# jilljenn/vae

Hardware: AMD Instinct MI355X
Metric: rating-triples/sec (ELBO step) at d=128 (higher is better)
Workload: dtype f32

## Files before the change

### include/vfm_hip.h

```cpp
#ifndef VFM_HIP_H
#define VFM_HIP_H

#include <stdint.h>

#ifdef __cplusplus
extern "C" {
#endif

#define VFM_ABI_VERSION 5
#define VFM_MAX_FIELDS 64
#define VFM_STRUCT_INIT(s) do { memset(&(s), 0, sizeof(s)); (s).struct_size = (uint32_t)sizeof(s); \
                                (s).abi_version = VFM_ABI_VERSION; } while (0)

#define VFM_E_INVALID (-1)
#define VFM_E_UNSUPPORTED (-2)

#define VFM_LIK_NORMAL 0
#define VFM_LIK_BERNOULLI 1

#define VFM_FLAG_NO_PRIOR_TERMS 1
#define VFM_FLAG_SPARSE_ADAM 4
#define VFM_FLAG_SCALED_MOMENTS 32
#define VFM_MOMENT_PERIOD 128
#define VFM_FLAG_ROWS_TOUCHED 128
#define VFM_FLAG_ZREC 1024
#define VFM_FLAG_SHARE_GPU 2048
#define VFM_FLAG_EPS_ZERO 2
#define VFM_FLAG_LINK_SOFTPLUS 16

#define VFM_P_LL 0
#define VFM_P_KL 1
#define VFM_P_G 2
#define VFM_P_ALPHA 3
#define VFM_P_BADID 4
#define VFM_P_GE0 5
#define VFM_P_REDUCED 6
#define VFM_N_PARTIALS 8
#define VFM_SLOT_NTERMS 6
#define VFM_MAX_FWD_BLOCKS 4096
#define VFM_PARTIALS_LEN (VFM_N_PARTIALS * (1 + VFM_MAX_FWD_BLOCKS))

typedef struct vfm_step_consts {
  float step_size, bc2_sqrt;
  float a1, q2, c1, c2, s1, s2;
  int32_t store_true;
  int32_t k;
  int32_t scaled;
  int32_t reserved;
  float lr, beta1, beta2, eps;
} vfm_step_consts_t;
typedef struct vfm_dev_step {
  uint64_t philox_step;
  int64_t adam_step;
  uint64_t philox_step_bwd;
  int64_t adam_step_bwd;
  int64_t tab_first, tab_len;
  const vfm_step_consts_t* tab;
  int64_t error;
} vfm_dev_step_t;
int vfm_step_consts(float lr, float beta1, float beta2, float eps_adam, int64_t step, int32_t scaled,
                    vfm_step_consts_t* out);
int vfm_dev_step_set(vfm_dev_step_t* dev_step, uint64_t philox_step, int64_t adam_step, void* stream);

typedef struct vfm_problem {
  uint32_t struct_size;
  uint32_t abi_version;
  int64_t B;
  int64_t B_global;
  int64_t T;
  int64_t nb_train;
  int32_t F;
  int32_t d;
  int32_t likelihood;
  int32_t id_bits;
  int32_t n_samples;
  int32_t flags;
  int64_t group_hi[VFM_MAX_FIELDS];
  double group_n[VFM_MAX_FIELDS];
  uint64_t seed;
  uint64_t step;
  int64_t e_lo, e_hi;
  vfm_dev_step_t* dev_step;
  float* wrec;
} vfm_problem_t;
int vfm_wrec_build_f32(const float* bias_params, const float* inv_occ, int64_t T, float* wrec, void* stream);

#define VFM_HEAVY_LIST 64
#define VFM_HEAVY_MIN 8
#define VFM_HEAVY_DIRECT 8
typedef struct vfm_index {
  uint32_t struct_size;
  uint32_t abi_version;
  const int32_t* occ_ptr;
  const int32_t* occ_rows;
  const int32_t* heavy_ids;
  const int32_t* heavy_items;
  float* heavy_acc;
  int32_t n_heavy;
  int32_t n_items;
  const int32_t* touched_ids;
  int64_t n_touched;
  const int32_t* occ_other;
  int32_t max_items;
  int32_t heavy_list, heavy_threshold;
  int32_t* status;
} vfm_index_t;

int vfm_abi_version(void);
const char* vfm_last_error(void);

int64_t vfm_index_workspace_bytes(int64_t B, int32_t F, int64_t T);
int vfm_rebuild_heavy(int64_t T, const int32_t* occ_ptr, void* ws, int32_t heavy_list, int32_t threshold, int32_t* heavy_ids,
                      int64_t cap_heavy, int32_t* heavy_items, int64_t cap_items, int32_t* counts , void* stream);
int32_t vfm_heavy_threshold(int32_t heavy_list);
#define VFM_HEAVY_UNITS 8192
int32_t vfm_heavy_list_for(int64_t n_occ, int64_t T);
int vfm_build_index(int64_t B, int32_t F, int64_t T, int32_t id_bits, const void* x, void* ws, int32_t* occ_ptr,
                    int32_t* occ_rows, int32_t heavy_list, int32_t* heavy_ids, int64_t cap_heavy,
                    int32_t* heavy_items, int64_t cap_items, int32_t* touched_ids, int32_t* occ_other,
                    const float* inv_occ, double* W, int32_t* counts, int32_t* counts_host, void* stream);

int vfm_inv_occ_f32(const int64_t* nb_occ, float* inv_occ, int64_t T, void* stream);

int vfm_batch_norms(const vfm_problem_t* p, const void* x, const float* inv_occ, double* W,
                    void* stream);

int vfm_elbo_fwd_f32(const vfm_problem_t* p, const void* x, const float* y,
                     const float* entity_params, const float* bias_params,
                     const float* inv_occ, const float* scalars, const double* W,
                     const float* eps_entity, const float* eps_bias, const float* eps_global,
                     float* pred, double* partials, float* sumz, float* grow, void* stream);

int vfm_elbo_finalize_f32(const vfm_problem_t* p, double* partials, const float* scalars,
                          float* loss, void* stream);

int vfm_elbo_bwd_f32(const vfm_problem_t* p, const vfm_index_t* idx,
                     const float* entity_params, const float* bias_params,
                     const float* inv_occ, const float* scalars, const double* W,
                     const float* eps_entity, const float* eps_bias, const float* eps_global,
                     const float* sumz, const float* grow, const double* partials,
                     const float* grad_out, float* g_entity, float* g_bias, float* g_scalars,
                     void* stream);

int vfm_elbo_bwd_adam_f32(const vfm_problem_t* p, const vfm_index_t* idx,
                          float* entity_params, float* bias_params, float* scalars,
                          const float* inv_occ, const double* W,
                          const float* eps_entity, const float* eps_bias, const float* eps_global,
                          const float* sumz, const float* grow, double* partials,
                          float* m_entity, float* v_entity, float* m_bias, float* v_bias,
                          float* m_scalars, float* v_scalars,
                          float lr, float beta1, float beta2, float eps_adam, int64_t step, float* loss,
                          void* stream);

int vfm_elbo_bwd_acc_f32(const vfm_problem_t* p, const vfm_index_t* idx,
                         const float* sumz, const float* grow, const double* partials, float* acc,
                         float* sums, void* stream);
int vfm_elbo_apply_adam_f32(const vfm_problem_t* p, const float* acc, const float* sums,
                            float* entity_params, float* bias_params, float* scalars, const float* inv_occ,
                            const double* W, const float* eps_entity, const float* eps_bias,
                            const float* eps_global, float* m_entity, float* v_entity, float* m_bias,
                            float* v_bias, float* m_scalars, float* v_scalars, float lr, float beta1,
                            float beta2, float eps_adam, int64_t step, void* stream);
int vfm_elbo_bwd_acc_rows_f32(const vfm_problem_t* p, const vfm_index_t* idx, const int32_t* row_ids, int64_t n_rows,
                              const float* sumz, const float* grow, const double* partials, float* acc,
                              float* sums, void* stream);
int vfm_elbo_apply_adam_rows_f32(const vfm_problem_t* p, const float* acc, const float* sums, const int32_t* row_ids,
                                 int64_t n_rows, int32_t compact_records, float* entity_params, float* bias_params, float* scalars,
                                 const float* inv_occ, const double* W, float* m_entity, float* v_entity, float* m_bias,
                                 float* v_bias, float* m_scalars, float* v_scalars, float lr, float beta1, float beta2,
                                 float eps_adam, int64_t step, void* stream);
int vfm_adam_f32(float* p, const float* g, float* m, float* v, int64_t n, float lr, float beta1,
                 float beta2, float eps, int64_t step, void* stream);

typedef struct vfm_pipe {
  uint32_t struct_size;
  uint32_t abi_version;
  const float* zrec;
  float* zrec_next;
  const int32_t* next_occ_ptr;
  const double* next_W;
  uint64_t next_step;
  int32_t* last_step;
  float* step_tab;
} vfm_pipe_t;
int vfm_sample_records_f32(const vfm_problem_t* p, const int32_t* ids, int64_t n, const float* entity_params,
                           const float* bias_params, const float* inv_occ, const double* W, float* zrec, void* stream);
int vfm_elbo_bwd_adam_pipe_f32(const vfm_problem_t* p, const vfm_index_t* idx, const vfm_pipe_t* pipe,
                               float* entity_params, float* bias_params, float* scalars,
                               const float* inv_occ, const double* W, const float* grow, double* partials,
                               float* m_entity, float* v_entity, float* m_bias, float* v_bias,
                               float* m_scalars, float* v_scalars,
                               float lr, float beta1, float beta2, float eps_adam, int64_t step, float* loss,
                               void* stream);

int vfm_adam_catchup_f32(float* entity_params, float* bias_params, const float* m_entity, const float* v_entity,
                         const float* m_bias, const float* v_bias, int32_t* last_step, const int32_t* ids, int64_t n,
                         int64_t T, int32_t d, const float* lr_of_step, int64_t n_lr, float beta1, float beta2,
                         float eps_adam, int64_t upto, int64_t mark, float* wrec, void* stream);

int64_t vfm_union_workspace_bytes(int64_t T);
int vfm_union_rows(int64_t T, const int32_t* occ_ptr_a, const int32_t* occ_ptr_b, void* ws, int32_t* rows, int32_t* count,
                   int32_t* count_host, void* stream);
int vfm_elbo_bwd_adam_lookahead_f32(const vfm_problem_t* p, const vfm_index_t* idx,
                                    float* entity_params, float* bias_params, float* scalars,
                                    const float* inv_occ, const double* W,
                                    const float* sumz, const float* grow, double* partials,
                                    float* m_entity, float* v_entity, float* m_bias, float* v_bias,
                                    float* m_scalars, float* v_scalars,
                                    float lr, float beta1, float beta2, float eps_adam, int64_t step, float* loss,
                                    int32_t* last_step, const int32_t* next_occ_ptr, float* step_tab, void* stream);

int vfm_moments_rescale_f32(float* m, float* v, int64_t n, float beta1, float beta2, int64_t step, int32_t to_scaled,
                            void* stream);

#define VFM_OBJ_SAMPLED 0
#define VFM_OBJ_CLOSED_FORM 1
int vfm_variant_fwd_f32(const vfm_problem_t* p, int32_t objective, const void* x, const float* values, const float* y,
                        const float* entity_params, const float* bias_params, const float* inv_occ,
                        const float* scalars, const double* W, const float* priors, const float* eps_entity,
                        const float* eps_bias, const float* eps_global, float* pred, double* partials, float* state,
                        float* grow, float* loss, void* stream);
int64_t vfm_variant_workspace_elems(int64_t B, int32_t F, int32_t d);
int vfm_variant_bwd_f32(const vfm_problem_t* p, int32_t objective, const vfm_index_t* idx, int32_t* occ_pos_ws,
                        const void* x, const float* values, const float* entity_params, const float* bias_params,
                        const float* inv_occ, const float* scalars, const double* W, const float* priors,
                        const float* eps_entity, const float* eps_bias, const float* eps_global, const float* state,
                        const float* grow, const double* partials, const float* grad_out, float* g_entity,
                        float* g_bias, float* g_scalars, float* g_priors, void* stream);

int vfm_philox_eps_f32(const vfm_problem_t* p, float* eps_entity, float* eps_bias,
                       float* eps_global, void* stream);

#ifdef __cplusplus
}
#endif
#endif
```

### vae_amd/_abi_gen.py

```python
import ctypes as C

VFM_ABI_VERSION = 5
VFM_E_INVALID = -1
VFM_E_UNSUPPORTED = -2
VFM_FLAG_EPS_ZERO = 2
VFM_FLAG_LINK_SOFTPLUS = 16
VFM_FLAG_NO_PRIOR_TERMS = 1
VFM_FLAG_ROWS_TOUCHED = 128
VFM_FLAG_SCALED_MOMENTS = 32
VFM_FLAG_SHARE_GPU = 2048
VFM_FLAG_SPARSE_ADAM = 4
VFM_FLAG_ZREC = 1024
VFM_HEAVY_DIRECT = 8
VFM_HEAVY_LIST = 64
VFM_HEAVY_MIN = 8
VFM_HEAVY_UNITS = 8192
VFM_LIK_BERNOULLI = 1
VFM_LIK_NORMAL = 0
VFM_MAX_FIELDS = 64
VFM_MAX_FWD_BLOCKS = 4096
VFM_MOMENT_PERIOD = 128
VFM_N_PARTIALS = 8
VFM_OBJ_CLOSED_FORM = 1
VFM_OBJ_SAMPLED = 0
VFM_PARTIALS_LEN = 32776
VFM_P_ALPHA = 3
VFM_P_BADID = 4
VFM_P_G = 2
VFM_P_GE0 = 5
VFM_P_KL = 1
VFM_P_LL = 0
VFM_P_REDUCED = 6
VFM_SLOT_NTERMS = 6


class StepConsts(C.Structure):
    _fields_ = [
        ("step_size", C.c_float),
        ("bc2_sqrt", C.c_float),
        ("a1", C.c_float),
        ("q2", C.c_float),
        ("c1", C.c_float),
        ("c2", C.c_float),
        ("s1", C.c_float),
        ("s2", C.c_float),
        ("store_true", C.c_int32),
        ("k", C.c_int32),
        ("scaled", C.c_int32),
        ("reserved", C.c_int32),
        ("lr", C.c_float),
        ("beta1", C.c_float),
        ("beta2", C.c_float),
        ("eps", C.c_float),
    ]


class DevStep(C.Structure):
    _fields_ = [
        ("philox_step", C.c_uint64),
        ("adam_step", C.c_int64),
        ("philox_step_bwd", C.c_uint64),
        ("adam_step_bwd", C.c_int64),
        ("tab_first", C.c_int64),
        ("tab_len", C.c_int64),
        ("tab", C.c_void_p),
        ("error", C.c_int64),
    ]


class Problem(C.Structure):
    _fields_ = [
        ("struct_size", C.c_uint32),
        ("abi_version", C.c_uint32),
        ("B", C.c_int64),
        ("B_global", C.c_int64),
        ("T", C.c_int64),
        ("nb_train", C.c_int64),
        ("F", C.c_int32),
        ("d", C.c_int32),
        ("likelihood", C.c_int32),
        ("id_bits", C.c_int32),
        ("n_samples", C.c_int32),
        ("flags", C.c_int32),
        ("group_hi", C.c_int64 * VFM_MAX_FIELDS),
        ("group_n", C.c_double * VFM_MAX_FIELDS),
        ("seed", C.c_uint64),
        ("step", C.c_uint64),
        ("e_lo", C.c_int64),
        ("e_hi", C.c_int64),
        ("dev_step", C.c_void_p),
        ("wrec", C.c_void_p),
    ]

    def __init__(self, *a, **k):
        super().__init__(*a, **k)
        self.struct_size, self.abi_version = C.sizeof(type(self)), VFM_ABI_VERSION


class Index(C.Structure):
    _fields_ = [
        ("struct_size", C.c_uint32),
        ("abi_version", C.c_uint32),
        ("occ_ptr", C.c_void_p),
        ("occ_rows", C.c_void_p),
        ("heavy_ids", C.c_void_p),
        ("heavy_items", C.c_void_p),
        ("heavy_acc", C.c_void_p),
        ("n_heavy", C.c_int32),
        ("n_items", C.c_int32),
        ("touched_ids", C.c_void_p),
        ("n_touched", C.c_int64),
        ("occ_other", C.c_void_p),
        ("max_items", C.c_int32),
        ("heavy_list", C.c_int32),
        ("heavy_threshold", C.c_int32),
        ("status", C.c_void_p),
    ]

    def __init__(self, *a, **k):
        super().__init__(*a, **k)
        self.struct_size, self.abi_version = C.sizeof(type(self)), VFM_ABI_VERSION


class Pipe(C.Structure):
    _fields_ = [
        ("struct_size", C.c_uint32),
        ("abi_version", C.c_uint32),
        ("zrec", C.c_void_p),
        ("zrec_next", C.c_void_p),
        ("next_occ_ptr", C.c_void_p),
        ("next_W", C.c_void_p),
        ("next_step", C.c_uint64),
        ("last_step", C.c_void_p),
        ("step_tab", C.c_void_p),
    ]

    def __init__(self, *a, **k):
        super().__init__(*a, **k)
        self.struct_size, self.abi_version = C.sizeof(type(self)), VFM_ABI_VERSION
```

### vae_amd/csrc/vfm_abi.hip

```cpp
#include <stdio.h>
#include <string.h>
#include <math.h>
#include <stdlib.h>
#include <mutex>

#include "vfm_args.hpp"

namespace vfm {

namespace {
thread_local char g_err[512] = "";
}

int fail(int code, const char* msg) {
  snprintf(g_err, sizeof(g_err), "%s", msg);
  return code;
}
int fail_hip(hipError_t e, const char* where) {
  snprintf(g_err, sizeof(g_err), "%s: %s", where, hipGetErrorString(e));
  return (int)e;
}
int env_int(const char* name, int dflt) {
  const char* v = getenv(name);
  return (v && *v) ? atoi(v) : dflt;
}

namespace {

#include "vfm_rng.hpp"
#include "vfm_common.hpp"
#include "vfm_reduce.hpp"
#include "vfm_small_kernels.hpp"
#include "vfm_heavy.hpp"
#include "vfm_adam.hpp"

bool pick_shape(int d, Shape* s) {
  auto pow2ceil = [](int v) { int p = 1; while (p < v) p <<= 1; return p; };
  if (d % 4 == 0) {
    const int C = d / 4;
    s->vec = 4;
    s->lpe = pow2ceil(C) < 64 ? (pow2ceil(C) < 4 ? 4 : pow2ceil(C)) : 64;
    const int cpl = (C + s->lpe - 1) / s->lpe;
    s->cpl = cpl <= 1 ? 1 : (cpl <= 2 ? 2 : 4);
    return cpl <= 4;
  }
  s->vec = 1;
  if (d <= 8) { s->lpe = 8; s->cpl = 1; return true; }
  if (d <= 64) { s->lpe = 64; s->cpl = 1; return true; }
  s->lpe = 64; s->cpl = 4;
  return d <= 256;
}

int check_struct(uint32_t size, uint32_t abi, size_t want, const char* name) {
  if (size == (uint32_t)want && abi == (uint32_t)VFM_ABI_VERSION) return 0;
  snprintf(g_err, sizeof(g_err), "%s: struct_size %u / abi_version %u, this library expects %zu / %d (set them with "
           "VFM_STRUCT_INIT; a binding generated from another version of include/vfm_hip.h must be regenerated)",
           name, size, abi, want, VFM_ABI_VERSION);
  return VFM_E_INVALID;
}

int check_problem(const vfm_problem_t* p, bool dev_ok = false) {
  if (!p) return fail(VFM_E_INVALID, "problem is NULL");
  if (int rc = check_struct(p->struct_size, p->abi_version, sizeof(vfm_problem_t), "vfm_problem_t")) return rc;
  if (p->dev_step && !dev_ok)
    return fail(VFM_E_UNSUPPORTED, "vfm_problem_t.dev_step: only the training forward and the fused backward+Adam entry points read the step from device memory");
  if (p->dev_step && p->n_samples != 1) return fail(VFM_E_UNSUPPORTED, "vfm_problem_t.dev_step: one variational sample");
  if (p->dev_step && (((uintptr_t)p->dev_step) & 15) != 0) return fail(VFM_E_INVALID, "vfm_problem_t.dev_step must be 16-byte aligned");
  if (p->wrec && (((uintptr_t)p->wrec) & 15) != 0) return fail(VFM_E_INVALID, "vfm_problem_t.wrec must be 16-byte aligned");
  if (p->B < 0 || p->T <= 0 || p->T > 0xFFFFFFFELL) return fail(VFM_E_INVALID, "bad B or T");
  if (p->F < 1 || p->F > VFM_MAX_FIELDS) return fail(VFM_E_INVALID, "F out of range [1,64]");
  if (p->d < 1) return fail(VFM_E_INVALID, "d < 1");
  if (p->id_bits != 32 && p->id_bits != 64) return fail(VFM_E_INVALID, "id_bits must be 32 or 64");
  if (p->likelihood != VFM_LIK_NORMAL && p->likelihood != VFM_LIK_BERNOULLI)
    return fail(VFM_E_INVALID, "unknown likelihood");
  if (p->n_samples < 1 || p->n_samples > MAX_SAMPLES) return fail(VFM_E_INVALID, "n_samples out of range [1,64]");
  if (p->n_samples > 1 && (p->step >> 48) != 0) return fail(VFM_E_INVALID, "step must stay below 2^48 when n_samples > 1");
  if (p->B_global < p->B) return fail(VFM_E_INVALID, "B_global < B");
  if (p->B * (int64_t)p->F > 0x7FFFFFFFLL) return fail(VFM_E_INVALID, "B*F exceeds int32 index range");
  if (p->e_lo < 0 || p->e_lo > p->T || (p->e_hi != 0 && p->e_hi < p->e_lo)) return fail(VFM_E_INVALID, "bad entity range");
  if (p->flags & ~(VFM_FLAG_NO_PRIOR_TERMS | VFM_FLAG_EPS_ZERO | VFM_FLAG_SPARSE_ADAM | VFM_FLAG_LINK_SOFTPLUS |
                   VFM_FLAG_SCALED_MOMENTS | VFM_FLAG_ROWS_TOUCHED | VFM_FLAG_ZREC | VFM_FLAG_SHARE_GPU))
    return fail(VFM_E_INVALID, "unknown bit in vfm_problem_t.flags");
  Shape s;
  if (!pick_shape(p->d, &s)) return fail(VFM_E_UNSUPPORTED, "embedding size d not supported (d%4==0: d<=1024, else d<=256)");
  return 0;
}

bool softplus(const vfm_problem_t* p) { return (p->flags & VFM_FLAG_LINK_SOFTPLUS) != 0; }

int single_sample_only(const vfm_problem_t* p, const char* who) {
  if (p->n_samples == 1) return 0;
  snprintf(g_err, sizeof(g_err), "%s: n_samples > 1 is not supported by this entry point", who);
  return VFM_E_UNSUPPORTED;
}


int eps_mode(const vfm_problem_t* p, const float* ee, const float* eb, const float* eg, int* mode) {
  const int neps = (ee != nullptr) + (eb != nullptr) + (eg != nullptr);
  if (neps != 0 && neps != 3) return fail(VFM_E_INVALID, "give all three eps tables or none");
  *mode = (p->flags & VFM_FLAG_EPS_ZERO) ? EPS_ZERO : (neps == 3 ? EPS_TABLE : EPS_PHILOX);
  return 0;
}

KArgs make_args(const vfm_problem_t* p, const void* x, const float* y, const float* entity,
                const float* bias, const float* inv_occ, const float* scalars, const double* W,
                const float* ee, const float* eb, const float* eg, int sample = 0) {
  KArgs a;
  memset(&a, 0, sizeof(a));
  a.S = p->n_samples; a.sample = sample; a.inv_S = 1.0f / (float)p->n_samples;
  if (sample > 0) {
    if (ee) ee += (size_t)sample * (size_t)p->T * (size_t)p->d;
    if (eb) eb += (size_t)sample * (size_t)p->T;
  }
  a.B = p->B; a.T = p->T; a.F = p->F; a.d = p->d; a.lik = p->likelihood;
  a.e_lo = p->e_lo; a.e_hi = (p->e_hi > 0 && p->e_hi < p->T) ? p->e_hi : p->T;
  a.id64 = p->id_bits == 64; a.G = p->F; a.flags = p->flags;
  a.ll_scale_d = (double)p->nb_train / ((double)(p->B_global > 0 ? p->B_global : 1) * (double)p->n_samples);
  a.ll_scale = (float)a.ll_scale_d;
  a.key.seed_lo = (uint32_t)p->seed; a.key.seed_hi = (uint32_t)(p->seed >> 32);
  a.key.step_lo = (uint32_t)p->step; a.key.step_hi = (uint32_t)(p->step >> 32);
  a.key.chunk_off = 0;
  a.x = x; a.y = y; a.entity = entity; a.bias = bias; a.inv_occ = inv_occ; a.scalars = scalars;
  a.W = W; a.eps_entity = ee; a.eps_bias = eb; a.eps_global = eg;
  a.dev = p->dev_step; a.wrec = p->wrec;
  for (int g = 0; g < p->F; ++g) { a.group_hi[g] = p->group_hi[g]; a.group_n[g] = p->group_n[g]; }
  return a;
}

bool use_fwd2(const vfm_problem_t* p, int eps, bool multi = false) {
  if (p->F != 2 || (p->d & 3) != 0 || p->d > 512) return false;
  if (multi ? (p->n_samples < 2 || p->n_samples > 4 || eps == EPS_ZERO) : p->n_samples != 1) return false;
  if (softplus(p)) return false;
  const int forced = env_int("VFM_FWD_KERNEL", 0);
  if (forced == 1) return false;
  return forced == 2 || eps == EPS_ZREC || multi || p->d >= 20;
}

bool use_fwdg(const vfm_problem_t* p, int eps, int mode) {
  if (p->F == 2 || (p->d & 3) != 0 || p->d < 16 || p->d > 512 || p->n_samples != 1) return false;
  if ((p->flags & VFM_FLAG_ZREC) || softplus(p)) return false;
  if (!(eps == EPS_PHILOX || (eps == EPS_ZERO && mode == MODE_PREDICT))) return false;
  return env_int("VFM_FWD_KERNEL", 0) != 1;
}

int dispatch_fwd(const vfm_problem_t* p, const Shape& s, int eps, int mode, int ff, KArgs& a, const FwdOut& o,
                 hipStream_t st) {
  if (use_fwdg(p, eps, mode)) return launch_fwdg_abs(eps, mode, a, o, st);
  if (use_fwd2(p, eps)) {
    if (mode == MODE_TRAIN && eps == EPS_PHILOX && env_int("VFM_FWD_AB_NORNG", 0) == 1) eps = EPS_ZERO;
    return launch_fwd2_abs(eps, mode, a, o, st);
  }
  return softplus(p) ? launch_fwd_softplus(s, eps, mode, ff, a, o, st) : launch_fwd_abs(s, eps, mode, ff, a, o, st);
}
int dispatch_bwd(const vfm_problem_t* p, const Shape& s, int eps, int adam, KArgs& a, const BwdArgs& b,
                 const AdamArgs& ad, hipStream_t st) {
  if (adam == 0 || adam == 10)
    return softplus(p) ? launch_bwd0_softplus(s, eps, adam, a, b, ad, st) : launch_bwd0_abs(s, eps, adam, a, b, ad, st);
  return softplus(p) ? launch_bwd1_softplus(s, eps, adam, a, b, ad, st) : launch_bwd1_abs(s, eps, adam, a, b, ad, st);
}

BwdArgs bwd_args(const vfm_problem_t* p, const vfm_index_t* idx) {
  BwdArgs b;
  memset(&b, 0, sizeof(b));
  if (idx) { b.occ_ptr = idx->occ_ptr; b.occ_rows = idx->occ_rows; b.status = idx->status; }
  b.n_occ = (int32_t)(p->B * (int64_t)p->F);
  return b;
}

template <int LPE, int CPL, int VEC>
int launch_heavy_t(const vfm_problem_t* p, const vfm_index_t* idx, const float* sumz, const float* grow, float* hacc, int d,
                   hipStream_t st, const float* zrec = nullptr) {
  constexpr int GPB = BLOCK / LPE;
  const size_t xs = 4 + (((size_t)d + 3) & ~(size_t)3);
  float* item_acc = hacc + xs * (size_t)idx->n_heavy;
  int64_t nb = ((int64_t)idx->n_items + GPB - 1) / GPB;
  if (nb > 4096) nb = 4096;
  hipLaunchKernelGGL((k_heavy<LPE, CPL, VEC>), dim3((unsigned)nb), dim3(BLOCK), 0, st, idx->heavy_items,
                     (int)idx->n_items, idx->occ_rows, sumz, grow, item_acc, d, zrec ? idx->occ_other : nullptr, zrec, hacc,
                     (int)idx->n_heavy, (int)(p->B * (int64_t)p->F), (int)p->B, p->T, idx->status);
  if (idx->max_items > 0 && idx->max_items <= VFM_HEAVY_DIRECT) return 0;
  nb = idx->n_heavy;
  if (nb > 4096) nb = 4096;
  hipLaunchKernelGGL((k_heavy_sum<LPE, CPL, VEC>), dim3((unsigned)nb), dim3(BLOCK), 0, st, idx->heavy_items,
                     (int)idx->n_items, (int)idx->n_heavy, item_acc, hacc, d);
  return 0;
}

int run_heavy(const vfm_problem_t* p, const vfm_index_t* idx, const float* sumz, const float* grow,
              hipStream_t st, BwdArgs* b, const float* zrec = nullptr) {
  b->heavy_ids = nullptr; b->heavy_acc = nullptr; b->n_heavy = 0; b->heavy_stride = 0;
  if (idx->n_heavy <= 0 || idx->n_items <= 0) return 0;
  if (!idx->heavy_ids || !idx->heavy_items || !idx->heavy_acc)
    return fail(VFM_E_INVALID, "index: heavy_ids / heavy_items / heavy_acc missing");
  if ((int64_t)idx->n_heavy > p->T || (int64_t)idx->n_items > p->B * (int64_t)p->F + idx->n_heavy)
    return fail(VFM_E_INVALID, "index: more heavy entities than table rows, or more work items than occurrences");
  const size_t xs = 4 + (((size_t)p->d + 3) & ~(size_t)3);
  const size_t per_sample = xs * ((size_t)idx->n_heavy + (size_t)idx->n_items);
  Shape s;
  pick_shape(p->d, &s);
  for (int sm = 0; sm < p->n_samples; ++sm) {
    const float* sz = sumz ? sumz + (size_t)sm * (size_t)p->B * (size_t)p->d : nullptr;
    float* hacc = idx->heavy_acc + (size_t)sm * per_sample;
#define X(L_, C_, V_) \
    if (s.lpe == L_ && s.cpl == C_ && s.vec == V_) launch_heavy_t<L_, C_, V_>(p, idx, sz, grow, hacc, p->d, st, zrec);
    VFM_FOR_SHAPES(X)
#undef X
  }
  b->heavy_ids = idx->heavy_ids; b->heavy_acc = idx->heavy_acc; b->n_heavy = idx->n_heavy;
  b->heavy_stride = idx->n_heavy + idx->n_items;
  return 0;
}

struct Side { hipStream_t s = nullptr; hipEvent_t e1 = nullptr, e2 = nullptr; bool ok = false, tried = false; std::mutex mu; };
Side* side_of_device() {
  static Side sides[64];
  static std::mutex mu;
  int dev = 0;
  if (hipGetDevice(&dev) != hipSuccess || dev < 0 || dev >= 64) return nullptr;
  std::lock_guard<std::mutex> lk(mu);
  Side& sd = sides[dev];
  if (!sd.tried) {
    sd.tried = true;
    sd.ok = hipStreamCreateWithFlags(&sd.s, hipStreamNonBlocking) == hipSuccess &&
            hipEventCreateWithFlags(&sd.e1, hipEventDisableTiming) == hipSuccess &&
            hipEventCreateWithFlags(&sd.e2, hipEventDisableTiming) == hipSuccess;
  }
  return sd.ok ? &sd : nullptr;
}
bool heavy_overlap(const vfm_problem_t* p, const vfm_index_t* idx) {
  return idx->n_heavy > 0 && idx->n_items > 0 && (int64_t)idx->n_heavy * 16 < p->T && p->n_samples == 1 &&
         env_int("VFM_HEAVY_OVERLAP", 1) != 0;
}

int bwd_adam_overlapped(const vfm_problem_t* p, const vfm_index_t* idx, const Shape& s, int eps, int adam, KArgs& a, BwdArgs& b,
                        const AdamArgs& ad, const float* sumz, const float* grow, hipStream_t st, Side* sd) {
  std::lock_guard<std::mutex> lk(sd->mu);
  hipError_t e = hipEventRecord(sd->e1, st);
  if (e == hipSuccess) e = hipStreamWaitEvent(sd->s, sd->e1, 0);
  if (e != hipSuccess) return fail_hip(e, "heavy-list overlap: events");
  if (int rc = run_heavy(p, idx, sumz, grow, sd->s, &b)) return rc;
  e = hipEventRecord(sd->e2, sd->s);
  if (e != hipSuccess) return fail_hip(e, "heavy-list overlap: events");
  const int32_t keep = a.row_filter;
  a.row_filter = 4;
  if (int rc = dispatch_bwd(p, s, eps, adam, a, b, ad, st)) return rc;
  e = hipStreamWaitEvent(st, sd->e2, 0);
  if (e != hipSuccess) return fail_hip(e, "heavy-list overlap: events");
  BwdArgs bh = b;
  bh.row_ids = idx->heavy_ids; bh.n_rows = idx->n_heavy;
  a.row_filter = 3;
  const int rc = dispatch_bwd(p, s, eps, adam, a, bh, ad, st);
  a.row_filter = keep;
  return rc;
}

bool small_table_step(const vfm_problem_t* p, const vfm_index_t* idx, int eps, int rows_flags) {
  if (eps != EPS_PHILOX || rows_flags != 0 || p->n_samples != 1 || (p->flags & VFM_FLAG_SPARSE_ADAM)) return false;
  if ((p->d & 3) != 0 || p->d > 256) return false;
  if (idx->heavy_list < VFM_HEAVY_MIN || idx->heavy_threshold < VFM_HEAVY_MIN || idx->heavy_threshold > idx->heavy_list) return false;
  if (p->T * (2 * (int64_t)p->d + 2) * 4 > (2LL << 20)) return false;
  return env_int("VFM_BWD_SMALL", 1) != 0;
}

int check_index(const vfm_problem_t* p, const vfm_index_t* idx, const char* who) {
  if (!idx) { snprintf(g_err, sizeof(g_err), "%s: inverted index missing", who); return VFM_E_INVALID; }
  if (int rc = check_struct(idx->struct_size, idx->abi_version, sizeof(vfm_index_t), "vfm_index_t")) return rc;
  if (!idx->occ_ptr || (p->B > 0 && !idx->occ_rows)) {
    snprintf(g_err, sizeof(g_err), "%s: inverted index missing", who);
    return VFM_E_INVALID;
  }
  if (idx->n_heavy < 0 || idx->n_items < 0 || idx->n_touched < 0 || idx->max_items < 0) {
    snprintf(g_err, sizeof(g_err), "%s: negative count in vfm_index_t", who);
    return VFM_E_INVALID;
  }
  return 0;
}

int after_launch(const char* where) {
  const hipError_t e = hipGetLastError();
  if (e != hipSuccess) return fail_hip(e, where);
  return 0;
}

void adam_consts(float lr, float beta1, float beta2, int64_t step, float* step_size, float* bc2_sqrt) {
  const double bc1 = 1.0 - pow((double)beta1, (double)step);
  const double bc2 = 1.0 - pow((double)beta2, (double)step);
  *step_size = (float)((double)lr / bc1);
  *bc2_sqrt = (float)sqrt(bc2);
}

void scaled_step_consts(float step_size, float bc2_sqrt, double s1, double s2, float* a1, float* q2) {
  *a1 = (float)((double)step_size * s1);
  *q2 = (float)(sqrt(s2) / (double)bc2_sqrt);
}

int scaled_moment_consts(const vfm_problem_t* p, float beta1, float beta2, int64_t step, AdamArgs* ad) {
  ad->scaled = 0; ad->store_true = 0; ad->s1 = ad->s2 = 1.f; ad->c1 = 1.f - beta1; ad->c2 = 1.f - beta2;
  ad->inv_bc2_sqrt = 1.0f / ad->bc2_sqrt;
  ad->a1 = ad->step_size; ad->q2 = ad->inv_bc2_sqrt;
  if (!(p->flags & VFM_FLAG_SCALED_MOMENTS)) return 0;
  if (p->flags & VFM_FLAG_SPARSE_ADAM)
    return fail(VFM_E_INVALID, "VFM_FLAG_SCALED_MOMENTS and VFM_FLAG_SPARSE_ADAM exclude each other");
  const int64_t k = (step - 1) % VFM_MOMENT_PERIOD + 1;
  const double s1 = pow((double)beta1, (double)k), s2 = pow((double)beta2, (double)k);
  if (!(s1 > 1e-30) || !(s2 > 1e-30))
    return fail(VFM_E_UNSUPPORTED, "VFM_FLAG_SCALED_MOMENTS: beta^128 underflows (use the plain moments for such betas)");
  ad->scaled = 1; ad->store_true = (k == VFM_MOMENT_PERIOD);
  ad->s1 = (float)s1; ad->s2 = (float)s2;
  ad->c1 = (float)((1.0 - (double)beta1) / s1); ad->c2 = (float)((1.0 - (double)beta2) / s2);
  scaled_step_consts(ad->step_size, ad->bc2_sqrt, s1, s2, &ad->a1, &ad->q2);
  return 0;
}

}
}

using namespace vfm;

int vfm::launch_norms(int64_t B, int F, int64_t T, int id_bits, const void* x, const float* inv_occ, double* W, hipStream_t st) {
  hipLaunchKernelGGL(k_zero_f64, dim3(1), dim3(64), 0, st, W, F);
  if (B == 0) return after_launch("vfm_batch_norms");
  int64_t nbx = (B + BLOCK * 8 - 1) / (BLOCK * 8);
  if (nbx > 1024) nbx = 1024;
  hipLaunchKernelGGL(k_norms, dim3((unsigned)nbx, (unsigned)F), dim3(BLOCK), 0, st, x, (int)(id_bits == 64), inv_occ, B, F, T,
                     reinterpret_cast<unsigned long long*>(W));
  hipLaunchKernelGGL(k_norms_fix, dim3(1), dim3(64), 0, st, W, F);
  return after_launch("vfm_batch_norms");
}

extern "C" {

int vfm_abi_version(void) { return VFM_ABI_VERSION; }
const char* vfm_last_error(void) { return g_err; }

int vfm_step_consts(float lr, float beta1, float beta2, float eps_adam, int64_t step, int32_t scaled,
                    vfm_step_consts_t* out) {
  if (!out || step < 1) return fail(VFM_E_INVALID, "vfm_step_consts: bad argument");
  vfm_problem_t p;
  memset(&p, 0, sizeof(p));
  p.flags = scaled ? VFM_FLAG_SCALED_MOMENTS : 0;
  AdamArgs ad;
  memset(&ad, 0, sizeof(ad));
  ad.b1 = beta1; ad.b2 = beta2; ad.eps = eps_adam;
  adam_consts(lr, beta1, beta2, step, &ad.step_size, &ad.bc2_sqrt);
  if (int rc = scaled_moment_consts(&p, beta1, beta2, step, &ad)) return rc;
  memset(out, 0, sizeof(*out));
  out->step_size = ad.step_size; out->bc2_sqrt = ad.bc2_sqrt; out->a1 = ad.a1; out->q2 = ad.q2;
  out->c1 = ad.c1; out->c2 = ad.c2; out->s1 = ad.s1; out->s2 = ad.s2;
  out->store_true = ad.store_true; out->k = (int32_t)((step - 1) % VFM_MOMENT_PERIOD + 1); out->scaled = ad.scaled;
  out->lr = lr; out->beta1 = beta1; out->beta2 = beta2; out->eps = eps_adam;
  return 0;
}

int vfm_dev_step_set(vfm_dev_step_t* dev_step, uint64_t philox_step, int64_t adam_step, void* stream) {
  if (!dev_step || adam_step < 1) return fail(VFM_E_INVALID, "vfm_dev_step_set: bad argument");
  hipLaunchKernelGGL(k_dev_step_set, dim3(1), dim3(64), 0, (hipStream_t)stream, dev_step, philox_step, adam_step);
  return after_launch("vfm_dev_step_set");
}

int vfm_wrec_build_f32(const float* bias_params, const float* inv_occ, int64_t T, float* wrec, void* stream) {
  if (!bias_params || !inv_occ || !wrec || T <= 0 || (((uintptr_t)wrec) & 15) != 0)
    return fail(VFM_E_INVALID, "vfm_wrec_build_f32: bad argument");
  const int grid = (int)((T + 255) / 256 < 2048 ? (T + 255) / 256 : 2048);
  hipLaunchKernelGGL(k_wrec_build, dim3(grid), dim3(256), 0, (hipStream_t)stream, bias_params, inv_occ, T, wrec);
  return after_launch("vfm_wrec_build_f32");
}

int vfm_inv_occ_f32(const int64_t* nb_occ, float* inv_occ, int64_t T, void* stream) {
  if (!nb_occ || !inv_occ || T <= 0) return fail(VFM_E_INVALID, "vfm_inv_occ_f32: bad argument");
  const int grid = (int)((T + 255) / 256 < 2048 ? (T + 255) / 256 : 2048);
  hipLaunchKernelGGL(k_inv_occ, dim3(grid), dim3(256), 0, (hipStream_t)stream, nb_occ, inv_occ, T);
  return after_launch("vfm_inv_occ_f32");
}

int vfm_batch_norms(const vfm_problem_t* p, const void* x, const float* inv_occ, double* W,
                    void* stream) {
  if (int rc = check_problem(p)) return rc;
  if (!W || (p->B > 0 && (!x || !inv_occ))) return fail(VFM_E_INVALID, "vfm_batch_norms: NULL pointer");
  return launch_norms(p->B, p->F, p->T, p->id_bits, x, inv_occ, W, (hipStream_t)stream);
}

int vfm_elbo_fwd_f32(const vfm_problem_t* p, const void* x, const float* y,
                     const float* entity_params, const float* bias_params,
                     const float* inv_occ, const float* scalars, const double* W,
                     const float* eps_entity, const float* eps_bias, const float* eps_global,
                     float* pred, double* partials, float* sumz, float* grow, void* stream) {
  if (int rc = check_problem(p, true)) return rc;
  if (!partials) return fail(VFM_E_INVALID, "vfm_elbo_fwd_f32: partials is NULL");
  if (p->dev_step && (eps_entity || eps_bias || eps_global || (p->flags & VFM_FLAG_EPS_ZERO)))
    return fail(VFM_E_UNSUPPORTED, "vfm_elbo_fwd_f32: dev_step goes with the in-kernel Philox eps stream only");
  hipStream_t st0 = (hipStream_t)stream;
  if (p->B == 0) {
    hipLaunchKernelGGL(k_zero_f64, dim3(1), dim3(64), 0, st0, partials, (int)VFM_N_PARTIALS);
    return after_launch("vfm_elbo_fwd_f32");
  }
  const bool zrec = (p->flags & VFM_FLAG_ZREC) != 0;
  if (zrec) {
    if (!use_fwd2(p, EPS_ZREC)) return fail(VFM_E_UNSUPPORTED, "VFM_FLAG_ZREC: two fields, one sample, d % 4 == 0, d <= 512, |.| link");
    if (!x || !y || !entity_params || !scalars || !pred || !grow || eps_entity || eps_bias || eps_global)
      return fail(VFM_E_INVALID, "vfm_elbo_fwd_f32 (VFM_FLAG_ZREC): x, y, the record table, scalars, pred, grow; no eps tables");
    KArgs a = make_args(p, x, y, entity_params, nullptr, nullptr, scalars, nullptr, nullptr, nullptr, nullptr, 0);
    FwdOut o{pred, partials, nullptr, grow};
    if (int rc = launch_fwd2_abs(EPS_ZREC, MODE_TRAIN, a, o, (hipStream_t)stream)) return rc;
    return after_launch("vfm_elbo_fwd_f32");
  }
  if (!x || !entity_params || !bias_params || !scalars || !pred)
    return fail(VFM_E_INVALID, "vfm_elbo_fwd_f32: NULL pointer");
  const bool train = y != nullptr;
  if (train && (!inv_occ || !W || !sumz || !grow))
    return fail(VFM_E_INVALID, "vfm_elbo_fwd_f32: y given, so inv_occ, W, sumz and grow are required");
  if (!train && (sumz || grow)) return fail(VFM_E_INVALID, "vfm_elbo_fwd_f32: sumz / grow need y");
  int eps;
  if (int rc = eps_mode(p, eps_entity, eps_bias, eps_global, &eps)) return rc;
  if (train && eps == EPS_ZERO) return fail(VFM_E_UNSUPPORTED, "vfm_elbo_fwd_f32: VFM_FLAG_EPS_ZERO is prediction-only");
  hipStream_t st = (hipStream_t)stream;
  FwdOut o{pred, partials, sumz, grow};
  Shape s;
  pick_shape(p->d, &s);
  if (use_fwd2(p, eps, true)) {
    KArgs a = make_args(p, x, y, entity_params, bias_params, inv_occ, scalars, W, eps_entity, eps_bias, eps_global, 0);
    const int md = train ? MODE_TRAIN : MODE_PREDICT;
    if (int rc = launch_fwd2m_abs(eps, md, a, o, st)) return rc;
    return after_launch("vfm_elbo_fwd_f32");
  }
  for (int sm = 0; sm < p->n_samples; ++sm) {
    KArgs a = make_args(p, x, y, entity_params, bias_params, inv_occ, scalars, W, eps_entity, eps_bias,
                        eps_global, sm);
    if (int rc = dispatch_fwd(p, s, eps, train ? MODE_TRAIN : MODE_PREDICT, p->F == 2 ? 2 : 0, a, o, st)) return rc;
  }
  return after_launch("vfm_elbo_fwd_f32");
}

int vfm_elbo_finalize_f32(const vfm_problem_t* p, double* partials, const float* scalars,
                          float* loss, void* stream) {
  if (int rc = check_problem(p)) return rc;
  if (!partials || !scalars || !loss) return fail(VFM_E_INVALID, "vfm_elbo_finalize_f32: NULL pointer");
  const double ll_scale = (double)p->nb_train / ((double)(p->B_global > 0 ? p->B_global : 1) * (double)p->n_samples);
  hipLaunchKernelGGL(k_finalize, dim3(1), dim3(BLOCK), 0, (hipStream_t)stream, partials, scalars, ll_scale,
                     (int)p->flags, loss);
  return after_launch("vfm_elbo_finalize_f32");
}

int vfm_elbo_bwd_f32(const vfm_problem_t* p, const vfm_index_t* idx,
                     const float* entity_params, const float* bias_params,
                     const float* inv_occ, const float* scalars, const double* W,
                     const float* eps_entity, const float* eps_bias, const float* eps_global,
                     const float* sumz, const float* grow, const double* partials,
                     const float* grad_out, float* g_entity, float* g_bias, float* g_scalars,
                     void* stream) {
  if (int rc = check_problem(p)) return rc;
  if (int rc = check_index(p, idx, "vfm_elbo_bwd_f32")) return rc;
  if (!entity_params || !bias_params || !inv_occ || !scalars || !W || !partials || !grad_out ||
      !g_entity || !g_bias || !g_scalars || (p->B > 0 && (!sumz || !grow)))
    return fail(VFM_E_INVALID, "vfm_elbo_bwd_f32: NULL pointer");
  int eps;
  if (int rc = eps_mode(p, eps_entity, eps_bias, eps_global, &eps)) return rc;
  if (eps == EPS_ZERO) return fail(VFM_E_UNSUPPORTED, "vfm_elbo_bwd_f32: VFM_FLAG_EPS_ZERO is prediction-only");
  KArgs a = make_args(p, nullptr, nullptr, entity_params, bias_params, inv_occ, scalars, W, eps_entity,
                      eps_bias, eps_global);
  BwdArgs b = bwd_args(p, idx);
  b.sumz = sumz; b.grow = grow; b.partials = const_cast<double*>(partials); b.grad_out = grad_out;
  b.g_entity = g_entity; b.g_bias = g_bias; b.g_scalars = g_scalars;
  if (int rc = run_heavy(p, idx, sumz, grow, (hipStream_t)stream, &b)) return rc;
  AdamArgs ad;
  memset(&ad, 0, sizeof(ad));
  Shape s;
  pick_shape(p->d, &s);
  if (int rc = dispatch_bwd(p, s, eps, 0, a, b, ad, (hipStream_t)stream)) return rc;
  return after_launch("vfm_elbo_bwd_f32");
}

int vfm_elbo_bwd_adam_f32(const vfm_problem_t* p, const vfm_index_t* idx,
                          float* entity_params, float* bias_params, float* scalars,
                          const float* inv_occ, const double* W,
                          const float* eps_entity, const float* eps_bias, const float* eps_global,
                          const float* sumz, const float* grow, double* partials,
                          float* m_entity, float* v_entity, float* m_bias, float* v_bias,
                          float* m_scalars, float* v_scalars,
                          float lr, float beta1, float beta2, float eps_adam, int64_t step, float* loss,
                          void* stream) {
  if (int rc = check_problem(p, true)) return rc;
  if (int rc = check_index(p, idx, "vfm_elbo_bwd_adam_f32")) return rc;
  if (p->dev_step) {
    if ((p->flags & VFM_FLAG_SPARSE_ADAM) || eps_entity || eps_bias || eps_global)
      return fail(VFM_E_UNSUPPORTED, "vfm_elbo_bwd_adam_f32: dev_step excludes VFM_FLAG_SPARSE_ADAM and eps tables");
    step = 1; lr = 0.f;
  }
  const int rows_flags = p->flags & VFM_FLAG_ROWS_TOUCHED;
  if (rows_flags && (p->flags & VFM_FLAG_SPARSE_ADAM))
    return fail(VFM_E_INVALID, "vfm_elbo_bwd_adam_f32: VFM_FLAG_ROWS_TOUCHED does not combine with VFM_FLAG_SPARSE_ADAM");
  if (!entity_params || !bias_params || !scalars || !m_entity ||
      !v_entity || !m_bias || !v_bias || !m_scalars || !v_scalars || step < 1 ||
      !inv_occ || !W || !partials || (p->B > 0 && (!sumz || !grow)))
    return fail(VFM_E_INVALID, "vfm_elbo_bwd_adam_f32: bad argument");
  if (p->flags & VFM_FLAG_NO_PRIOR_TERMS)
    return fail(VFM_E_INVALID, "vfm_elbo_bwd_adam_f32: single-rank only (gradients never leave the kernel)");
  int eps;
  if (int rc = eps_mode(p, eps_entity, eps_bias, eps_global, &eps)) return rc;
  if (eps == EPS_ZERO) return fail(VFM_E_UNSUPPORTED, "vfm_elbo_bwd_adam_f32: VFM_FLAG_EPS_ZERO is prediction-only");
  KArgs a = make_args(p, nullptr, nullptr, entity_params, bias_params, inv_occ, scalars, W, eps_entity,
                      eps_bias, eps_global);
  a.row_filter = rows_flags == VFM_FLAG_ROWS_TOUCHED ? 2 : 0;
  BwdArgs b = bwd_args(p, idx);
  b.sumz = sumz; b.grow = grow; b.partials = partials; b.loss = loss;
  if (small_table_step(p, idx, eps, rows_flags)) {
    AdamArgs ad{m_entity, v_entity, m_bias, v_bias, m_scalars, v_scalars, beta1, beta2, eps_adam, 0.f, 0.f};
    adam_consts(lr, beta1, beta2, step, &ad.step_size, &ad.bc2_sqrt);
    if (int rc = scaled_moment_consts(p, beta1, beta2, step, &ad)) return rc;
    Shape s;
    pick_shape(p->d, &s);
    if (int rc = softplus(p) ? launch_bwd_small_softplus(s, a, b, ad, idx->heavy_list, idx->heavy_threshold, (hipStream_t)stream)
                             : launch_bwd_small_abs(s, a, b, ad, idx->heavy_list, idx->heavy_threshold, (hipStream_t)stream))
      return rc;
    return after_launch("vfm_elbo_bwd_adam_f32");
  }
  Side* sd = (!(p->flags & VFM_FLAG_SPARSE_ADAM) && heavy_overlap(p, idx)) ? side_of_device() : nullptr;
  if (!sd)
    if (int rc = run_heavy(p, idx, sumz, grow, (hipStream_t)stream, &b)) return rc;
  AdamArgs ad{m_entity, v_entity, m_bias, v_bias, m_scalars, v_scalars, beta1, beta2, eps_adam, 0.f, 0.f};
  adam_consts(lr, beta1, beta2, step, &ad.step_size, &ad.bc2_sqrt);
  if (int rc = scaled_moment_consts(p, beta1, beta2, step, &ad)) return rc;
  Shape s;
  pick_shape(p->d, &s);
  int adam = (p->flags & VFM_FLAG_SPARSE_ADAM) ? 2 : 1;
  if (rows_flags == VFM_FLAG_ROWS_TOUCHED && idx->touched_ids && idx->n_touched <= p->T && env_int("VFM_ROWS_LIST", 1) != 0) {
    b.row_ids = idx->touched_ids; b.n_rows = idx->n_touched;
    a.row_filter = 0;
  }
  if (sd && a.row_filter == 0) {
    if (int rc = bwd_adam_overlapped(p, idx, s, eps, adam, a, b, ad, sumz, grow, (hipStream_t)stream, sd)) return rc;
    return after_launch("vfm_elbo_bwd_adam_f32");
  }
  if (sd)
    if (int rc = run_heavy(p, idx, sumz, grow, (hipStream_t)stream, &b)) return rc;
  if (int rc = dispatch_bwd(p, s, eps, adam, a, b, ad, (hipStream_t)stream)) return rc;
  return after_launch("vfm_elbo_bwd_adam_f32");
}

static int bwd_acc_impl(const vfm_problem_t* p, const vfm_index_t* idx, const int32_t* row_ids, int64_t n_rows,
                        const float* sumz, const float* grow, const double* partials, float* acc, float* sums, void* stream,
                        const char* who) {
  if (int rc = check_problem(p)) return rc;
  if (int rc = single_sample_only(p, who)) return rc;
  if (int rc = check_index(p, idx, who)) return rc;
  if (!partials || !acc || !sums || (p->B > 0 && (!sumz || !grow)))
    return fail(VFM_E_INVALID, "vfm_elbo_bwd_acc_f32: NULL pointer");
  KArgs a = make_args(p, nullptr, nullptr, nullptr, nullptr, nullptr, nullptr, nullptr, nullptr, nullptr, nullptr);
  BwdArgs b = bwd_args(p, idx);
  b.sumz = sumz; b.grow = grow; b.partials = const_cast<double*>(partials); b.acc = acc; b.sums = sums;
  if (row_ids) {
    if (n_rows < 0 || n_rows > p->T || p->e_lo != 0 || (p->e_hi != 0 && p->e_hi != p->T))
      return fail(VFM_E_INVALID, "vfm_elbo_bwd_acc_rows_f32: 0 <= n_rows <= T, whole entity range");
    b.row_ids = row_ids; b.n_rows = n_rows; b.rec_by_slot = 1;
  }
  if (p->e_lo == 0)
    if (int rc = run_heavy(p, idx, sumz, grow, (hipStream_t)stream, &b)) return rc;
  if (p->e_lo != 0 && idx->n_heavy > 0) {
    b.heavy_ids = idx->heavy_ids; b.heavy_acc = idx->heavy_acc; b.n_heavy = idx->n_heavy;
    b.heavy_stride = idx->n_heavy + idx->n_items;
  }
  AdamArgs ad;
  memset(&ad, 0, sizeof(ad));
  Shape s;
  pick_shape(p->d, &s);
  if (int rc = dispatch_bwd(p, s, EPS_ZERO, 10, a, b, ad, (hipStream_t)stream)) return rc;
  return after_launch(who);
}

int vfm_elbo_bwd_acc_f32(const vfm_problem_t* p, const vfm_index_t* idx,
                         const float* sumz, const float* grow, const double* partials, float* acc,
                         float* sums, void* stream) {
  return bwd_acc_impl(p, idx, nullptr, 0, sumz, grow, partials, acc, sums, stream, "vfm_elbo_bwd_acc_f32");
}

int vfm_elbo_bwd_acc_rows_f32(const vfm_problem_t* p, const vfm_index_t* idx, const int32_t* row_ids, int64_t n_rows,
                              const float* sumz, const float* grow, const double* partials, float* acc,
                              float* sums, void* stream) {
  static const int32_t none = 0;
  if (!row_ids && n_rows != 0) return fail(VFM_E_INVALID, "vfm_elbo_bwd_acc_rows_f32: row_ids is NULL");
  return bwd_acc_impl(p, idx, row_ids ? row_ids : &none, n_rows, sumz, grow, partials, acc, sums, stream,
                      "vfm_elbo_bwd_acc_rows_f32");
}

static int apply_adam_impl(const vfm_problem_t* p, const float* acc, const float* sums,
                           float* entity_params, float* bias_params, float* scalars, const float* inv_occ,
                           const double* W, const float* eps_entity, const float* eps_bias,
                           const float* eps_global, float* m_entity, float* v_entity, float* m_bias,
                           float* v_bias, float* m_scalars, float* v_scalars, float lr, float beta1,
                           float beta2, float eps_adam, int64_t step, const int32_t* row_ids, int64_t n_rows,
                           int32_t compact, void* stream, const char* who) {
  if (int rc = check_problem(p)) return rc;
  if (int rc = single_sample_only(p, who)) return rc;
  if (!acc || !sums || !entity_params || !bias_params || !scalars || !inv_occ || !W || !m_entity ||
      !v_entity || !m_bias || !v_bias || !m_scalars || !v_scalars || step < 1)
    return fail(VFM_E_INVALID, "vfm_elbo_apply_adam_f32: bad argument");
  int eps;
  if (int rc = eps_mode(p, eps_entity, eps_bias, eps_global, &eps)) return rc;
  if (eps == EPS_ZERO) return fail(VFM_E_UNSUPPORTED, "vfm_elbo_apply_adam_f32: VFM_FLAG_EPS_ZERO is prediction-only");
  KArgs a = make_args(p, nullptr, nullptr, entity_params, bias_params, inv_occ, scalars, W, eps_entity, eps_bias,
                      eps_global);
  BwdArgs b = bwd_args(p, nullptr);
  b.acc = const_cast<float*>(acc); b.sums = const_cast<float*>(sums);
  if (row_ids) {
    if (n_rows < 0 || n_rows > p->T) return fail(VFM_E_INVALID, "vfm_elbo_apply_adam_rows_f32: 0 <= n_rows <= T");
    b.row_ids = row_ids; b.n_rows = n_rows; b.rec_by_slot = compact ? 1 : 0;
  }
  AdamArgs ad{m_entity, v_entity, m_bias, v_bias, m_scalars, v_scalars, beta1, beta2, eps_adam, 0.f, 0.f};
  adam_consts(lr, beta1, beta2, step, &ad.step_size, &ad.bc2_sqrt);
  if (int rc = scaled_moment_consts(p, beta1, beta2, step, &ad)) return rc;
  if (row_ids && (!ad.scaled || ad.store_true))
    return fail(VFM_E_INVALID, "vfm_elbo_apply_adam_rows_f32: scaled moments only, and not on the last step of a moment period "
                               "(bring every row up to date and run vfm_elbo_apply_adam_f32)");
  Shape s;
  pick_shape(p->d, &s);
  if (int rc = dispatch_bwd(p, s, eps, 11, a, b, ad, (hipStream_t)stream)) return rc;
  return after_launch(who);
}

int vfm_elbo_apply_adam_f32(const vfm_problem_t* p, const float* acc, const float* sums,
                            float* entity_params, float* bias_params, float* scalars, const float* inv_occ,
                            const double* W, const float* eps_entity, const float* eps_bias,
                            const float* eps_global, float* m_entity, float* v_entity, float* m_bias,
                            float* v_bias, float* m_scalars, float* v_scalars, float lr, float beta1,
                            float beta2, float eps_adam, int64_t step, void* stream) {
  return apply_adam_impl(p, acc, sums, entity_params, bias_params, scalars, inv_occ, W, eps_entity, eps_bias, eps_global,
                         m_entity, v_entity, m_bias, v_bias, m_scalars, v_scalars, lr, beta1, beta2, eps_adam, step,
                         nullptr, 0, 0, stream, "vfm_elbo_apply_adam_f32");
}

int vfm_elbo_apply_adam_rows_f32(const vfm_problem_t* p, const float* acc, const float* sums, const int32_t* row_ids,
                                 int64_t n_rows, int32_t compact_records, float* entity_params, float* bias_params, float* scalars,
                                 const float* inv_occ, const double* W, float* m_entity, float* v_entity, float* m_bias,
                                 float* v_bias, float* m_scalars, float* v_scalars, float lr, float beta1, float beta2,
                                 float eps_adam, int64_t step, void* stream) {
  if (!row_ids && n_rows != 0) return fail(VFM_E_INVALID, "vfm_elbo_apply_adam_rows_f32: row_ids is NULL");
  static const int32_t none = 0;
  return apply_adam_impl(p, acc, sums, entity_params, bias_params, scalars, inv_occ, W, nullptr, nullptr, nullptr,
                         m_entity, v_entity, m_bias, v_bias, m_scalars, v_scalars, lr, beta1, beta2, eps_adam, step,
                         row_ids ? row_ids : &none, n_rows, compact_records, stream,
                         "vfm_elbo_apply_adam_rows_f32");
}

int vfm_adam_f32(float* p, const float* g, float* m, float* v, int64_t n, float lr, float beta1,
                 float beta2, float eps, int64_t step, void* stream) {
  if (!p || !g || !m || !v || n < 0 || step < 1) return fail(VFM_E_INVALID, "vfm_adam_f32: bad argument");
  if (n == 0) return 0;
  if ((((uintptr_t)p | (uintptr_t)g | (uintptr_t)m | (uintptr_t)v) & 15) != 0)
    return fail(VFM_E_INVALID, "vfm_adam_f32: pointers must be 16-byte aligned");
  float step_size, bc2_sqrt;
  adam_consts(lr, beta1, beta2, step, &step_size, &bc2_sqrt);
  const int64_t n4 = n / 4;
  int64_t nb = (n4 + BLOCK - 1) / BLOCK;
  if (nb < 1) nb = 1;
  const int grid = (int)(nb < 4096 ? nb : 4096);
  hipLaunchKernelGGL(k_adam, dim3(grid), dim3(BLOCK), 0, (hipStream_t)stream, p, g, m, v, n4, n, beta1,
                     beta2, eps, step_size, bc2_sqrt);
  return after_launch("vfm_adam_f32");
}

int vfm_sample_records_f32(const vfm_problem_t* p, const int32_t* ids, int64_t n, const float* entity_params,
                           const float* bias_params, const float* inv_occ, const double* W, float* zrec, void* stream) {
  if (int rc = check_problem(p)) return rc;
  if (int rc = single_sample_only(p, "vfm_sample_records_f32")) return rc;
  if ((p->d & 3) != 0 || softplus(p)) return fail(VFM_E_UNSUPPORTED, "vfm_sample_records_f32: d % 4 == 0, |.| link");
  if (n < 0 || n > 0x7FFFFFFFLL || (n > 0 && (!ids || !entity_params || !bias_params || !inv_occ || !W || !zrec)))
    return fail(VFM_E_INVALID, "vfm_sample_records_f32: bad argument");
  if (n == 0) return 0;
  KArgs a = make_args(p, nullptr, nullptr, entity_params, bias_params, inv_occ, nullptr, W, nullptr, nullptr, nullptr);
  Shape s;
  pick_shape(p->d, &s);
  if (int rc = launch_sample_rec_abs(s, a, ids, (int)n, zrec, (hipStream_t)stream)) return rc;
  return after_launch("vfm_sample_records_f32");
}

int vfm_elbo_bwd_adam_pipe_f32(const vfm_problem_t* p, const vfm_index_t* idx, const vfm_pipe_t* pipe,
                               float* entity_params, float* bias_params, float* scalars,
                               const float* inv_occ, const double* W, const float* grow, double* partials,
                               float* m_entity, float* v_entity, float* m_bias, float* v_bias,
                               float* m_scalars, float* v_scalars,
                               float lr, float beta1, float beta2, float eps_adam, int64_t step, float* loss,
                               void* stream) {
  if (int rc = check_problem(p, true)) return rc;
  if (p->dev_step) { step = 1; lr = 0.f; }
  if (int rc = single_sample_only(p, "vfm_elbo_bwd_adam_pipe_f32")) return rc;
  if (int rc = check_index(p, idx, "vfm_elbo_bwd_adam_pipe_f32")) return rc;
  if (p->F != 2 || (p->d & 3) != 0 || p->d > 512)
    return fail(VFM_E_UNSUPPORTED, "vfm_elbo_bwd_adam_pipe_f32: two fields, d % 4 == 0, d <= 512");
  if (p->flags & ~(VFM_FLAG_SCALED_MOMENTS | VFM_FLAG_SHARE_GPU))
    return fail(VFM_E_UNSUPPORTED, "vfm_elbo_bwd_adam_pipe_f32: only VFM_FLAG_SCALED_MOMENTS (the record step exists for the |.| link)");
  if (!pipe) return fail(VFM_E_INVALID, "vfm_elbo_bwd_adam_pipe_f32: pipe is NULL");
  if (int rc = check_struct(pipe->struct_size, pipe->abi_version, sizeof(vfm_pipe_t), "vfm_pipe_t")) return rc;
  if (!pipe->zrec || (p->B > 0 && !idx->occ_other) ||
      (pipe->zrec_next && (!pipe->next_occ_ptr || !pipe->next_W)))
    return fail(VFM_E_INVALID, "vfm_elbo_bwd_adam_pipe_f32: pipe / idx->occ_other incomplete");
  if (pipe->last_step) {
    if (!pipe->next_occ_ptr || !pipe->step_tab || !(p->flags & VFM_FLAG_SCALED_MOMENTS))
      return fail(VFM_E_INVALID, "vfm_elbo_bwd_adam_pipe_f32 (look-ahead form): next_occ_ptr, step_tab and VFM_FLAG_SCALED_MOMENTS");
    if (!p->dev_step && step % VFM_MOMENT_PERIOD == 0)
      return fail(VFM_E_INVALID, "vfm_elbo_bwd_adam_pipe_f32 (look-ahead form): the last step of a moment period is a dense one");
  }
  if (!entity_params || !bias_params || !scalars || !m_entity || !v_entity || !m_bias || !v_bias || !m_scalars ||
      !v_scalars || step < 1 || !inv_occ || !W || !partials || (p->B > 0 && !grow))
    return fail(VFM_E_INVALID, "vfm_elbo_bwd_adam_pipe_f32: bad argument");
  KArgs a = make_args(p, nullptr, nullptr, entity_params, bias_params, inv_occ, scalars, W, nullptr, nullptr, nullptr);
  BwdArgs b = bwd_args(p, idx);
  b.grow = grow; b.partials = partials; b.loss = loss;
  if (int rc = run_heavy(p, idx, nullptr, grow, (hipStream_t)stream, &b, pipe->zrec)) return rc;
  b.zrec = pipe->zrec; b.occ_other = idx->occ_other;
  b.zrec_next = pipe->zrec_next; b.next_occ_ptr = pipe->next_occ_ptr; b.next_W = pipe->next_W;
  b.next_key = a.key;
  b.next_key.step_lo = (uint32_t)pipe->next_step; b.next_key.step_hi = (uint32_t)(pipe->next_step >> 32);
  if (pipe->last_step) {
    b.last_step = pipe->last_step; b.step_tab = reinterpret_cast<float2*>(pipe->step_tab);
    b.la_step = (int32_t)step; b.la_k = (int32_t)((step - 1) % VFM_MOMENT_PERIOD + 1);
    if (idx->touched_ids && idx->n_touched > 0) {
      if (idx->n_touched > p->T) return fail(VFM_E_INVALID, "vfm_elbo_bwd_adam_pipe_f32: more listed rows than table rows");
      b.row_ids = idx->touched_ids; b.n_rows = idx->n_touched;
    }
  }
  AdamArgs ad{m_entity, v_entity, m_bias, v_bias, m_scalars, v_scalars, beta1, beta2, eps_adam, 0.f, 0.f};
  adam_consts(lr, beta1, beta2, step, &ad.step_size, &ad.bc2_sqrt);
  if (int rc = scaled_moment_consts(p, beta1, beta2, step, &ad)) return rc;
  Shape s;
  pick_shape(p->d, &s);
  if (int rc = dispatch_bwd(p, s, EPS_PHILOX, 1, a, b, ad, (hipStream_t)stream)) return rc;
  return after_launch("vfm_elbo_bwd_adam_pipe_f32");
}

int vfm_elbo_bwd_adam_lookahead_f32(const vfm_problem_t* p, const vfm_index_t* idx,
                                    float* entity_params, float* bias_params, float* scalars,
                                    const float* inv_occ, const double* W,
                                    const float* sumz, const float* grow, double* partials,
                                    float* m_entity, float* v_entity, float* m_bias, float* v_bias,
                                    float* m_scalars, float* v_scalars,
                                    float lr, float beta1, float beta2, float eps_adam, int64_t step, float* loss,
                                    int32_t* last_step, const int32_t* next_occ_ptr, float* step_tab, void* stream) {
  if (int rc = check_problem(p, true)) return rc;
  if (p->dev_step) { step = 1; lr = 0.f; }
  if (int rc = single_sample_only(p, "vfm_elbo_bwd_adam_lookahead_f32")) return rc;
  if (int rc = check_index(p, idx, "vfm_elbo_bwd_adam_lookahead_f32")) return rc;
  if ((p->flags & ~(VFM_FLAG_LINK_SOFTPLUS | VFM_FLAG_SHARE_GPU)) != VFM_FLAG_SCALED_MOMENTS)
    return fail(VFM_E_INVALID, "vfm_elbo_bwd_adam_lookahead_f32: VFM_FLAG_SCALED_MOMENTS (and optionally the link flag) only");
  if (!entity_params || !bias_params || !scalars || !m_entity || !v_entity || !m_bias || !v_bias || !m_scalars ||
      !v_scalars || step < 1 || !inv_occ || !W || !partials || (p->B > 0 && (!sumz || !grow)) || !last_step ||
      !next_occ_ptr || !step_tab)
    return fail(VFM_E_INVALID, "vfm_elbo_bwd_adam_lookahead_f32: bad argument");
  if (step % VFM_MOMENT_PERIOD == 0)
    return fail(VFM_E_INVALID, "vfm_elbo_bwd_adam_lookahead_f32: the last step of a moment period is a dense one "
                               "(bring every row up to date, then vfm_elbo_bwd_adam_f32)");
  KArgs a = make_args(p, nullptr, nullptr, entity_params, bias_params, inv_occ, scalars, W, nullptr, nullptr, nullptr);
  BwdArgs b = bwd_args(p, idx);
  b.sumz = sumz; b.grow = grow; b.partials = partials; b.loss = loss;
  Side* sd = heavy_overlap(p, idx) ? side_of_device() : nullptr;
  if (!sd)
    if (int rc = run_heavy(p, idx, sumz, grow, (hipStream_t)stream, &b)) return rc;
  b.last_step = last_step; b.next_occ_ptr = next_occ_ptr; b.step_tab = reinterpret_cast<float2*>(step_tab);
  if (idx->touched_ids && idx->n_touched > 0) {
    if (idx->n_touched > p->T) return fail(VFM_E_INVALID, "vfm_elbo_bwd_adam_lookahead_f32: more listed rows than table rows");
    b.row_ids = idx->touched_ids; b.n_rows = idx->n_touched;
  }
  b.la_step = (int32_t)step; b.la_k = (int32_t)((step - 1) % VFM_MOMENT_PERIOD + 1);
  AdamArgs ad{m_entity, v_entity, m_bias, v_bias, m_scalars, v_scalars, beta1, beta2, eps_adam, 0.f, 0.f};
  adam_consts(lr, beta1, beta2, step, &ad.step_size, &ad.bc2_sqrt);
  if (int rc = scaled_moment_consts(p, beta1, beta2, step, &ad)) return rc;
  Shape s;
  pick_shape(p->d, &s);
  if (sd) {
    if (int rc = bwd_adam_overlapped(p, idx, s, EPS_PHILOX, 1, a, b, ad, sumz, grow, (hipStream_t)stream, sd)) return rc;
    return after_launch("vfm_elbo_bwd_adam_lookahead_f32");
  }
  if (int rc = dispatch_bwd(p, s, EPS_PHILOX, 1, a, b, ad, (hipStream_t)stream)) return rc;
  return after_launch("vfm_elbo_bwd_adam_lookahead_f32");
}

int vfm_adam_catchup_f32(float* entity_params, float* bias_params, const float* m_entity, const float* v_entity,
                         const float* m_bias, const float* v_bias, int32_t* last_step, const int32_t* ids, int64_t n,
                         int64_t T, int32_t d, const float* lr_of_step, int64_t n_lr, float beta1, float beta2,
                         float eps_adam, int64_t upto, int64_t mark, float* wrec, void* stream) {
  if (!entity_params || !bias_params || !m_entity || !v_entity || !m_bias || !v_bias || !last_step || n < 0 || T < 1 ||
      d < 1 || upto < 0 || mark < upto || mark > 0x7FFFFFFFLL || (ids == nullptr && n != T))
    return fail(VFM_E_INVALID, "vfm_adam_catchup_f32: bad argument (ids == NULL means all T rows: n == T)");
  if (n == 0 || upto == 0) {
    if (n == 0) return 0;
  }
  const int64_t pstart = upto > 0 ? ((upto - 1) / VFM_MOMENT_PERIOD) * VFM_MOMENT_PERIOD : 0;
  const int kmax = (int)(upto - pstart);
  if (kmax > 0 && (!lr_of_step || n_lr < kmax))
    return fail(VFM_E_INVALID, "vfm_adam_catchup_f32: lr_of_step (host) needs one entry per step of the period up to `upto` (n_lr too small)");
  if (wrec && (((uintptr_t)wrec) & 15) != 0) return fail(VFM_E_INVALID, "vfm_adam_catchup_f32: wrec must be 16-byte aligned");
  CatchTab tab;
  memset(&tab, 0, sizeof(tab));
  for (int k = 1; k <= kmax; ++k) {
    float step_size, bc2_sqrt;
    adam_consts(lr_of_step[k - 1], beta1, beta2, pstart + k, &step_size, &bc2_sqrt);
    const double s1 = pow((double)beta1, (double)k), s2 = pow((double)beta2, (double)k);
    if (!(s1 > 1e-30) || !(s2 > 1e-30)) return fail(VFM_E_UNSUPPORTED, "vfm_adam_catchup_f32: beta^k underflows");
    float a1, q2;
    scaled_step_consts(step_size, bc2_sqrt, s1, s2, &a1, &q2);
    tab.c[k] = make_float4(a1, q2, 0.f, 0.f);
  }
  int64_t nb = (n + BLOCK / 64 - 1) / (BLOCK / 64);
  if (nb > 8192) nb = 8192;
  if ((d & 1) == 0)
    hipLaunchKernelGGL(k_adam_catchup<4>, dim3((unsigned)nb), dim3(BLOCK), 0, (hipStream_t)stream, entity_params, bias_params,
                       m_entity, v_entity, m_bias, v_bias, last_step, ids, n, (int)d, (int32_t)pstart, (int32_t)upto,
                       (int32_t)mark, eps_adam, tab, wrec);
  else
    hipLaunchKernelGGL(k_adam_catchup<1>, dim3((unsigned)nb), dim3(BLOCK), 0, (hipStream_t)stream, entity_params, bias_params,
                       m_entity, v_entity, m_bias, v_bias, last_step, ids, n, (int)d, (int32_t)pstart, (int32_t)upto,
                       (int32_t)mark, eps_adam, tab, wrec);
  return after_launch("vfm_adam_catchup_f32");
}

int vfm_moments_rescale_f32(float* m, float* v, int64_t n, float beta1, float beta2, int64_t step, int32_t to_scaled,
                            void* stream) {
  if (!m || !v || n < 0 || step < 0) return fail(VFM_E_INVALID, "vfm_moments_rescale_f32: bad argument");
  const int64_t k = step % VFM_MOMENT_PERIOD;
  if (k == 0 || n == 0) return 0;
  double c1 = pow((double)beta1, (double)k), c2 = pow((double)beta2, (double)k);
  if (!(c1 > 1e-30) || !(c2 > 1e-30)) return fail(VFM_E_UNSUPPORTED, "vfm_moments_rescale_f32: beta^k underflows");
  if (to_scaled) { c1 = 1.0 / c1; c2 = 1.0 / c2; }
  int64_t nb = (n + BLOCK - 1) / BLOCK;
  if (nb > 4096) nb = 4096;
  hipLaunchKernelGGL(k_rescale2, dim3((unsigned)nb), dim3(BLOCK), 0, (hipStream_t)stream, m, v, n, (float)c1, (float)c2);
  return after_launch("vfm_moments_rescale_f32");
}

int vfm_philox_eps_f32(const vfm_problem_t* p, float* eps_entity, float* eps_bias, float* eps_global,
                       void* stream) {
  if (int rc = check_problem(p)) return rc;
  if (!eps_entity || !eps_bias || !eps_global) return fail(VFM_E_INVALID, "vfm_philox_eps_f32: NULL pointer");
  for (int sm = 0; sm < p->n_samples; ++sm) {
    KArgs a = make_args(p, nullptr, nullptr, nullptr, nullptr, nullptr, nullptr, nullptr, nullptr, nullptr,
                        nullptr, sm);
    hipLaunchKernelGGL(k_philox_dump, dim3(1024), dim3(256), 0, (hipStream_t)stream, a,
                       eps_entity + (size_t)sm * (size_t)p->T * (size_t)p->d, eps_bias + (size_t)sm * (size_t)p->T,
                       eps_global + sm);
  }
  return after_launch("vfm_philox_eps_f32");
}

}
```

### vae_amd/csrc/vfm_args.hpp

```cpp
#pragma once
#include <hip/hip_runtime.h>
#include <stdint.h>

#include "vfm_hip.h"

#define VFM_INTERNAL __attribute__((visibility("hidden")))

namespace vfm {

constexpr int BLOCK = 256;
constexpr float LOG_SQRT_2PI = 0.918938533204672742f;
constexpr float LN2 = 0.693147180559945309f;
constexpr float LOG2E = 1.4426950408889634f;

struct RngKey {
  uint32_t seed_lo, seed_hi, step_lo, step_hi;
  uint32_t chunk_off;
};

struct KArgs {
  int64_t B, T;
  int64_t e_lo, e_hi;
  int32_t F, d, lik, id64, G, flags;
  int32_t S, sample;
  int32_t row_filter;
  float inv_S;
  float ll_scale;
  double ll_scale_d;
  RngKey key;
  const void* x;
  const float* y;
  const float* entity;
  const float* bias;
  const float* inv_occ;
  const float* scalars;
  const double* W;
  const float* eps_entity;
  const float* eps_bias;
  const float* eps_global;
  vfm_dev_step_t* dev;
  float* wrec;
  int64_t group_hi[VFM_MAX_FIELDS];
  double group_n[VFM_MAX_FIELDS];
};

struct FwdOut {
  float* pred;
  double* partials;
  float* sumz;
  float* grow;
};

struct BwdArgs {
  const int32_t* occ_ptr;
  const int32_t* occ_rows;
  const float* sumz;
  const float* grow;
  double* partials;
  const float* grad_out;
  float* g_entity;
  float* g_bias;
  float* g_scalars;
  float* loss;
  float* acc;
  float* sums;
  const int32_t* heavy_ids;
  const float* heavy_acc;
  int32_t n_heavy;
  int32_t heavy_stride;
  const int32_t* row_ids;
  int64_t n_rows;
  const float* zrec;
  const int32_t* occ_other;
  float* zrec_next;
  const int32_t* next_occ_ptr;
  const double* next_W;
  RngKey next_key;
  int32_t* last_step;
  float2* step_tab;
  int32_t la_step, la_k;
  int32_t rec_by_slot;
  int32_t n_occ;
  int32_t* status;
};

struct AdamArgs {
  float* m_entity; float* v_entity; float* m_bias; float* v_bias; float* m_scal; float* v_scal;
  float b1, b2, eps, step_size, bc2_sqrt;
  int32_t scaled, store_true;
  float s1, s2, c1, c2, inv_bc2_sqrt;
  float a1, q2;
};

__device__ __forceinline__ RngKey key_of_step(const KArgs& a, bool writer) {
  RngKey key = a.key;
  if (a.dev) {
    const uint64_t s = a.dev->philox_step;
    key.step_lo = (uint32_t)s; key.step_hi = (uint32_t)(s >> 32);
    if (writer) { a.dev->philox_step_bwd = s; a.dev->adam_step_bwd = a.dev->adam_step; }
  }
  return key;
}
__device__ __forceinline__ void load_dev_step(const KArgs& a, RngKey& key, AdamArgs& ad, int32_t& la_step, int32_t& la_k,
                                              RngKey& next_key, bool bump) {
  if (!a.dev) return;
  const uint64_t s = a.dev->philox_step_bwd;
  const int64_t t = a.dev->adam_step_bwd;
  key.step_lo = (uint32_t)s; key.step_hi = (uint32_t)(s >> 32);
  next_key.step_lo = (uint32_t)(s + 1); next_key.step_hi = (uint32_t)((s + 1) >> 32);
  int64_t i = t - a.dev->tab_first;
  const bool miss = i < 0 || i >= a.dev->tab_len;
  if (miss) i = i < 0 ? 0 : a.dev->tab_len - 1;
  const vfm_step_consts_t c = a.dev->tab[i];
  ad.step_size = c.step_size; ad.bc2_sqrt = c.bc2_sqrt; ad.inv_bc2_sqrt = 1.0f / c.bc2_sqrt;
  ad.a1 = c.a1; ad.q2 = c.q2; ad.c1 = c.c1; ad.c2 = c.c2; ad.s1 = c.s1; ad.s2 = c.s2;
  ad.store_true = c.store_true; ad.scaled = c.scaled;
  ad.b1 = c.beta1; ad.b2 = c.beta2; ad.eps = c.eps;
  la_step = (int32_t)t; la_k = c.k;
  if (bump) {
    a.dev->philox_step = s + 1; a.dev->adam_step = t + 1;
    if (miss) a.dev->error = 1;
  }
}

struct Shape {
  int lpe, cpl, vec;
};

enum { EPS_PHILOX = 0, EPS_TABLE = 1, EPS_ZERO = 2, EPS_ZREC = 4 };
enum { MODE_PREDICT = 0, MODE_TRAIN = 1 };
enum { STAGE_FULL = 0, STAGE_ACC = 1, STAGE_APPLY = 2 };
enum { LINK_ABS = 0, LINK_SOFTPLUS = 1 };
constexpr int MAX_SAMPLES = 64;

VFM_INTERNAL int fail(int code, const char* msg);
VFM_INTERNAL int fail_hip(hipError_t e, const char* where);
VFM_INTERNAL int env_int(const char* name, int dflt);
VFM_INTERNAL int launch_norms(int64_t B, int F, int64_t T, int id_bits, const void* x, const float* inv_occ, double* W,
                              hipStream_t st);

#define VFM_DECLARE_LAUNCHERS(SUFFIX)                                                                          \
  VFM_INTERNAL int launch_fwd_##SUFFIX(const Shape& s, int eps, int mode, int ff, KArgs& a, const FwdOut& o,   \
                                       hipStream_t st);                                                        \
  VFM_INTERNAL int launch_bwd0_##SUFFIX(const Shape& s, int eps, int adam, KArgs& a, const BwdArgs& b,         \
                                        const AdamArgs& ad, hipStream_t st);                                   \
  VFM_INTERNAL int launch_bwd1_##SUFFIX(const Shape& s, int eps, int adam, KArgs& a, const BwdArgs& b,         \
                                        const AdamArgs& ad, hipStream_t st);
VFM_DECLARE_LAUNCHERS(abs)
VFM_DECLARE_LAUNCHERS(softplus)
VFM_INTERNAL int launch_bwd_small_abs(const Shape& s, KArgs& a, const BwdArgs& b, const AdamArgs& ad, int L, int THR, hipStream_t st);
VFM_INTERNAL int launch_bwd_small_softplus(const Shape& s, KArgs& a, const BwdArgs& b, const AdamArgs& ad, int L, int THR, hipStream_t st);
VFM_INTERNAL int launch_fwd2_abs(int eps, int mode, KArgs& a, const FwdOut& o, hipStream_t st);
VFM_INTERNAL int launch_fwd2m_abs(int eps, int mode, KArgs& a, const FwdOut& o, hipStream_t st);
VFM_INTERNAL int launch_fwdg_abs(int eps, int mode, KArgs& a, const FwdOut& o, hipStream_t st);
VFM_INTERNAL int launch_sample_rec_abs(const Shape& s, KArgs& a, const int32_t* ids, int n, float* zrec, hipStream_t st);

#define VFM_FOR_SHAPES(X)                                                                      \
  X(4, 1, 4) X(8, 1, 4) X(16, 1, 4) X(32, 1, 4) X(64, 1, 4) X(64, 2, 4) \
  X(64, 4, 4) X(8, 1, 1) X(64, 1, 1) X(64, 4, 1)

}
```

### vae_amd/csrc/vfm_bwd.hip

```cpp
#include <math.h>

#include "vfm_args.hpp"

#ifndef VFM_LINK
#error "compile with -DVFM_LINK=0 (abs) or -DVFM_LINK=1 (softplus)"
#endif
#ifndef VFM_BWD_PART
#error "compile with -DVFM_BWD_PART=0 (gradient / statistics forms) or =1 (fused-Adam forms)"
#endif

namespace vfm {
namespace {

#include "vfm_rng.hpp"
#include "vfm_common.hpp"
#include "vfm_reduce.hpp"
#include "vfm_bwd.hpp"
#include "vfm_sample.hpp"
#if VFM_BWD_PART == 1
#include "vfm_bwd_small.hpp"
#endif

constexpr int LINK = VFM_LINK;

template <int LPE, int CPL, int VEC, int EPS, int ADAM, int STAGE = STAGE_FULL>
int launch_bwd_t(KArgs& a, const BwdArgs& b, const AdamArgs& ad, hipStream_t st) {
  constexpr int GPB = BLOCK / LPE;
  const int per_cu = env_int("VFM_BWD_BLOCKS_PER_CU", 8);
  int64_t nb = (a.e_hi - a.e_lo + GPB - 1) / GPB;
  if (ADAM != 0 && b.row_ids) nb = (b.n_rows + GPB - 1) / GPB;
  const int64_t cap = 256LL * per_cu;
  if (nb > cap) nb = cap;
  { const int share = env_int("VFM_SHARE_CAP", 960); if ((a.flags & VFM_FLAG_SHARE_GPU) && share > 0 && nb > share) nb = share; }
  { const int forced = env_int("VFM_BWD_GRID", 0); if (forced > 0 && nb > forced) nb = forced; }
  if (nb < 1) nb = 1;
  if constexpr (STAGE == STAGE_FULL && ADAM == 1 && EPS == EPS_PHILOX && VEC == 4 && LINK == LINK_ABS) {
    if (b.zrec != nullptr) {
      if (a.S > 1) return fail(VFM_E_UNSUPPORTED, "pipelined step: one variational sample");
      if (b.last_step != nullptr)
        hipLaunchKernelGGL((k_bwd<LPE, CPL, VEC, EPS, ADAM, STAGE, LINK, false, true, true>), dim3((unsigned)nb), dim3(BLOCK), 0, st, a, b, ad);
      else
        hipLaunchKernelGGL((k_bwd<LPE, CPL, VEC, EPS, ADAM, STAGE, LINK, false, true>), dim3((unsigned)nb), dim3(BLOCK), 0, st, a, b, ad);
      return 0;
    }
  }
  if (b.zrec != nullptr) return fail(VFM_E_UNSUPPORTED, "pipelined step: fused Adam, Philox eps, d % 4 == 0, |.| link only");
  if constexpr (STAGE == STAGE_FULL && ADAM == 1 && EPS == EPS_PHILOX) {
    if (b.last_step != nullptr) {
      if (a.S > 1) return fail(VFM_E_UNSUPPORTED, "look-ahead lazy Adam: one variational sample");
      hipLaunchKernelGGL((k_bwd<LPE, CPL, VEC, EPS, ADAM, STAGE, LINK, false, false, true>), dim3((unsigned)nb), dim3(BLOCK), 0, st, a, b, ad);
      return 0;
    }
  }
  if (b.last_step != nullptr) return fail(VFM_E_UNSUPPORTED, "look-ahead lazy Adam: fused Adam with Philox eps only");
  if constexpr (STAGE == STAGE_FULL) {
    if (a.S > 1) {
      hipLaunchKernelGGL((k_bwd<LPE, CPL, VEC, EPS, ADAM, STAGE, LINK, true>), dim3((unsigned)nb), dim3(BLOCK), 0, st, a, b, ad);
      return 0;
    }
  }
  hipLaunchKernelGGL((k_bwd<LPE, CPL, VEC, EPS, ADAM, STAGE, LINK, false>), dim3((unsigned)nb), dim3(BLOCK), 0, st, a, b, ad);
  return 0;
}

template <int LPE, int CPL, int VEC>
int launch_bwd_s(int eps, int adam, KArgs& a, const BwdArgs& b, const AdamArgs& ad, hipStream_t st) {
#if VFM_BWD_PART == 0
  if (eps == EPS_PHILOX && adam == 0) return launch_bwd_t<LPE, CPL, VEC, EPS_PHILOX, 0>(a, b, ad, st);
  if (eps == EPS_TABLE && adam == 0) return launch_bwd_t<LPE, CPL, VEC, EPS_TABLE, 0>(a, b, ad, st);
  if (adam == 10) return launch_bwd_t<LPE, CPL, VEC, EPS_ZERO, 0, STAGE_ACC>(a, b, ad, st);
#else
  if (eps == EPS_PHILOX && adam == 1) return launch_bwd_t<LPE, CPL, VEC, EPS_PHILOX, 1>(a, b, ad, st);
  if (eps == EPS_TABLE && adam == 1) return launch_bwd_t<LPE, CPL, VEC, EPS_TABLE, 1>(a, b, ad, st);
  if (eps == EPS_PHILOX && adam == 2) return launch_bwd_t<LPE, CPL, VEC, EPS_PHILOX, 2>(a, b, ad, st);
  if (eps == EPS_TABLE && adam == 2) return launch_bwd_t<LPE, CPL, VEC, EPS_TABLE, 2>(a, b, ad, st);
  if (eps == EPS_PHILOX && adam == 11) return launch_bwd_t<LPE, CPL, VEC, EPS_PHILOX, 1, STAGE_APPLY>(a, b, ad, st);
  if (eps == EPS_TABLE && adam == 11) return launch_bwd_t<LPE, CPL, VEC, EPS_TABLE, 1, STAGE_APPLY>(a, b, ad, st);
#endif
  return fail(VFM_E_UNSUPPORTED, "backward: unsupported eps source / form in this translation unit");
}

int dispatch_bwd(const Shape& s, int eps, int adam, KArgs& a, const BwdArgs& b, const AdamArgs& ad,
                 hipStream_t st) {
#define X(L_, C_, V_) \
  if (s.lpe == L_ && s.cpl == C_ && s.vec == V_) return launch_bwd_s<L_, C_, V_>(eps, adam, a, b, ad, st);
  VFM_FOR_SHAPES(X)
#undef X
  return fail(VFM_E_UNSUPPORTED, "no kernel instance for this embedding size");
}

#if VFM_BWD_PART == 1 && VFM_LINK == 0
int dispatch_sample_rec(const Shape& s, KArgs& a, const int32_t* ids, int n, float* zrec, hipStream_t st) {
#define X(L_, C_, V_)                                                                                   \
  if (s.lpe == L_ && s.cpl == C_ && s.vec == V_) {                                                      \
    constexpr int GPB = BLOCK / L_;                                                                     \
    int64_t nb = ((int64_t)n + GPB - 1) / GPB;                                                          \
    if (nb > 65535) nb = 65535;                                                                         \
    hipLaunchKernelGGL((k_sample_rec<L_, C_, V_, LINK>), dim3((unsigned)nb), dim3(BLOCK), 0, st, a, ids, n, zrec); \
    return 0;                                                                                           \
  }
  VFM_FOR_SHAPES(X)
#undef X
  return fail(VFM_E_UNSUPPORTED, "no kernel instance for this embedding size");
}

#endif

}

#if VFM_BWD_PART == 1 && VFM_LINK == 0
int launch_sample_rec_abs(const Shape& s, KArgs& a, const int32_t* ids, int n, float* zrec, hipStream_t st) {
  return dispatch_sample_rec(s, a, ids, n, zrec, st);
}
#endif

#if VFM_BWD_PART == 1
namespace {
int dispatch_bwd_small(const Shape& s, KArgs& a, const BwdArgs& b, const AdamArgs& ad, int L, int THR, hipStream_t st) {
  if (s.vec != 4 || s.cpl != 1) return fail(VFM_E_UNSUPPORTED, "small-table backward: d % 4 == 0, d <= 256");
  int64_t nb = (a.T + BLOCK / 64 - 1) / (BLOCK / 64);
  if (nb > 256 * 16) nb = 256 * 16;
#define X(L_)                                                                                                              \
  if (s.lpe == L_) {                                                                                                       \
    hipLaunchKernelGGL((k_bwd_small<L_, LINK>), dim3((unsigned)nb), dim3(BLOCK), 0, st, a, b, ad, L, THR);                 \
    return 0;                                                                                                              \
  }
  X(4) X(8) X(16) X(32) X(64)
#undef X
  return fail(VFM_E_UNSUPPORTED, "small-table backward: no instance for this embedding size");
}
}
#if VFM_LINK == 0
int launch_bwd_small_abs(const Shape& s, KArgs& a, const BwdArgs& b, const AdamArgs& ad, int L, int THR, hipStream_t st) {
  return dispatch_bwd_small(s, a, b, ad, L, THR, st);
}
#else
int launch_bwd_small_softplus(const Shape& s, KArgs& a, const BwdArgs& b, const AdamArgs& ad, int L, int THR, hipStream_t st) {
  return dispatch_bwd_small(s, a, b, ad, L, THR, st);
}
#endif
#endif

#define VFM_CAT3(a, b, c) a##b##c
#define VFM_BWD_NAME(part, suffix) VFM_CAT3(launch_bwd, part, suffix)
#if VFM_LINK == 0
int VFM_BWD_NAME(VFM_BWD_PART, _abs)(const Shape& s, int eps, int adam, KArgs& a, const BwdArgs& b, const AdamArgs& ad, hipStream_t st) {
  return dispatch_bwd(s, eps, adam, a, b, ad, st);
}
#else
int VFM_BWD_NAME(VFM_BWD_PART, _softplus)(const Shape& s, int eps, int adam, KArgs& a, const BwdArgs& b, const AdamArgs& ad, hipStream_t st) {
  return dispatch_bwd(s, eps, adam, a, b, ad, st);
}
#endif

}
```

### vae_amd/csrc/vfm_bwd.hpp

```cpp
#pragma once

__device__ __forceinline__ float adam_update(float p, float g, float& m, float& v, const AdamArgs& ad) {
  if (ad.scaled) {
    m = fmaf(ad.c1, g, m);
    v = fmaf(ad.c2 * g, g, v);
    const float denom = fmaf(__builtin_amdgcn_sqrtf(v), ad.q2, ad.eps);
    const float pn = fmaf(-ad.a1 * m, __builtin_amdgcn_rcpf(denom), p);
    if (ad.store_true) { m = m * ad.s1; v = v * ad.s2; }
    return pn;
  }
  m = m + (g - m) * (1.0f - ad.b1);
  v = v * ad.b2 + ((1.0f - ad.b2) * g) * g;
  const float denom = __fsqrt_rn(v) / ad.bc2_sqrt + ad.eps;
  return p + (-ad.step_size * m) / denom;
}

__device__ __forceinline__ int heavy_slot_of(const int32_t* ids, int n, int e) {
  int lo = 0, hi = n - 1;
  while (lo < hi) {
    const int mid = (lo + hi) >> 1;
    if (ids[mid] < e) lo = mid + 1; else hi = mid;
  }
  return (n > 0 && ids[lo] == e) ? lo : -1;
}
// ... 64 lines not shown
    const float prior = (a.flags & VFM_FLAG_NO_PRIOR_TERMS) ? 0.f : 1.f;
    const float ga = (a.lik == VFM_LIK_NORMAL)
                         ? gout * dlink_f<LINK>(alpha) * a.ll_scale * sum_a : 0.f;
    const float gm = gout * (sum_g + prior * m0);
    const float ge0 = MULTI ? (float)(fold ? fin[VFM_P_GE0] : b.partials[VFM_P_GE0]) : e0 * sum_g;
    const float gs = gout * dlink_f<LINK>(s0) * (ge0 + prior * (as0 - inv_sigma(as0)));
    if constexpr (ADAM) {
      float* sc = const_cast<float*>(a.scalars);
      auto upd = [&](int i, float g) {
        float m = ad.m_scal[i], v = ad.v_scal[i];
        sc[i] = adam_update(sc[i], g, m, v, ad);
        ad.m_scal[i] = m; ad.v_scal[i] = v;
      };
      if (a.lik == VFM_LIK_NORMAL) upd(0, ga);
      upd(1, gm);
      upd(2, gs);
    } else {
      b.g_scalars[0] = ga; b.g_scalars[1] = gm; b.g_scalars[2] = gs;
    }
  }

  const int64_t stride = (int64_t)gridDim.x * GPB;
  const int64_t xs = 4 + (((int64_t)d + 3) & ~(int64_t)3);
  const bool listed = b.row_ids != nullptr && (STAGE == STAGE_FULL ? ADAM != 0 : true);
  int nclamp = 0;
  const int n_occ = b.n_occ;
  const int Bm1 = a.B > 0 ? (int)a.B - 1 : 0;
  auto ent_ok = [&](int64_t v) -> int64_t {
    const bool ok = v >= 0 && v < a.T;
    nclamp += ok ? 0 : 1;
    return ok ? v : 0;
  };
  auto span_ok = [&](int2 v) -> int2 {
    const bool ok = v.x >= 0 && v.y >= v.x && v.y <= n_occ;
    nclamp += ok ? 0 : 1;
    return ok ? v : make_int2(0, 0);
  };
  auto row_ok = [&](int v) -> int {
    const bool ok = (unsigned)v <= (unsigned)Bm1;
    nclamp += ok ? 0 : 1;
    return ok ? v : 0;
  };
  const int64_t li_end = listed ? b.n_rows : a.e_hi;
  int64_t li = (listed ? 0 : a.e_lo) + (int64_t)blockIdx.x * GPB + tid / LPE;
  int64_t e_cur = li;
  if (listed && li < li_end) e_cur = ent_ok(b.row_ids[li]);
  int2 pq = make_int2(0, 0);
  if (STAGE != STAGE_APPLY && li < li_end) pq = span_ok(make_int2(b.occ_ptr[e_cur], b.occ_ptr[e_cur + 1]));
  for (; li < li_end; li += stride) {
    const int64_t e = listed ? e_cur : li;
    const int64_t rec = (listed && !b.rec_by_slot) ? e : li;
    int beg = pq.x, end = pq.y;
    const int64_t en = li + stride;
    float2 gc = make_float2(0.f, 0.f);
    if constexpr (STAGE == STAGE_APPLY) {
      gc = *reinterpret_cast<const float2*>(b.acc + (size_t)rec * xs);
      if (listed && en < li_end) e_cur = ent_ok(b.row_ids[en]);
      beg = 0; end = 0;
    } else {
      if (en < li_end) {
        const int64_t e_next = listed ? ent_ok(b.row_ids[en]) : en;
        e_cur = e_next;
        pq = span_ok(make_int2(b.occ_ptr[e_next], b.occ_ptr[e_next + 1]));
      }
    }
    bool in_next = false;
    if constexpr (PIPE) {
      if (b.zrec_next) in_next = b.next_occ_ptr[e + 1] != b.next_occ_ptr[e];
    }
    float* prow = const_cast<float*>(a.entity) + (size_t)e * (2 * (size_t)d);
    float* grow_e = (ADAM || STAGE == STAGE_ACC) ? nullptr : b.g_entity + (size_t)e * (2 * (size_t)d);
    const bool touched = (STAGE == STAGE_APPLY) ? gc.y > 0.f : beg != end;
    const float cntf = (STAGE == STAGE_APPLY) ? gc.y : (float)(end - beg);
    int la_gap = 0;
    if constexpr (LA) {
      if (!touched && b.next_occ_ptr[e + 1] == b.next_occ_ptr[e]) continue;
      la_gap = (la_step - 1) - b.last_step[e];
    }
    if (ADAM == 2 && !touched) continue;
    if (ADAM == 1 && STAGE == STAGE_FULL && a.row_filter == 2 && !touched) continue;

    Chunk<VEC> mu[CPL], s[CPL], ep[CPL], mm[CPL], ms[CPL], vm[CPL], vs[CPL];
    float2 th = make_float2(0.f, 1.f), mb = make_float2(0.f, 0.f), vb = make_float2(0.f, 0.f);
    float io = 0.f, epw = 0.f;
    if (STAGE != STAGE_ACC && (ADAM || touched)) {
#pragma unroll
      for (int i = 0; i < CPL; ++i) {
        const int j = lig + i * LPE;
        if (j < C) {
          mu[i] = ld_chunk<VEC>(prow + (size_t)j * VEC);
          s[i] = ld_chunk<VEC>(prow + d + (size_t)j * VEC);
          if constexpr (ADAM) {
            const size_t o = (size_t)e * (2 * (size_t)d) + (size_t)j * VEC;
            mm[i] = ld_chunk_nt<VEC>(ad.m_entity + o); ms[i] = ld_chunk_nt<VEC>(ad.m_entity + o + d);
            vm[i] = ld_chunk_nt<VEC>(ad.v_entity + o); vs[i] = ld_chunk_nt<VEC>(ad.v_entity + o + d);
          }
          if constexpr (EPS == EPS_TABLE)
            if (touched) ep[i] = ld_chunk<VEC>(a.eps_entity + (size_t)e * d + (size_t)j * VEC);
        }
      }
      if (lig == 0) {
        th = *reinterpret_cast<const float2*>(a.bias + 2 * (size_t)e);
        if constexpr (ADAM) {
          mb = *reinterpret_cast<const float2*>(ad.m_bias + 2 * (size_t)e);
          vb = *reinterpret_cast<const float2*>(ad.v_bias + 2 * (size_t)e);
        }
      }
      if (touched || (PIPE && in_next)) {
        io = a.inv_occ[e];
        if constexpr (EPS == EPS_TABLE) epw = a.eps_bias[e];
      }
    }

    int hslot = -1;
    if (STAGE != STAGE_APPLY && b.n_heavy > 0 && end - beg > VFM_HEAVY_MIN)
      hslot = heavy_slot_of(b.heavy_ids, b.n_heavy, (int)e);
    if (ADAM == 1 && STAGE == STAGE_FULL && a.row_filter == 4 && hslot >= 0) continue;
    auto walk = [&](const float* __restrict__ sz, const float* __restrict__ hacc, Chunk<VEC>(&A)[CPL], float& gs) {
#pragma unroll
      for (int i = 0; i < CPL; ++i)
#pragma unroll
        for (int t = 0; t < VEC; ++t) A[i].v[t] = 0.f;
      gs = 0.f;
      int o = beg;
      if (hslot >= 0) {
        const float* rec = hacc + (size_t)hslot * xs;
        int4 hd = *reinterpret_cast<const int4*>(rec);
        if (hd.z < 0 || hd.w < hd.z || hd.w > b.heavy_stride - b.n_heavy) { hd.z = hd.w = 0; ++nclamp; }
        if (hd.w - hd.z <= VFM_HEAVY_DIRECT) {
          for (int it = hd.z; it < hd.w; ++it) {
            const float* ir = hacc + ((size_t)b.n_heavy + (size_t)it) * xs;
            gs += ir[0];
#pragma unroll
            for (int i = 0; i < CPL; ++i) {
              const int j = lig + i * LPE;
              if (j < C) {
                const Chunk<VEC> t4 = ld_chunk<VEC>(ir + 4 + (size_t)j * VEC);
#pragma unroll
                for (int t = 0; t < VEC; ++t) A[i].v[t] += t4.v[t];
              }
            }
          }
        } else {
          gs = __int_as_float(hd.x);
#pragma unroll
          for (int i = 0; i < CPL; ++i) {
            const int j = lig + i * LPE;
            if (j < C) A[i] = ld_chunk<VEC>(rec + 4 + (size_t)j * VEC);
          }
        }
        o = end;
      }
      auto src = [&](int oo, int r) -> const float* {
        if constexpr (PIPE) return b.zrec + (size_t)ent_ok(b.occ_other[oo]) * xs + 4;
        return sz + (size_t)r * d;
      };
      for (; o + 1 < end; o += 2) {
        const int r0 = row_ok(b.occ_rows[o]), r1 = row_ok(b.occ_rows[o + 1]);
        const float g0 = b.grow[r0], g1 = b.grow[r1];
        const float* p0 = src(o, r0);
        const float* p1 = src(o + 1, r1);
        gs += g0 + g1;
#pragma unroll
        for (int i = 0; i < CPL; ++i) {
          const int j = lig + i * LPE;
          if (j < C) {
            const Chunk<VEC> s0v = ld_chunk<VEC>(p0 + (size_t)j * VEC);
            const Chunk<VEC> s1v = ld_chunk<VEC>(p1 + (size_t)j * VEC);
#pragma unroll
            for (int t = 0; t < VEC; ++t) A[i].v[t] = fmaf(g1, s1v.v[t], fmaf(g0, s0v.v[t], A[i].v[t]));
          }
        }
      }
      if (o < end) {
        const int r0 = row_ok(b.occ_rows[o]);
        const float g0 = b.grow[r0];
        const float* p0 = src(o, r0);
        gs += g0;
#pragma unroll
        for (int i = 0; i < CPL; ++i) {
          const int j = lig + i * LPE;
          if (j < C) {
            const Chunk<VEC> s0v = ld_chunk<VEC>(p0 + (size_t)j * VEC);
#pragma unroll
            for (int t = 0; t < VEC; ++t) A[i].v[t] = fmaf(g0, s0v.v[t], A[i].v[t]);
          }
        }
      }
    };
    Chunk<VEC> A[CPL];
    float gs;
    walk(b.sumz, b.heavy_acc, A, gs);

    if constexpr (STAGE == STAGE_ACC) {
#pragma unroll
      for (int i = 0; i < CPL; ++i) {
        const int j = lig + i * LPE;
        if (j < C) st_chunk<VEC>(b.acc + (size_t)rec * xs + 4 + (size_t)j * VEC, A[i]);
      }
      if (lig == 0) *reinterpret_cast<float4*>(b.acc + (size_t)rec * xs) = make_float4(gs, cntf, 0.f, 0.f);
      continue;
    }
    if constexpr (STAGE == STAGE_APPLY) {
      gs = gc.x;
      if (touched) {
#pragma unroll
        for (int i = 0; i < CPL; ++i) {
          const int j = lig + i * LPE;
          if (j < C) A[i] = ld_chunk<VEC>(b.acc + (size_t)rec * xs + 4 + (size_t)j * VEC);
        }
      }
    }

    if (!touched && !ADAM) {
      Chunk<VEC> zc;
#pragma unroll
      for (int t = 0; t < VEC; ++t) zc.v[t] = 0.f;
#pragma unroll
      for (int i = 0; i < CPL; ++i) {
        const int j = lig + i * LPE;
        if (j < C) {
          st_chunk_nt<VEC>(grow_e + (size_t)j * VEC, zc);
          st_chunk_nt<VEC>(grow_e + d + (size_t)j * VEC, zc);
        }
      }
      if (lig == 0) *reinterpret_cast<float2*>(b.g_bias + 2 * (size_t)e) = make_float2(0.f, 0.f);
      continue;
    }

    float c = 0.f;
    if (touched) {
      c = sh_cs[group_index(sh_hi, a.G, e)] * io * cntf;
    }
    float nb_eps = 0.f;
    float nb_next = 0.f, kl_next = 0.f, w_next = 0.f;
    constexpr bool multi = MULTI && STAGE == STAGE_FULL;
    Chunk<VEC> g1s[CPL], g2s[CPL];
    if (multi && touched) {
#pragma unroll
      for (int i = 0; i < CPL; ++i)
#pragma unroll
        for (int t = 0; t < VEC; ++t) { g1s[i].v[t] = 0.f; g2s[i].v[t] = 0.f; }
      for (int sm = 0; sm < a.S; ++sm) {
        if (sm > 0)
          walk(b.sumz + (size_t)sm * (size_t)a.B * d, b.heavy_acc + (size_t)sm * (size_t)b.heavy_stride * xs, A, gs);
        const RngKey ks = key_of_sample(key, sm);
#pragma unroll
        for (int i = 0; i < CPL; ++i) {
          const int j = lig + i * LPE;
          if (j < C) {
            Chunk<VEC> epc;
            if constexpr (EPS == EPS_TABLE) {
              epc = ld_chunk<VEC>(a.eps_entity + ((size_t)sm * (size_t)a.T + (size_t)e) * d + (size_t)j * VEC);
            } else if constexpr (EPS == EPS_ZERO) {
#pragma unroll
              for (int t = 0; t < VEC; ++t) epc.v[t] = 0.f;
            } else {
              float nb;
              eps_of_chunk<VEC>(ks, (uint32_t)e, j, epc.v, nb);
              if (i == 0) nb_eps += nb;
            }
#pragma unroll
            for (int t = 0; t < VEC; ++t) {
              const float z = fmaf(link_f<LINK>(s[i].v[t]), epc.v[t], mu[i].v[t]);
              const float gz = A[i].v[t] - z * gs;
              g1s[i].v[t] += gz;
              g2s[i].v[t] = fmaf(gz, epc.v[t], g2s[i].v[t]);
            }
          }
        }
        if constexpr (EPS == EPS_TABLE) nb_eps += a.eps_bias[(size_t)sm * (size_t)a.T + (size_t)e];
      }
      nb_eps *= a.inv_S;
#pragma unroll
      for (int i = 0; i < CPL; ++i)
#pragma unroll
        for (int t = 0; t < VEC; ++t) { g1s[i].v[t] *= a.inv_S; g2s[i].v[t] *= a.inv_S; }
    }
#pragma unroll
    for (int i = 0; i < CPL; ++i) {
      const int j = lig + i * LPE;
      if (j < C) {
        Chunk<VEC> gm, gv;
        if (touched && multi) {
#pragma unroll
          for (int t = 0; t < VEC; ++t) {
            const float sg = link_f<LINK>(s[i].v[t]);
            gm.v[t] = gout * (g1s[i].v[t] + c * mu[i].v[t]);
            gv.v[t] = gout * dlink_f<LINK>(s[i].v[t]) * (g2s[i].v[t] + c * (sg - inv_sigma(sg)));
          }
        } else if (touched) {
          Chunk<VEC> epc;
          if constexpr (EPS == EPS_TABLE) {
            epc = ep[i];
          } else if constexpr (EPS == EPS_ZERO) {
#pragma unroll
            for (int t = 0; t < VEC; ++t) epc.v[t] = 0.f;
          } else {
            float nb;
            eps_of_chunk<VEC>(key, (uint32_t)e, j, epc.v, nb);
            if (i == 0) nb_eps = nb;
          }
#pragma unroll
          for (int t = 0; t < VEC; ++t) {
            const float sg = link_f<LINK>(s[i].v[t]);
            const float z = fmaf(sg, epc.v[t], mu[i].v[t]);
            const float gz = PIPE ? A[i].v[t] : A[i].v[t] - z * gs;
            gm.v[t] = gout * (gz + c * mu[i].v[t]);
            gv.v[t] = gout * dlink_f<LINK>(s[i].v[t]) * (gz * epc.v[t] + c * (sg - inv_sigma(sg)));
          }
        } else {
#pragma unroll
          for (int t = 0; t < VEC; ++t) { gm.v[t] = 0.f; gv.v[t] = 0.f; }
        }
        if constexpr (LA) {
          if (la_gap > 0) {
            float rm[VEC], rs[VEC];
#pragma unroll
            for (int t = 0; t < VEC; ++t) { rm[t] = __builtin_amdgcn_sqrtf(vm[i].v[t]); rs[t] = __builtin_amdgcn_sqrtf(vs[i].v[t]); }
            for (int k = la_k - la_gap; k < la_k; ++k) {
              const float2 c = sh_tab[k];
#pragma unroll
              for (int t = 0; t < VEC; ++t) {
                mu[i].v[t] = replay_one(mu[i].v[t], mm[i].v[t], rm[t], c, ad.eps);
                s[i].v[t] = replay_one(s[i].v[t], ms[i].v[t], rs[t], c, ad.eps);
              }
            }
          }
        }
        if constexpr (ADAM) {
          Chunk<VEC> pm, ps;
#pragma unroll
          for (int t = 0; t < VEC; ++t) {
            pm.v[t] = adam_update(mu[i].v[t], gm.v[t], mm[i].v[t], vm[i].v[t], ad);
            ps.v[t] = adam_update(s[i].v[t], gv.v[t], ms[i].v[t], vs[i].v[t], ad);
          }
          const size_t o2 = (size_t)e * (2 * (size_t)d) + (size_t)j * VEC;
          st_chunk<VEC>(prow + (size_t)j * VEC, pm);
          st_chunk<VEC>(prow + d + (size_t)j * VEC, ps);
          if (!ad.scaled || touched || ad.store_true) {
            st_chunk_nt<VEC>(ad.m_entity + o2, mm[i]); st_chunk_nt<VEC>(ad.m_entity + o2 + d, ms[i]);
            st_chunk_nt<VEC>(ad.v_entity + o2, vm[i]); st_chunk_nt<VEC>(ad.v_entity + o2 + d, vs[i]);
          }
          if constexpr (PIPE) {
            if (in_next) {
              Chunk<VEC> ep2, zn;
              float nb2;
              eps_of_chunk<VEC>(next_key, (uint32_t)e, j, ep2.v, nb2);
              if (i == 0) nb_next = nb2;
#pragma unroll
              for (int t = 0; t < VEC; ++t) {
                const float sg2 = link_f<LINK>(ps.v[t]);
                zn.v[t] = fmaf(sg2, ep2.v[t], pm.v[t]);
                kl_next += kl_std_normal(pm.v[t], sg2);
              }
              st_chunk<VEC>(b.zrec_next + (size_t)e * xs + 4 + (size_t)j * VEC, zn);
            }
          }

        } else {
          st_chunk_nt<VEC>(grow_e + (size_t)j * VEC, gm);
          st_chunk_nt<VEC>(grow_e + d + (size_t)j * VEC, gv);
        }
      }
    }
    if (lig == 0) {
      float g0 = 0.f, g1 = 0.f;
      if (touched) {
        if constexpr (EPS == EPS_TABLE)
          if (!multi) nb_eps = epw;
        const float sg = link_f<LINK>(th.y);
        g0 = gout * (gs + c * th.x);
        g1 = gout * dlink_f<LINK>(th.y) * (gs * nb_eps + c * (sg - inv_sigma(sg)));
      }
      if constexpr (LA) {
        if (la_gap > 0) {
          const float r0 = __builtin_amdgcn_sqrtf(vb.x), r1 = __builtin_amdgcn_sqrtf(vb.y);
          for (int k = la_k - la_gap; k < la_k; ++k) {
            const float2 c = sh_tab[k];
            th.x = replay_one(th.x, mb.x, r0, c, ad.eps);
            th.y = replay_one(th.y, mb.y, r1, c, ad.eps);
          }
        }
        b.last_step[e] = la_step;
      }
      if constexpr (ADAM) {
        float2 pn;
        pn.x = adam_update(th.x, g0, mb.x, vb.x, ad);
        pn.y = adam_update(th.y, g1, mb.y, vb.y, ad);
        *reinterpret_cast<float2*>(const_cast<float*>(a.bias) + 2 * (size_t)e) = pn;
        if (a.wrec) *reinterpret_cast<float2*>(a.wrec + 4 * (size_t)e) = pn;
        if constexpr (PIPE) {
          if (in_next) {
            const float sgw2 = link_f<LINK>(pn.y);
            w_next = fmaf(sgw2, nb_next, pn.x);
            kl_next += kl_std_normal(pn.x, sgw2);
          }
        }
        if (!ad.scaled || touched || ad.store_true) {
          *reinterpret_cast<float2*>(ad.m_bias + 2 * (size_t)e) = mb;
          *reinterpret_cast<float2*>(ad.v_bias + 2 * (size_t)e) = vb;
        }
      } else {
        *reinterpret_cast<float2*>(b.g_bias + 2 * (size_t)e) = make_float2(g0, g1);
      }
    }
    if constexpr (PIPE) {
      if (in_next) {
        kl_next = group_sum<LPE>(kl_next);
        if (lig == 0)
          *reinterpret_cast<float4*>(b.zrec_next + (size_t)e * xs) =
              make_float4(w_next, kl_next * (sh_cs_next[group_index(sh_hi, a.G, e)] * io), 0.f, 0.f);
      }
    }
  }
  if (nclamp != 0 && b.status) atomicAdd(b.status, nclamp);
}
```

### vae_amd/csrc/vfm_fwd2.hpp

```cpp
#pragma once


template <int EPS>
struct EntRegs {
  uint32_t e;
  Chunk<4> mu[2], s[2], ep[2];
  float2 th;
  float io;
  float epw;
};

template <bool ID64>
struct RawIds {
  uint32_t ulo, uhi, ilo, ihi;
};
struct Ids {
  uint32_t u, i;
};
constexpr uint32_t BAD_ID = 0xFFFFFFFFu;

template <bool ID64>
__device__ __forceinline__ RawIds<ID64> load_row_ids(const KArgs& a, int r) {
  RawIds<ID64> v;
  if constexpr (ID64) {
    const uint4 t = reinterpret_cast<const uint4*>(a.x)[r];
    v.ulo = t.x; v.uhi = t.y; v.ilo = t.z; v.ihi = t.w;
  } else {
    const uint2 t = reinterpret_cast<const uint2*>(a.x)[r];
    v.ulo = t.x; v.uhi = 0u; v.ilo = t.y; v.ihi = 0u;
  }
  return v;
}

template <bool ID64>
__device__ __forceinline__ Ids fold_ids(const RawIds<ID64>& v, uint32_t T32) {
  Ids o;
  o.u = ((!ID64 || v.uhi == 0u) && v.ulo < T32) ? v.ulo : BAD_ID;
  o.i = ((!ID64 || v.ihi == 0u) && v.ilo < T32) ? v.ilo : BAD_ID;
  return o;
}

__device__ __forceinline__ uint32_t entity_of(uint32_t id, bool live, float& bad) {
  const bool ok = id != BAD_ID;
  bad += (live && !ok) ? 1.f : 0.f;
  return ok ? id : 0u;
}

template <int EPS, int MODE, bool WREC = false>
__device__ __forceinline__ void load_ent(const KArgs& a, uint32_t e, int off0, int off1, EntRegs<EPS>& R) {
  const size_t d = (size_t)a.d;
  R.e = e;
  if constexpr (EPS == EPS_ZREC) {
    const float* rec = a.entity + (size_t)e * (4 + d);
    R.mu[0] = ld_chunk<4>(rec + 4 + off0);
    R.mu[1] = ld_chunk<4>(rec + 4 + off1);
    const float4 h = *reinterpret_cast<const float4*>(rec);
    R.th = make_float2(h.x, 0.f);
    R.io = h.y;
    return;
  }
  const float* row = a.entity + (size_t)e * (2 * d);
  R.mu[0] = ld_chunk<4>(row + off0);
  R.mu[1] = ld_chunk<4>(row + off1);
  R.s[0] = ld_chunk<4>(row + d + off0);
  R.s[1] = ld_chunk<4>(row + d + off1);
  if constexpr (EPS == EPS_TABLE) {
    const float* er = a.eps_entity + (size_t)e * d;
    R.ep[0] = ld_chunk<4>(er + off0);
    R.ep[1] = ld_chunk<4>(er + off1);
    R.epw = a.eps_bias[e];
  }
  if constexpr (WREC) {
    const float4 h = *reinterpret_cast<const float4*>(a.wrec + 4 * (size_t)e);
    R.th = make_float2(h.x, h.y);
    R.io = h.z;
  } else {
    R.th = *reinterpret_cast<const float2*>(a.bias + 2 * (size_t)e);
    if constexpr (MODE == MODE_TRAIN) R.io = a.inv_occ[e];
  }
}

template <bool FULL, int EPS, int MODE, int LINK>
__device__ __forceinline__ void sample_ent(const RngKey& key, const EntRegs<EPS>& R, uint32_t pg, bool v0, bool v1,
                                           bool owns_bias, float cs, float (&z)[8], float& w, float& klw) {
  if constexpr (EPS == EPS_ZREC) {
#pragma unroll
    for (int t = 0; t < 4; ++t) {
      z[t] = (FULL || v0) ? R.mu[0].v[t] : 0.f;
      z[4 + t] = (FULL || v1) ? R.mu[1].v[t] : 0.f;
    }
    w = owns_bias ? R.th.x : 0.f;
    klw = (MODE == MODE_TRAIN && owns_bias) ? R.io : 0.f;
    return;
  }
  float ep[8], epw = 0.f;
  if constexpr (EPS == EPS_TABLE) {
#pragma unroll
    for (int t = 0; t < 4; ++t) { ep[t] = R.ep[0].v[t]; ep[4 + t] = R.ep[1].v[t]; }
    epw = R.epw;
  } else if constexpr (EPS == EPS_PHILOX) {
    normal8b(key, R.e, pg, ep, epw);
  } else {
#pragma unroll
    for (int t = 0; t < 8; ++t) ep[t] = 0.f;
  }
  float klv = 0.f;
#pragma unroll
  for (int c = 0; c < 2; ++c) {
    const bool valid = FULL || (c == 0 ? v0 : v1);
    v2f kq = {0.f, 0.f};
    float lg = 0.f;
#pragma unroll
    for (int h = 0; h < 2; ++h) {
      const v2f m2 = {R.mu[c].v[2 * h], R.mu[c].v[2 * h + 1]};
      const v2f g2 = {link_f<LINK>(R.s[c].v[2 * h]), link_f<LINK>(R.s[c].v[2 * h + 1])};
      const v2f e2 = {ep[4 * c + 2 * h], ep[4 * c + 2 * h + 1]};
      const v2f z2 = g2 * e2 + m2;
      z[4 * c + 2 * h] = valid ? z2.x : 0.f;
      z[4 * c + 2 * h + 1] = valid ? z2.y : 0.f;
      if constexpr (MODE == MODE_TRAIN) {
        kq = g2 * g2 + kq;
        kq = m2 * m2 + kq;
        lg += __builtin_amdgcn_logf(fmaxf(g2.x, SIGMA_MIN) * fmaxf(g2.y, SIGMA_MIN));
      }
    }
    if constexpr (MODE == MODE_TRAIN) klv += valid ? fmaf(0.5f, kq.x + kq.y, fmaf(-LN2, lg, -2.0f)) : 0.f;
  }
  const float sgw = link_f<LINK>(R.th.y);
  w = owns_bias ? fmaf(sgw, epw, R.th.x) : 0.f;
  klw = 0.f;
  if constexpr (MODE == MODE_TRAIN) {
    klv += owns_bias ? kl_std_normal(R.th.x, sgw) : 0.f;
    klw = klv * (cs * R.io);
  }
}

template <int LPE, bool FULL, int EPS, int MODE, bool ID64, int LINK, bool WREC = false>
__global__ __launch_bounds__(BLOCK, 4) void k_fwd2(const KArgs a, const FwdOut out) {
  constexpr int GPB = BLOCK / LPE;
  __shared__ float sh_cs[2];
  __shared__ int64_t sh_hi[2];
  __shared__ float sh_red[6 * 4];
  __shared__ float sh_e0;

  const int tid = threadIdx.x;
  const int lig = tid % LPE;
  const int C = a.d >> 2;
  const int NG = (int)gridDim.x * GPB;
  const int gid = (int)blockIdx.x * GPB + tid / LPE;
  const int q = (int)(a.B / NG), rem = (int)(a.B % NG);
  const int gbeg = gid * q + (gid < rem ? gid : rem);
  const int gend = gbeg + q + (gid < rem ? 1 : 0);
  const int glast = gend - 1;
  RawIds<ID64> raw0, raw1, raw2;
  float y_first = 0.f;
  if (gbeg < gend) {
    raw0 = load_row_ids<ID64>(a, gbeg);
    raw1 = load_row_ids<ID64>(a, gbeg + 1 < gend ? gbeg + 1 : glast);
    raw2 = load_row_ids<ID64>(a, gbeg + 2 < gend ? gbeg + 2 : glast);
    if constexpr (MODE == MODE_TRAIN) y_first = a.y[gbeg];
  }
  const RngKey key = key_of_step(a, blockIdx.x == 0 && tid == 0);

  if (MODE == MODE_TRAIN && EPS != EPS_ZREC && tid < 2) {
    sh_cs[tid] = (float)(a.group_n[tid] / a.W[tid]);
    sh_hi[tid] = a.group_hi[tid];
  }
  if constexpr (EPS == EPS_PHILOX || EPS == EPS_ZREC) {
    if (tid < 64) {
      float n[8], nb;
      normal8b(key, 0xFFFFFFFFu, 0u, n, nb);
      if (tid == 0) sh_e0 = n[0];
    }
  } else if (tid == 0) {
    sh_e0 = (EPS == EPS_TABLE) ? a.eps_global[0] : 0.f;
  }
  __syncthreads();
  const float alpha = a.scalars[0], m0 = a.scalars[1], s0 = a.scalars[2];
  const float aabs = link_f<LINK>(alpha);
  const float w0 = fmaf(link_f<LINK>(s0), sh_e0, m0);
  const float half_log_a = 0.5f * LN2 * __builtin_amdgcn_logf(aabs);
  const bool owns_bias = lig == 0;
  float cs0 = 0.f, cs1 = 0.f;
  uint32_t hi0 = 0u;
  if constexpr (MODE == MODE_TRAIN && EPS != EPS_ZREC) {
    cs0 = sh_cs[0]; cs1 = sh_cs[1];
    hi0 = sh_hi[0] > 0xFFFFFFFFLL ? 0xFFFFFFFFu : (uint32_t)sh_hi[0];
  }
  const uint32_t T32 = (uint32_t)a.T;

  const int j0 = 2 * lig, j1 = 2 * lig + 1;
  const bool v0 = j0 < C, v1 = j1 < C;
  const int off0 = 4 * (v0 ? j0 : C - 1), off1 = 4 * (v1 ? j1 : C - 1);
  const uint32_t pg = (uint32_t)lig + (key.chunk_off >> 1);

  float tot[6] = {0.f, 0.f, 0.f, 0.f, 0.f, 0.f};
  if (gbeg < gend) {
    int r0 = gbeg;
    Ids id0 = fold_ids<ID64>(raw0, T32);
    Ids id1 = fold_ids<ID64>(raw1, T32);
    RawIds<ID64> id2 = raw2;
    bool cur_item = true;
    EntRegs<EPS> A, Bq;
    load_ent<EPS, MODE, WREC>(a, entity_of(id0.i, true, tot[4]), off0, off1, A);
    float ycur = y_first;
    float zi[8], wi = 0.f, klwi = 0.f;
#pragma unroll
    for (int t = 0; t < 8; ++t) zi[t] = 0.f;

// ... 77 lines not shown
```

### vae_amd/csrc/vfm_heavy.hpp

```cpp
#pragma once

template <int LPE, int CPL, int VEC>
__global__ __launch_bounds__(BLOCK) void k_heavy(const int32_t* __restrict__ items, int n_items,
                                                 const int32_t* __restrict__ occ_rows,
                                                 const float* __restrict__ sumz, const float* __restrict__ grow,
                                                 float* __restrict__ item_acc, int d,
                                                 const int32_t* __restrict__ occ_other, const float* __restrict__ zrec,
                                                 float* __restrict__ heavy_acc, int n_heavy, int n_occ, int B, int64_t T,
                                                 int32_t* __restrict__ status) {
  constexpr int GPB = BLOCK / LPE;
  const int lig = threadIdx.x % LPE;
  const int C = (d + VEC - 1) / VEC;
  const int64_t xs = 4 + (((int64_t)d + 3) & ~(int64_t)3);
  int nclamp = 0;
  for (int it = blockIdx.x * GPB + threadIdx.x / LPE; it < n_items; it += gridDim.x * GPB) {
    int slot = items[4 * it], beg = items[4 * it + 1], end = items[4 * it + 2];
    if (slot < 0 || slot >= n_heavy || beg < 0 || end < beg || end > n_occ) { slot = 0; beg = end = 0; ++nclamp; }
    Chunk<VEC> A[CPL];
#pragma unroll
    for (int i = 0; i < CPL; ++i)
#pragma unroll
      for (int t = 0; t < VEC; ++t) A[i].v[t] = 0.f;
    float gs = 0.f;
    constexpr int W = 8 / CPL > 2 ? 8 / CPL : 2;
    int rn[W], on[W];
    auto load_idx = [&](int o0) {
#pragma unroll
      for (int u = 0; u < W; ++u) {
        const int oo = o0 + u < end ? o0 + u : beg;
        rn[u] = occ_rows[oo];
        on[u] = zrec ? occ_other[oo] : 0;
      }
    };
    if (beg < end) load_idx(beg);
    for (int o = beg; o < end; o += W) {
      int r[W]; float g[W];
      const float* src[W];
#pragma unroll
      for (int u = 0; u < W; ++u) {
        const bool ok = o + u < end;
        r[u] = rn[u];
        if ((unsigned)r[u] >= (unsigned)B) { r[u] = 0; ++nclamp; }
        g[u] = ok ? grow[r[u]] : 0.f;
        gs += g[u];
        int64_t oe = on[u];
        if (oe < 0 || oe >= T) { oe = 0; ++nclamp; }
        src[u] = zrec ? zrec + (size_t)oe * xs + 4 : sumz + (size_t)r[u] * d;
      }
      Chunk<VEC> sv0[W];
      const bool has0 = lig < C;
      if (has0) {
#pragma unroll
        for (int u = 0; u < W; ++u) sv0[u] = ld_chunk<VEC>(src[u] + (size_t)lig * VEC);
      }
      load_idx(o + W);
#pragma unroll
      for (int i = 0; i < CPL; ++i) {
        const int j = lig + i * LPE;
        if (j < C) {
          Chunk<VEC> sv[W];
#pragma unroll
          for (int u = 0; u < W; ++u) sv[u] = i == 0 ? sv0[u] : ld_chunk<VEC>(src[u] + (size_t)j * VEC);
#pragma unroll
          for (int u = 0; u < W; ++u)
#pragma unroll
            for (int t = 0; t < VEC; ++t) A[i].v[t] = fmaf(g[u], sv[u].v[t], A[i].v[t]);
        }
      }
    }
    if (lig == 0) {
      int* hdr = reinterpret_cast<int*>(heavy_acc + (size_t)slot * xs);
      if (it == 0 || items[4 * (it - 1)] != slot) hdr[2] = it;
      if (it + 1 == n_items || items[4 * (it + 1)] != slot) hdr[3] = it + 1;
    }
    float* rec = item_acc + (size_t)it * xs;
#pragma unroll
    for (int i = 0; i < CPL; ++i) {
      const int j = lig + i * LPE;
      if (j < C) st_chunk<VEC>(rec + 4 + (size_t)j * VEC, A[i]);
    }
    if (lig == 0) *reinterpret_cast<float4*>(rec) = make_float4(gs, (float)(end - beg), 0.f, 0.f);
  }
  if (nclamp != 0 && status) atomicAdd(status, nclamp);
}

template <int LPE, int CPL, int VEC>
__global__ __launch_bounds__(BLOCK) void k_heavy_sum(const int32_t* __restrict__ items, int n_items, int n_heavy,
                                                     const float* __restrict__ item_acc,
                                                     float* __restrict__ heavy_acc, int d) {
  (void)items;
  constexpr int GPB = BLOCK / LPE;
  __shared__ float sh[BLOCK * CPL * VEC + 2 * GPB];
  const int lig = threadIdx.x % LPE, grp = threadIdx.x / LPE;
  const int C = (d + VEC - 1) / VEC;
  const int64_t xs = 4 + (((int64_t)d + 3) & ~(int64_t)3);
  for (int slot = blockIdx.x; slot < n_heavy; slot += gridDim.x) {
    const int* hdr = reinterpret_cast<const int*>(heavy_acc + (size_t)slot * xs);
    int lo = hdr[2], end = hdr[3];
    if (lo < 0 || end < lo || end > n_items) lo = end = 0;
    if (end - lo <= VFM_HEAVY_DIRECT) continue;
    Chunk<VEC> A[CPL];
#pragma unroll
    for (int i = 0; i < CPL; ++i)
#pragma unroll
      for (int t = 0; t < VEC; ++t) A[i].v[t] = 0.f;
    float gs = 0.f, cnt = 0.f;
    for (int it = lo + grp; it < end; it += GPB) {
      const float* rec = item_acc + (size_t)it * xs;
      gs += rec[0]; cnt += rec[1];
#pragma unroll
      for (int i = 0; i < CPL; ++i) {
        const int j = lig + i * LPE;
        if (j < C) {
          const Chunk<VEC> t4 = ld_chunk<VEC>(rec + 4 + (size_t)j * VEC);
#pragma unroll
          for (int t = 0; t < VEC; ++t) A[i].v[t] += t4.v[t];
        }
      }
    }
    __syncthreads();
#pragma unroll
    for (int i = 0; i < CPL; ++i)
#pragma unroll
      for (int t = 0; t < VEC; ++t) sh[((grp * CPL + i) * VEC + t) * LPE + lig] = A[i].v[t];
    if (lig == 0) { sh[BLOCK * CPL * VEC + 2 * grp] = gs; sh[BLOCK * CPL * VEC + 2 * grp + 1] = cnt; }
    __syncthreads();
    if (grp == 0) {
      float* out = heavy_acc + (size_t)slot * xs;
#pragma unroll
      for (int i = 0; i < CPL; ++i) {
        const int j = lig + i * LPE;
        Chunk<VEC> tot;
#pragma unroll
        for (int t = 0; t < VEC; ++t) {
          float acc = 0.f;
          for (int g2 = 0; g2 < GPB; ++g2) acc += sh[((g2 * CPL + i) * VEC + t) * LPE + lig];
          tot.v[t] = acc;
        }
        if (j < C) st_chunk<VEC>(out + 4 + (size_t)j * VEC, tot);
      }
      if (lig == 0) {
        float tg = 0.f, tc = 0.f;
        for (int g2 = 0; g2 < GPB; ++g2) { tg += sh[BLOCK * CPL * VEC + 2 * g2]; tc += sh[BLOCK * CPL * VEC + 2 * g2 + 1]; }
        *reinterpret_cast<float2*>(out) = make_float2(tg, tc);
      }
    }
  }
}
```

### vae_amd/csrc/vfm_sample.hpp

```cpp
#pragma once

template <int LPE, int CPL, int VEC, int LINK>
__global__ __launch_bounds__(BLOCK) void k_sample_rec(const KArgs a, const int32_t* __restrict__ ids, int n,
                                                      float* __restrict__ zrec) {
  constexpr int GPB = BLOCK / LPE;
  __shared__ float sh_cs[VFM_MAX_FIELDS];
  __shared__ int64_t sh_hi[VFM_MAX_FIELDS];
  if ((int)threadIdx.x < a.G) {
    sh_cs[threadIdx.x] = (float)(a.group_n[threadIdx.x] / a.W[threadIdx.x]);
    sh_hi[threadIdx.x] = a.group_hi[threadIdx.x];
  }
  __syncthreads();
  const int lig = threadIdx.x % LPE;
  const int d = a.d;
  const int C = (d + VEC - 1) / VEC;
  const int64_t xs = 4 + (((int64_t)d + 3) & ~(int64_t)3);
  for (int i = blockIdx.x * GPB + threadIdx.x / LPE; i < n; i += gridDim.x * GPB) {
    const uint32_t e = (uint32_t)ids[i];
    const float* row = a.entity + (size_t)e * (2 * (size_t)d);
    float* rec = zrec + (size_t)e * xs;
    float epw = 0.f, klv = 0.f;
#pragma unroll
    for (int c = 0; c < CPL; ++c) {
      const int j = lig + c * LPE;
      if (j < C) {
        const Chunk<VEC> mu = ld_chunk<VEC>(row + (size_t)j * VEC);
        const Chunk<VEC> s = ld_chunk<VEC>(row + d + (size_t)j * VEC);
        Chunk<VEC> ep, z;
        float nb;
        eps_of_chunk<VEC>(a.key, e, j, ep.v, nb);
        if (c == 0) epw = nb;
#pragma unroll
        for (int t = 0; t < VEC; ++t) {
          const float sg = link_f<LINK>(s.v[t]);
          z.v[t] = fmaf(sg, ep.v[t], mu.v[t]);
          klv += kl_std_normal(mu.v[t], sg);
        }
        st_chunk<VEC>(rec + 4 + (size_t)j * VEC, z);
      }
    }
    const float2 th = *reinterpret_cast<const float2*>(a.bias + 2 * (size_t)e);
    const float sgw = link_f<LINK>(th.y);
    if (lig == 0) klv += kl_std_normal(th.x, sgw);
    klv = group_sum<LPE>(klv);
    if (lig == 0) {
      const float cs = sh_cs[group_index(sh_hi, a.G, (int64_t)e)];
      *reinterpret_cast<float4*>(rec) = make_float4(fmaf(sgw, epw, th.x), klv * (cs * a.inv_occ[e]), 0.f, 0.f);
    }
  }
}
```

### vae_amd/dist.py

```python
from __future__ import annotations

import torch
import torch.distributed as dist


def shard_rows(lo: int, hi: int, rank: int, world: int):
    n = hi - lo
    per = (n + world - 1) // world
    a = min(lo + rank * per, hi)
    return a, min(a + per, hi)


def sum_normalisers(W: torch.Tensor, group=None) -> torch.Tensor:
    if group is not None or (dist.is_initialized() and dist.get_world_size() > 1):
        dist.all_reduce(W, op=dist.ReduceOp.SUM, group=group)
    return W


def allreduce_flat(flat: torch.Tensor, group=None) -> torch.Tensor:
    dist.all_reduce(flat, op=dist.ReduceOp.SUM, group=group)
    return flat


def prior_terms_flag(rank: int) -> int:
# ... 35 lines not shown
            gids32 = plan.__dict__.get("_gids32")
            if gids32 is None or gids32.numel() != g.numel():
                gids32 = plan.__dict__["_gids32"] = g.to(torch.int32)
    t = model._adam_t + 1
    k = (t - 1) % ops.MOMENT_PERIOD + 1
    if k == 1:
        model._lazy_lr = {}
    model._lazy_lr[k] = float(lr)
    lazy = gids is not None and model.exchange_lazy and model._moments_scaled and eps is None
    mv, vv = model._views(model._adam_m), model._views(model._adam_v)
    if model._lazy_dirty and (not lazy or model._lazy_kind != "list"):
        model.sync_lazy(t - 1)
    listed = False
    if lazy:
        if model._lazy_last is None:
            model._lazy_last = torch.empty(T, dtype=torch.int32, device=model.device)
        if not model._lazy_dirty:
            model._lazy_last.fill_(t - 1)
        if k < ops.MOMENT_PERIOD:
            ops.adam_catchup(ent, bia, mv, vv, model._lazy_last, gids32, model._lazy_lrs(k - 1), upto=t - 1, mark=t, wrec=wrec)
            model._lazy_dirty, model._lazy_kind, listed = True, "list", True
        else:
            ops.adam_catchup(ent, bia, mv, vv, model._lazy_last, None, model._lazy_lrs(k - 1), upto=t - 1, mark=t, wrec=wrec)
            model._lazy_dirty = False
        mark("catchup")
    st = ops.elbo_forward(plan, ent, bia, scal, model.inv_occ, eps=eps, seed=model.rng_seed, step=step, train=True,
                          flags=prior_terms_flag(dist.get_rank(group)), out_pred=out_pred if out_pred is not None else pred,
                          out_sumz=sumz, out_grow=grow, out_partials=model._partials, wrec=wrec)
    mark("fwd")
    xacc, xs, xl, bounds = model._xviews()
    works = []
    nch = len(bounds) - 1
    if gids is not None:
        Ug = gids.numel()
        sb = plan.__dict__.get("_gid_bounds")
        if sb is None or sb[0] != tuple(bounds):
            sb = plan.__dict__["_gid_bounds"] = (tuple(bounds), torch.searchsorted(
                gids, torch.tensor(bounds, dtype=torch.int64, device=gids.device)).tolist())
        sb = sb[1]
        if model._xcompact is None:
            model._xcompact = torch.empty(n + 8, dtype=torch.float32, device=model.device)
        cbuf = model._xcompact
        tail = cbuf[Ug * rl: Ug * rl + 8]
        model._exchanged_floats = Ug * rl + 8
    if listed:
        nch = max(1, min(int(model.exchange_chunks), -(-Ug // 49152)))
        sb = [Ug * i // nch for i in range(nch + 1)]
        xs, xl = tail[0:2], tail[4:7]
        ops.elbo_finalize(st, scal, out=xl)
        mark("finalize")
        ops.elbo_backward_acc_rows(plan, st, gids32, cbuf, xs)
        for c in range(nch):
            end = Ug * rl + 8 if c == nch - 1 else sb[c + 1] * rl
            works.append(dist.all_reduce(cbuf[sb[c] * rl: end], group=group, async_op=True))
    else:
        ops.elbo_finalize(st, scal, out=xl)
        mark("finalize")
        if gids is None:
            for c in range(nch):
                lo, hi = bounds[c], bounds[c + 1]
                ops.elbo_backward_acc(plan, st, xacc, xs, lo, hi)
                end = model._xflat.numel() if hi == T else hi * rl
                works.append(dist.all_reduce(model._xflat[lo * rl: end], group=group, async_op=True))
            model._exchanged_floats = model._xflat.numel()
        else:
            dense = xacc.view(T, rl)
            ops.elbo_backward_acc(plan, st, xacc, xs, 0, T)
            torch.index_select(dense, 0, gids, out=cbuf[: Ug * rl].view(Ug, rl))
            tail.copy_(model._xflat[n: n + 8])
            for c in range(nch):
                end = Ug * rl + 8 if c == nch - 1 else sb[c + 1] * rl
                works.append(dist.all_reduce(cbuf[sb[c] * rl: end], group=group, async_op=True))
    mark("bwd_acc")
    model._adam_t = t
    for c in range(nch):
        works[c].wait()
        if listed:
            ops.elbo_apply_adam_rows(plan, st, cbuf[sb[c] * rl:], xs, gids32[sb[c]: sb[c + 1]], ent, bia, scal, model.inv_occ,
                                     mv, vv, lr, t, move_scalars=c == nch - 1, compact=True, wrec=wrec)
            continue
        if gids is not None:
            if sb[c + 1] > sb[c]:
                dense.index_copy_(0, gids[sb[c]: sb[c + 1]], cbuf[sb[c] * rl: sb[c + 1] * rl].view(-1, rl))
            if c == nch - 1:
                model._xflat[n: n + 8].copy_(tail)
        ops.elbo_apply_adam(plan, st, xacc, xs, ent, bia, scal, model.inv_occ, mv, vv, lr, t,
                            e_lo=bounds[c], e_hi=bounds[c + 1], scaled_moments=model._moments_scaled)
        model._wrec_ok = False
    mark("exchange_apply_adam")
    loss3.copy_(xl)
    return loss3, st.pred


def gather_shards(x: torch.Tensor, y: torch.Tensor, group):
    world, rank = dist.get_world_size(group), dist.get_rank(group)
    dev = x.device
    n = torch.zeros(world, dtype=torch.int64, device=dev)
    n[rank] = x.shape[0]
    dist.all_reduce(n, op=dist.ReduceOp.SUM, group=group)
    counts = [int(v) for v in n.tolist()]
    nmax = max(max(counts), 1)
    xp = torch.zeros(nmax, x.shape[1], dtype=x.dtype, device=dev)
    yp = torch.zeros(nmax, dtype=torch.float32, device=dev)
    xp[: x.shape[0]] = x
    yp[: x.shape[0]] = y
    xs = [torch.empty_like(xp) for _ in range(world)]
    ys = [torch.empty_like(yp) for _ in range(world)]
    dist.all_gather(xs, xp, group=group)
    dist.all_gather(ys, yp, group=group)
    X = torch.cat([t[:c] for t, c in zip(xs, counts)]).contiguous()
    Y = torch.cat([t[:c] for t, c in zip(ys, counts)]).contiguous()
    return X, Y, sum(counts[:rank])


def global_plan(plan, group, model):
    hit = plan.__dict__.get("_gplan")
    if hit is not None and hit[0] is group:
        return hit[1], hit[2]
    from . import ops
    X, Y, off = gather_shards(plan.x, plan.y, group)
    if X.shape[0] != plan.B_global:
        raise RuntimeError(f"the ranks' shards hold {X.shape[0]} rows, the plan says B_global = {plan.B_global}")
    gp = ops.BatchPlan(plan.spec, X, Y, model.inv_occ, B_global=plan.B_global)
    plan.__dict__["_gplan"] = (group, gp, off)
    return gp, off


def rows_supported(spec) -> bool:
    from . import ops
    return ops.pipeline_supported(spec)


def step_rows(model, plan, lr, step, group, mark=lambda name: None, next_plan=None):
    from . import ops
    ent, bia, scal = model._views(model._flat)
    loss3 = model._gflat[model._n_flat: model._n_flat + 3]
    gp, off = global_plan(plan, group, model)
    gnext = global_plan(next_plan, group, model)[0] if (next_plan is not None and next_plan.y is not None) else None
    Bg, B = gp.B, plan.B
    scaled = model.scaled_moments and not model.sparse_adam
    model._set_moment_form(scaled)
    model._adam_t += 1
    t = model._adam_t
    k = (t - 1) % ops.MOMENT_PERIOD + 1
    if k == 1:
        model._lazy_lr = {}
    model._lazy_lr[k] = float(lr)
    la = (gnext is not None and scaled and k < ops.MOMENT_PERIOD and model.pipeline_lookahead
          and model._lookahead_pays(gp, gnext))
    if model._lazy_dirty and not (la and model._lazy_kind == "la"):
        model.sync_lazy(t - 1)
        mark("catchup")
    if model._zrec is None:
        rl = ops.record_len(model.d)
        model._zrec = [torch.zeros(model.T, rl, dtype=torch.float32, device=model.device) for _ in range(2)]
    cur, nxt = model._zrec
    fresh = not model._records_ready(gp, step)
    mv, vv = model._views(model._adam_m), model._views(model._adam_v)
    if la:
        if model._lazy_last is None:
            model._lazy_last = torch.empty(model.T, dtype=torch.int32, device=model.device)
        if not model._lazy_dirty:
            model._lazy_last.fill_(t - 1)
        if model._la_tab is None:
            model._la_tab = torch.zeros(2 * (ops.MOMENT_PERIOD + 1), dtype=torch.float32, device=model.device)
        ready = model._la_ready_for
        if model._lazy_dirty and not (ready is not None and ready[0] is gp and ready[1] == t - 1):
            ops.adam_catchup(ent, bia, mv, vv, model._lazy_last, gp.touched_ids(), model._lazy_lrs(k - 1), upto=t - 1, mark=t - 1)
            mark("catchup")
            fresh = True
    bufs = model.__dict__.setdefault("_rows_bufs", {})
    hit = bufs.get(Bg)
    if hit is None:
        dev = model.device
        hit = bufs[Bg] = (torch.zeros(Bg + 8, dtype=torch.float64, device=dev),
                          torch.zeros(Bg, dtype=torch.float32, device=dev),
                          torch.zeros(_PARTIALS_LEN(), dtype=torch.float64, device=dev))
        hit[2][7] = 1.0
        if len(bufs) > 8:
            bufs.pop(next(iter(bufs)))
    xbuf, g_all, pg = hit
    if fresh:
        ops.sample_records(gp, ent, bia, model.inv_occ, cur, model.rng_seed, step)
        mark("sample_rec")
    _, grow, pred = model._step_buffers(B)
    if B > 0:
        st = ops.elbo_forward_records(plan, cur, scal, model.rng_seed, step, pred, grow, model._partials)
        ops.elbo_finalize(st, scal, out=model.__dict__.setdefault("_rows_loss", torch.zeros(3, dtype=torch.float32, device=model.device)))
    mark("fwd")
    xbuf.zero_()
    if B > 0:
        xbuf[off: off + B] = grow[:B]
        xbuf[Bg: Bg + 6] = model._partials[:6]
    dist.all_reduce(xbuf, op=dist.ReduceOp.SUM, group=group)
    model._exchanged_floats = 2 * int(xbuf.numel())
    g_all.copy_(xbuf[:Bg])
    pg[8:14] = xbuf[Bg: Bg + 6]
    mark("exchange")
    p = ops._problem(gp.spec, Bg, Bg, gp.id_bits, model.rng_seed, step, 0)
    stg = ops.FwdState(pred, pg, None, g_all, p, None)
    ops.elbo_backward_adam_pipe(gp, stg, cur, nxt if gnext is not None else None, gnext, step + 1, ent, bia, scal, model.inv_occ,
                                mv, vv, lr, t, loss3, scaled_moments=scaled,
                                last_step=model._lazy_last if la else None, step_tab=model._la_tab if la else None,
                                listed=model.lookahead_list, la_next=gnext if la else None)
    mark("bwd_adam")
    if gnext is not None:
        model._zrec = [nxt, cur]
        model._zrec_for = (gnext, step + 1, model._flat._version)
    else:
        model._zrec_for = None
    if la:
        model._lazy_dirty, model._lazy_kind = True, "la"
        model._la_ready_for = (gnext, t)
    return loss3, pred[:B]


def _PARTIALS_LEN():
    from . import _lib
    return _lib.PARTIALS_LEN
```

### vae_amd/model.py

```python
from __future__ import annotations

import math
from typing import Optional, Sequence

import numpy as np
import torch
from torch import nn

from . import _lib, ops
from .dist import shard_rows, allreduce_flat, prior_terms_flag


class LikelihoodResult:

    def __init__(self, pred: torch.Tensor, output: str, alpha: torch.Tensor, link: str = "abs"):
        self.logits = pred.reshape(1, -1) if pred.dim() == 1 else pred
        self.output = output
        self._alpha = alpha
        self._link = link

    @property
    def mean(self):
        return self.logits if self.output == "reg" else torch.sigmoid(self.logits)

# ... 424 lines not shown
        step = self.global_step
        self.global_step += 1
        mark = mark or (lambda name: None)
        mark("start")
        if fused is None:
            fused = self.fuse_adam
        fused = fused and adam and process_group is None
        wrec = self._wrec_for_step((fused or stats_step) and eps is None and self.n_samples == 1 and not self.sparse_adam)
        if fused:
            return self._step_fused(plan, next_plan, lr, step, eps, out_pred, mark, wrec)
        if process_group is not None and adam and self.exchange == "stats" and self.n_samples == 1:
            from .dist import step_stats
            return step_stats(self, plan, lr, step, process_group, eps, out_pred, mark, wrec)
        if process_group is not None and adam and self.exchange == "rows":
            from .dist import step_rows, rows_supported
            if not rows_supported(plan.spec) or eps is not None or out_pred is not None or self.sparse_adam:
                raise ValueError('exchange = "rows": two fields, one sample, d % 4 == 0, d <= 512, Philox eps, dense Adam')
            return step_rows(self, plan, lr, step, process_group, mark, next_plan=next_plan)
        if self._lazy_dirty:
            self.sync_lazy()
        return self._step_unfused(plan, lr, step, eps, out_pred, adam, mark, process_group)

    def _step_unfused(self, plan, lr, step, eps, out_pred, adam, mark, process_group=None):
        ent, bia, scal = self._views(self._flat)
        g_ent, g_bias, g_scal = self._views(self._gflat)
        loss3 = self._gflat[self._n_flat: self._n_flat + 3]
        rank = 0 if process_group is None else torch.distributed.get_rank(process_group)
        sumz, grow, pred = self._step_buffers(plan.B)
        st = ops.elbo_forward(plan, ent, bia, scal, self.inv_occ, eps=eps, seed=self.rng_seed, step=step,
                              train=True, flags=prior_terms_flag(rank), out_pred=out_pred if out_pred is not None else pred,
                              out_sumz=sumz, out_grow=grow, out_partials=self._partials)
        mark("fwd")
        self._set_moment_form(False)
        ops.elbo_finalize(st, scal, out=loss3)
        mark("finalize")
        ops.elbo_backward(plan, st, ent, bia, scal, self.inv_occ, self._gout, g_ent, g_bias, g_scal)
        mark("bwd")
        if process_group is not None:
            allreduce_flat(self._gflat, process_group)
            mark("allreduce")
        if adam:
            self._adam_t += 1
            ops.adam_step(self._flat, self._gflat, self._adam_m, self._adam_v, lr, self._adam_t)
            mark("adam")
        return loss3, st.pred

    def _step_fused(self, plan, next_plan, lr, step, eps, out_pred, mark, wrec):
        ent, bia, scal = self._views(self._flat)
        loss3 = self._gflat[self._n_flat: self._n_flat + 3]
        sumz, grow, pred = self._step_buffers(plan.B)
        flags = ops.FLAG_SHARE_GPU if getattr(self, "_sharing", False) else 0
        lazy = rows = None
        la = False
        scaled = self.scaled_moments and not self.sparse_adam
        self._set_moment_form(scaled)
        self._adam_t += 1
        k = (self._adam_t - 1) % ops.MOMENT_PERIOD + 1
        la = (scaled and k < ops.MOMENT_PERIOD and eps is None and self.n_samples == 1 and self.lazy_adam is not True
              and next_plan is not None and next_plan.y is not None and next_plan.spec.T == self.T
              and self._lookahead_pays(plan, next_plan))
        lazy = scaled and not la and self.n_samples >= 1 and self._use_lazy(plan)
        if k == 1:
            self._lazy_lr = {}
        self._lazy_lr[k] = float(lr)
        pipe_la = la and self.pipeline_lookahead
        if (self.pipeline and not lazy and (not self._lazy_dirty or self._lazy_kind == "la") and eps is None
                and not self.sparse_adam
                and out_pred is None and ops.pipeline_supported(plan.spec)
                and (self.pipeline is True or (self.d >= self.pipeline_min_d and self.T >= self.pipeline_min_T))):
            ready = self._records_ready(plan, step)
            nxt = next_plan
            if nxt is not None and self.pipeline == "auto" and (nxt.B < self.pipeline_ratio * nxt.U or (
                    nxt.U < self.pipeline_min_touch * self.T and not pipe_la)):
                nxt = None
            if ready or (nxt is not None and (self.pipeline is True or (plan.B >= self.pipeline_ratio * plan.U and (
                    plan.U >= self.pipeline_min_touch * self.T or pipe_la)))):
                if self._lazy_dirty and not pipe_la:
                    self.sync_lazy(self._adam_t - 1)
                    mark("catchup")
                return self._train_step_pipelined(plan, nxt, lr, step, scaled, mark, wrec,
                                                  la_next=next_plan if pipe_la else None)
        kind = "list" if lazy else ("la" if la else None)
        if self._lazy_dirty and kind != self._lazy_kind:
            self.sync_lazy(self._adam_t - 1)
        if kind is not None:
            if self._lazy_last is None:
                self._lazy_last = torch.empty(self.T, dtype=torch.int32, device=self.device)
            if not self._lazy_dirty:
                self._lazy_last.fill_(self._adam_t - 1)
            mv, vv = self._views(self._adam_m), self._views(self._adam_v)
            if lazy and k < ops.MOMENT_PERIOD:
                ops.adam_catchup(ent, bia, mv, vv, self._lazy_last, plan.touched_ids(), self._lazy_lrs(k - 1),
                                 upto=self._adam_t - 1, mark=self._adam_t, wrec=wrec)
                rows, self._lazy_dirty, self._lazy_kind = "touched", True, "list"
                mark("catchup")
            elif la:
                if self._la_tab is None:
                    self._la_tab = torch.zeros(2 * (ops.MOMENT_PERIOD + 1), dtype=torch.float32, device=self.device)
                ready = self._la_ready_for
                if self._lazy_dirty and not (ready is not None and ready[0] is plan and ready[1] == self._adam_t - 1):
                    ops.adam_catchup(ent, bia, mv, vv, self._lazy_last, plan.touched_ids(), self._lazy_lrs(k - 1),
                                     upto=self._adam_t - 1, mark=self._adam_t - 1, wrec=wrec)
                    mark("catchup")
            else:
                ops.adam_catchup(ent, bia, mv, vv, self._lazy_last, None, self._lazy_lrs(k - 1),
                                 upto=self._adam_t - 1, mark=self._adam_t, wrec=wrec)
                self._lazy_dirty = False
                mark("catchup")
        elif self._lazy_dirty:
            self.sync_lazy(self._adam_t - 1)

        st = ops.elbo_forward(plan, ent, bia, scal, self.inv_occ, eps=eps, seed=self.rng_seed, step=step,
                              train=True, flags=flags, out_pred=out_pred if out_pred is not None else pred,
                              out_sumz=sumz, out_grow=grow, out_partials=self._partials, wrec=wrec)
        mark("fwd")
        if la:
            ops.elbo_backward_adam_lookahead(plan, st, next_plan, ent, bia, scal, self.inv_occ,
                                             self._views(self._adam_m), self._views(self._adam_v), lr, self._adam_t,
                                             loss3, self._lazy_last, self._la_tab,
                                             listed=self.lookahead_list and not getattr(self, "_sharing", False), wrec=wrec)
        else:
            ops.elbo_backward_adam(plan, st, ent, bia, scal, self.inv_occ, self._views(self._adam_m),
                                   self._views(self._adam_v), lr, self._adam_t, loss_out=loss3,
                                   sparse=self.sparse_adam, scaled_moments=scaled, rows=rows, wrec=wrec)
        mark("bwd_adam")
        if la:
            self._lazy_dirty, self._lazy_kind = True, "la"
            self._la_ready_for = (next_plan, self._adam_t)
        return loss3, st.pred

    def _wrec_for_step(self, keep: bool):
        if not (keep and self.use_wrec and self.d % 4 == 0 and 16 <= self.d <= 512):
            self._wrec_ok = False
            return None
        _, bia, _ = self._views(self._flat)
        if self._wrec is None:
            self._wrec = torch.empty(self.T, 4, dtype=torch.float32, device=self.device)
            self._wrec_ok = False
        if not self._wrec_ok:
            ops.wrec_build(bia, self.inv_occ, self._wrec)
            self._wrec_ok = True
        elif _CHECK_WREC:
            assert torch.equal(self._wrec[:, :2], bia) and torch.equal(self._wrec[:, 2], self.inv_occ), "stale packed records"
        return self._wrec

    def _records_ready(self, plan, step) -> bool:
        f = self._zrec_for
        return f is not None and f[0] is plan and f[1] == step and f[2] == self._flat._version

    def _train_step_pipelined(self, plan, next_plan, lr, step, scaled, mark, wrec=None, la_next=None):
        ent, bia, scal = self._views(self._flat)
        loss3 = self._gflat[self._n_flat: self._n_flat + 3]
        if self._zrec is None:
            rl = ops.record_len(self.d)
            self._zrec = [torch.zeros(self.T, rl, dtype=torch.float32, device=self.device) for _ in range(2)]
        cur, nxt = self._zrec
        fresh = not self._records_ready(plan, step)
        la = la_next is not None
        if la:
            k = (self._adam_t - 1) % ops.MOMENT_PERIOD + 1
            if self._lazy_last is None:
                self._lazy_last = torch.empty(self.T, dtype=torch.int32, device=self.device)
            if not self._lazy_dirty:
                self._lazy_last.fill_(self._adam_t - 1)
            if self._la_tab is None:
                self._la_tab = torch.zeros(2 * (ops.MOMENT_PERIOD + 1), dtype=torch.float32, device=self.device)
            ready = self._la_ready_for
            if self._lazy_dirty and not (ready is not None and ready[0] is plan and ready[1] == self._adam_t - 1):
                ops.adam_catchup(ent, bia, self._views(self._adam_m), self._views(self._adam_v), self._lazy_last,
                                 plan.touched_ids(), self._lazy_lrs(k - 1), upto=self._adam_t - 1, mark=self._adam_t - 1,
                                 wrec=wrec)
                mark("catchup")
                fresh = True
        if fresh:
            ops.sample_records(plan, ent, bia, self.inv_occ, cur, self.rng_seed, step)
            mark("sample_rec")
        _, grow, pred = self._step_buffers(plan.B)
        if next_plan is not None and (next_plan.spec.T != self.T or next_plan.y is None):
            next_plan = None

        st = ops.elbo_forward_records(plan, cur, scal, self.rng_seed, step, pred, grow, self._partials,
                                      flags=ops.FLAG_SHARE_GPU if getattr(self, "_sharing", False) else 0)
        mark("fwd")
        ops.elbo_backward_adam_pipe(plan, st, cur, nxt, next_plan, step + 1, ent, bia, scal, self.inv_occ,
                                    self._views(self._adam_m), self._views(self._adam_v), lr, self._adam_t, loss3,
                                    scaled_moments=scaled, wrec=wrec,
                                    last_step=self._lazy_last if la else None, step_tab=self._la_tab if la else None,
                                    listed=self.lookahead_list and not getattr(self, "_sharing", False), la_next=la_next)
        mark("bwd_adam")
        out = st.pred
        if next_plan is not None:
            self._zrec = [nxt, cur]
            self._zrec_for = (next_plan, step + 1, self._flat._version)
        else:
            self._zrec_for = None
        if la:
            self._lazy_dirty, self._lazy_kind = True, "la"
            self._la_ready_for = (la_next, self._adam_t)
        return loss3, out

    def fit(self, X_train, y_train, n_epochs: int = 50, batch_size: int = 100000, X_test=None,
            y_test=None, display_every: int = 1, lr: Optional[float] = None, verbose: bool = True,
            process_group=None, sort_within_batch: bool = True, stream_plans: bool = False):
        X_train = torch.as_tensor(X_train)
        y_train = torch.as_tensor(y_train, dtype=torch.float32)
        nb_train = X_train.shape[0]
        self.set_training_data(X_train, nb_train)
        self.lr = lr if lr is not None else 1.0 / (1 + nb_train // batch_size)
        world = 1 if process_group is None else torch.distributed.get_world_size(process_group)
        rank = 0 if process_group is None else torch.distributed.get_rank(process_group)
        Xd = X_train.to(self.device)
        yd = y_train.to(self.device)
        if sort_within_batch:
            Xd, yd = sort_rows_within_batches(Xd, yd, batch_size)
        plans, spans = [], []
        stream_plans = bool(stream_plans) and world == 1
        for lo in range(0, nb_train, batch_size):
            hi = min(lo + batch_size, nb_train)
            a, b = shard_rows(lo, hi, rank, world)
            spans.append((a, b))
            if not stream_plans:
                plans.append(self.plan(Xd[a:b], yd[a:b], B_global=hi - lo, process_group=process_group,
                                       defer_readback=True))
        if stream_plans:
            return self._fit_streamed(Xd, yd, spans, n_epochs, X_test, y_test, display_every, verbose)
        if world == 1 and self.lookahead and self.lookahead_list and len(plans) > 1 and self.n_samples == 1:
            for i, plan in enumerate(plans):
                nxt = plans[(i + 1) % len(plans)]
                if self._lookahead_pays(plan, nxt) and (not self._will_pipeline(plan, nxt) or self.pipeline_lookahead):
                    plan.prepare_lookahead(nxt)
        train_pred = torch.zeros(nb_train, dtype=torch.float32, device=self.device)
        hist = {"epoch": [], "elbo": [], "train_rmse": [], "train_auc": [], "test": []}
        losses = torch.zeros(len(plans), dtype=torch.float32, device=self.device)
        for epoch in range(n_epochs):
            for i, (plan, (a, b)) in enumerate(zip(plans, spans)):
                if self.n_samples == 1:
                    nxt = plans[(i + 1) % len(plans)] if (world == 1 or self.exchange == "rows") else None
                    loss3, pr = self.train_step(plan, process_group=process_group, next_plan=nxt)
                    train_pred[a:b] = pr
                else:
                    loss3, pr = self.train_step(plan, process_group=process_group)
                    train_pred[a:b] = pr.mean(0)
                losses[i] = loss3[0]
            if epoch == 0 or epoch == n_epochs - 1:
                for plan in plans:
                    plan.check_status()
            if self.output == "reg":
                self.save_weights()
            if epoch % display_every == 0:
                rec = {"epoch": epoch, "elbo": float(losses.mean())}
                tp = train_pred
                if world > 1:
                    tp = train_pred.clone()
                    torch.distributed.all_reduce(tp, group=process_group)
                if self.output == "reg":
                    pr = tp.clamp(1, 5)
                    rec["train_rmse"] = float(torch.sqrt(torch.mean((pr - yd) ** 2)))
                else:
                    rec["train_auc"], rec["train_map"] = _auc_map(yd, torch.sigmoid(tp))
                if X_test is not None:
                    rec["test"] = self.evaluate(X_test, y_test)
                hist["epoch"].append(epoch)
                hist["elbo"].append(rec["elbo"])
                hist["train_rmse"].append(rec.get("train_rmse"))
                hist["train_auc"].append(rec.get("train_auc"))
                hist["test"].append(rec.get("test"))
                if verbose and rank == 0:
                    print(f"Epoch {epoch}: Elbo {rec['elbo']:.4f} " +
                          (f"Minibatch train RMSE {rec['train_rmse']:.4f}" if self.output == "reg" else
                           f"Minibatch train AUC {rec['train_auc']:.4f} Minibatch train MAP {rec['train_map']:.4f}"),
                          rec.get("test", ""))
        self.sync_lazy()
        return hist

    def _fit_streamed(self, Xd, yd, spans, n_epochs, X_test, y_test, display_every, verbose):
        nb, nb_train = len(spans), Xd.shape[0]
        train_pred = torch.zeros(nb_train, dtype=torch.float32, device=self.device)
        hist = {"epoch": [], "elbo": [], "train_rmse": [], "train_auc": [], "test": []}
        losses = torch.zeros(nb, dtype=torch.float32, device=self.device)
        total = n_epochs * nb
        batch = lambda t: (Xd[spans[t % nb][0]:spans[t % nb][1]], yd[spans[t % nb][0]:spans[t % nb][1]], False)
        D = max(2, int(self.plan_prefetch_depth))
        self.plan_streams().wait_current()
        q = [self.plan(*batch(0)[:2], defer_readback=True)] + [self.plan_async(*batch(k)[:2]) for k in range(1, min(D, total))]
        for t in range(total):
            epoch, i = divmod(t, nb)
            a, b = spans[i]
            nxt = q[1] if len(q) > 1 else None
            loss3, pr = self.train_step(q[0], next_plan=nxt if self.n_samples == 1 else None,
                                        prefetch=batch(t + D) if t + D < total else None)
            train_pred[a:b] = pr if self.n_samples == 1 else pr.mean(0)
            losses[i] = loss3[0]
            q.pop(0)
            if t + D < total:
                q.append(self.prefetched)
            if i == nb - 1:
                if self.output == "reg":
                    self.save_weights()
                if epoch % display_every == 0:
                    rec = {"epoch": epoch, "elbo": float(losses.mean())}
                    if self.output == "reg":
                        rec["train_rmse"] = float(torch.sqrt(torch.mean((train_pred.clamp(1, 5) - yd) ** 2)))
                    else:
                        rec["train_auc"], rec["train_map"] = _auc_map(yd, torch.sigmoid(train_pred))
                    if X_test is not None:
                        rec["test"] = self.evaluate(X_test, y_test)
                    for k in ("epoch", "elbo"):
                        hist[k].append(rec[k])
# ... 85 lines not shown
```

### vae_amd/ops.py

```python
from __future__ import annotations

import contextlib
import ctypes as C
from dataclasses import dataclass
from typing import Optional

import torch

from . import _lib
from ._lib import Problem, check, ptr, current_stream_ptr

FLAG_NO_PRIOR_TERMS = 1
FLAG_EPS_ZERO = 2
FLAG_SPARSE_ADAM = 4
FLAG_LINK_SOFTPLUS = 16
FLAG_SCALED_MOMENTS = 32
FLAG_ROWS_TOUCHED = 128
FLAG_SHARE_GPU = 2048
MOMENT_PERIOD = 128
MAX_SAMPLES = 64
_I63 = (1 << 63) - 1


@dataclass
class Spec:
    T: int
    F: int
    d: int
    group_hi: tuple
    group_n: tuple
    likelihood: int
    nb_train: int = 1
    n_samples: int = 1
    link: str = "abs"

    def __post_init__(self):
        if self.link not in ("abs", "softplus"):
            raise ValueError("link must be 'abs' or 'softplus'")
        if not 1 <= int(self.n_samples) <= MAX_SAMPLES:
            raise ValueError(f"n_samples must be in [1,{MAX_SAMPLES}]")

    @property
    def link_flag(self) -> int:
        return FLAG_LINK_SOFTPLUS if self.link == "softplus" else 0


def _problem(spec: Spec, B: int, B_global: int, id_bits: int, seed: int = 0, step: int = 0,
             flags: int = 0, wrec=None, dev_step=None) -> Problem:
    p = Problem()
    if wrec is not None:
        p.wrec = wrec.data_ptr()
    if dev_step is not None:
        p.dev_step = dev_step.data_ptr()
    p.B, p.B_global, p.T, p.nb_train = B, B_global, spec.T, spec.nb_train
    p.F, p.d, p.likelihood, p.id_bits = spec.F, spec.d, spec.likelihood, id_bits
    p.n_samples, p.flags = int(spec.n_samples), flags | spec.link_flag
    for g in range(spec.F):
        p.group_hi[g] = int(spec.group_hi[g])
        p.group_n[g] = float(spec.group_n[g])
    p.seed, p.step = seed & (2 ** 64 - 1), step & (2 ** 62 - 1)
    return p


def _need_cuda(t: torch.Tensor, name: str):
    if not t.is_cuda:
        raise _lib.VfmLibraryError(
            f"{name} is on {t.device}: vae_amd runs on an MI355X only (no CPU fallback)")
    if not t.is_contiguous():
        raise ValueError(f"{name} must be contiguous")


def inv_occ_from_counts(nb_occ: torch.Tensor) -> torch.Tensor:
    _need_cuda(nb_occ, "nb_occ")
    assert nb_occ.dtype == torch.int64
    out = torch.empty(nb_occ.numel(), dtype=torch.float32, device=nb_occ.device)
    lib = _lib.load()
    check(lib.vfm_inv_occ_f32(ptr(nb_occ), ptr(out), nb_occ.numel(), current_stream_ptr(nb_occ.device)),
          "vfm_inv_occ_f32")
    return out


_WS = {}
_ENQUEUE_LOCK = __import__("threading").RLock()


def _index_workspace(n_int32: int, dev, stream: int) -> torch.Tensor:
    key = (dev.index, stream)
    t = _WS.get(key)
    if t is None or t.numel() < n_int32:
        with torch.cuda.stream(_stream_obj(dev, stream)):
            t = _WS[key] = torch.empty(n_int32, dtype=torch.int32, device=dev)
    return t


_ARENAS = {}


def _side_arena(dev, stream, numel: int) -> torch.Tensor:
    key = (dev.index, stream.cuda_stream, numel)
    stash = _ARENAS.get(key)
    if not stash:
        if len(_ARENAS) > 8:
            _ARENAS.clear()
        with torch.cuda.stream(stream):
            stash = _ARENAS[key] = [torch.empty(numel, dtype=torch.int32, device=dev) for _ in range(8)]
    return stash.pop()


_STREAMS = {}


def _stream_obj(dev, raw: int):
    s = _STREAMS.get((dev.index, raw))
    if s is None:
        s = torch.cuda.current_stream(dev)
        if s.cuda_stream != raw:
            s = torch.cuda.ExternalStream(raw, device=dev)
        if len(_STREAMS) > 64:
            _STREAMS.clear()
        _STREAMS[(dev.index, raw)] = s
    return s


_SIZES = {}


def _index_sizes(B: int, F: int, T: int):
    hit = _SIZES.get((B, F, T))
    if hit is None:
        lib = _lib.load()
        hit = (_lib.heavy_list_for(B * F, T), int(lib.vfm_index_workspace_bytes(B, F, T)))
        if len(_SIZES) > 256:
            _SIZES.clear()
        _SIZES[(B, F, T)] = hit
    return hit


_PINNED = {"chunk": None, "used": 0}


def _pinned_ints(n: int) -> torch.Tensor:
    if _PINNED["chunk"] is None or _PINNED["used"] + n > _PINNED["chunk"].numel():
        _PINNED["chunk"] = torch.empty(max(1024, n), dtype=torch.int32, pin_memory=True)
        _PINNED["used"] = 0
    t = _PINNED["chunk"][_PINNED["used"]:_PINNED["used"] + n]
    _PINNED["used"] += n
    return t


def _carve(total_dev, sizes):
    out, off = [], 0
    for n in sizes:
        out.append(total_dev[off:off + n])
        off += (n + 3) & ~3
    return out


class BatchPlan:
# ... 234 lines not shown
            base = base + list(self.heavy)
        if with_touched:
            base = base + [self._touched]
        return base + [self._heavy_meta]


def _index_struct(plan: BatchPlan) -> "_lib.Index":
    if plan.occ_ptr is None:
        plan.build_index()
    plan._finish()
    ix = _lib.Index()
    ix.occ_ptr, ix.occ_rows, ix.status = plan.occ_ptr.data_ptr(), plan.occ_rows.data_ptr(), plan.status.data_ptr()
    ix.heavy_list, ix.heavy_threshold = plan.heavy_list, getattr(plan, "heavy_threshold", plan.heavy_list)
    if plan.heavy is not None:
        hid, items, acc = plan.heavy
        ix.heavy_ids, ix.heavy_items, ix.heavy_acc = hid.data_ptr(), items.data_ptr(), acc.data_ptr()
        ix.n_heavy, ix.n_items = hid.numel(), items.numel() // 4
        ix.max_items = plan.heavy_max_items
    return ix


class PlanStream:

    def __init__(self, device, n_streams: Optional[int] = None):
        import os
        self.device = torch.device(device)
        n = int(os.environ.get("VFM_PLAN_STREAMS", "2")) if n_streams is None else int(n_streams)
        prio = int(os.environ.get("VFM_PLAN_PRIORITY", "-1"))
        self.streams = [torch.cuda.Stream(self.device, priority=prio) for _ in range(max(1, n))]
        self._turn = 0

    @property
    def stream(self):
        return self.streams[self._turn % len(self.streams)]

    def wait_current(self):
        ev = torch.cuda.Event()
        ev.record(_stream_obj(self.device, _lib.raw_stream(self.device)))
        for st in self.streams:
            st.wait_event(ev)

    def build(self, make, pair_with: Optional[BatchPlan] = None, fork: bool = True) -> BatchPlan:
        self._turn += 1
        st = self.stream
        if fork:
            main = _stream_obj(self.device, _lib.raw_stream(self.device))
            ev0 = torch.cuda.Event()
            ev0.record(main)
            st.wait_event(ev0)
        plan = make(st)
        if pair_with is not None:
            if pair_with._ready is not None and pair_with._ready[1] is not st:
                st.wait_event(pair_with._ready[0])
            pair_with.prepare_lookahead(plan, stream=st)
        ev = torch.cuda.Event()
        ev.record(st)
        plan._ready = (ev, st)
        return plan


@dataclass
class FwdState:
    pred: torch.Tensor
    partials: torch.Tensor
    sumz: Optional[torch.Tensor]
    grow: Optional[torch.Tensor]
    problem: Problem
    eps: Optional[tuple]


def elbo_forward(plan: BatchPlan, entity_params, bias_params, scalars, inv_occ, *, eps=None,
                 seed=0, step=0, train=True, flags=0, out_pred=None, out_sumz=None,
                 out_grow=None, out_partials=None, wrec=None, dev_step=None) -> FwdState:
    spec = plan.spec
    dev = plan.x.device
    for t, n in ((entity_params, "entity_params"), (bias_params, "bias_params"), (scalars, "scalars")):
        _need_cuda(t, n)
    if entity_params.shape != (spec.T, 2 * spec.d) or bias_params.shape != (spec.T, 2):
        raise ValueError("table shapes do not match the spec")
    have_y = plan.y is not None
    train = train and have_y
    B, S = plan.B, int(spec.n_samples)
    pshape = (B,) if S == 1 else (S, B)
    pred = out_pred if out_pred is not None else torch.empty(pshape, dtype=torch.float32, device=dev)
    partials = out_partials if out_partials is not None else torch.empty(
        _lib.PARTIALS_LEN, dtype=torch.float64, device=dev)
    sumz = grow = None
    if train:
        sumz = out_sumz if out_sumz is not None else torch.empty(S * B, spec.d, dtype=torch.float32, device=dev)
        grow = out_grow if out_grow is not None else torch.empty(B, dtype=torch.float32, device=dev)
    p = _problem(spec, B, plan.B_global, plan.id_bits, seed, step, flags)
    e = eps if eps is not None else (None, None, None)
    _lib.ops().elbo_fwd(plan.x, plan.y, entity_params, bias_params, inv_occ if have_y else None, scalars,
                        plan.W if have_y else None, e[0], e[1], e[2], pred, partials, sumz, grow,
                        list(spec.group_hi), list(spec.group_n), spec.nb_train, plan.B_global,
                        spec.likelihood, p.flags, p.seed & _I63, p.step, S,
                        wrec if (train and eps is None) else None, dev_step)
    return FwdState(pred, partials, sumz, grow, p, eps)


def elbo_finalize(st: FwdState, scalars, out=None) -> torch.Tensor:
    loss = out if out is not None else torch.empty(3, dtype=torch.float32, device=scalars.device)
    p = st.problem
    _lib.ops().elbo_finalize(st.partials, scalars, loss, p.nb_train, p.B_global, p.flags, p.n_samples)
    return loss


def elbo_backward(plan: BatchPlan, st: FwdState, entity_params, bias_params, scalars, inv_occ,
                  grad_out, g_entity=None, g_bias=None, g_scalars=None):
    dev = plan.x.device
    if plan.occ_ptr is None:
        plan.build_index()
    if g_entity is None:
        g_entity = torch.empty_like(entity_params)
    if g_bias is None:
        g_bias = torch.empty_like(bias_params)
    if g_scalars is None:
        g_scalars = torch.empty(3, dtype=torch.float32, device=dev)
    e = st.eps if st.eps is not None else (None, None, None)
    p, spec = st.problem, plan.spec
    _lib.ops().elbo_bwd(plan.index_tensors(), entity_params, bias_params, inv_occ, scalars, plan.W,
                        e[0], e[1], e[2], st.sumz, st.grow, st.partials, grad_out, g_entity, g_bias, g_scalars,
                        spec.F, list(spec.group_hi), list(spec.group_n), p.nb_train, p.B_global, p.likelihood,
                        p.flags, p.seed & _I63, p.step, p.n_samples)
    return g_entity, g_bias, g_scalars


def elbo_backward_adam(plan: BatchPlan, st: FwdState, entity_params, bias_params, scalars, inv_occ,
                       m_views, v_views, lr, step, beta1=0.9, beta2=0.999, eps_adam=1e-8, loss_out=None,
                       sparse=False, scaled_moments=False, rows=None, wrec=None, dev_step=None):
    rows_flag = {None: 0, "touched": FLAG_ROWS_TOUCHED}[rows]
    if plan.occ_ptr is None:
        plan.build_index()
    e = st.eps if st.eps is not None else (None, None, None)
    p, spec = st.problem, plan.spec
    _lib.ops().elbo_bwd_adam(plan.index_tensors(with_touched=rows == "touched"), entity_params, bias_params, scalars,
                             inv_occ, plan.W,
                             e[0], e[1], e[2], st.sumz, st.grow, st.partials, m_views[0], v_views[0],
                             m_views[1], v_views[1], m_views[2], v_views[2], spec.F, list(spec.group_hi),
                             list(spec.group_n), p.nb_train, p.B_global, p.likelihood,
                             p.flags | (FLAG_SPARSE_ADAM if sparse else 0) |
                             (FLAG_SCALED_MOMENTS if scaled_moments else 0) | rows_flag,
                             p.seed & _I63, p.step, lr, beta1, beta2, eps_adam, int(step), loss_out, p.n_samples,
                             wrec, dev_step)


FLAG_ZREC = 1024


def record_len(d: int) -> int:
    return 4 + d


def pipeline_supported(spec: Spec) -> bool:
    return spec.F == 2 and int(spec.n_samples) == 1 and spec.d % 4 == 0 and spec.d <= 512 and spec.link == "abs"


def sample_records(plan: BatchPlan, entity_params, bias_params, inv_occ, zrec, seed, step):
    p = _problem(plan.spec, plan.B, plan.B_global, plan.id_bits, seed, step, 0)
    ids = plan.touched_ids()
    check(_lib.load().vfm_sample_records_f32(C.byref(p), ptr(ids), ids.numel(), ptr(entity_params), ptr(bias_params),
                                             ptr(inv_occ), ptr(plan.W), ptr(zrec), current_stream_ptr(zrec.device)),
          "vfm_sample_records_f32")


def elbo_forward_records(plan: BatchPlan, zrec, scalars, seed, step, out_pred, out_grow, out_partials, dev_step=None, flags=0) -> FwdState:
    spec = plan.spec
    p = _problem(spec, plan.B, plan.B_global, plan.id_bits, seed, step, FLAG_ZREC | flags, dev_step=dev_step)
    check(_lib.load().vfm_elbo_fwd_f32(C.byref(p), ptr(plan.x), ptr(plan.y), ptr(zrec), None, None, ptr(scalars), None,
                                       None, None, None, ptr(out_pred), ptr(out_partials), None, ptr(out_grow),
                                       current_stream_ptr(zrec.device)), "vfm_elbo_fwd_f32 (records)")
    p.flags = spec.link_flag | (flags & FLAG_SHARE_GPU)
    return FwdState(out_pred, out_partials, None, out_grow, p, None)


def elbo_backward_adam_pipe(plan: BatchPlan, st: FwdState, zrec, zrec_next, next_plan, next_step, entity_params,
                            bias_params, scalars, inv_occ, m_views, v_views, lr, step, loss_out, beta1=0.9, beta2=0.999,
                            eps_adam=1e-8, scaled_moments=True, wrec=None, dev_step=None, last_step=None, step_tab=None,
                            listed=True, la_next=None):
    ix = _index_struct(plan)
    ix.occ_other = plan.occ_other.data_ptr()
    pipe = _lib.Pipe()
    pipe.zrec = zrec.data_ptr()
    if next_plan is not None:
        if next_plan.occ_ptr is None:
            next_plan.build_index()
        pipe.zrec_next, pipe.next_occ_ptr, pipe.next_W = zrec_next.data_ptr(), next_plan.occ_ptr.data_ptr(), next_plan.W.data_ptr()
        pipe.next_step = int(next_step)
    if last_step is not None:
        if la_next.occ_ptr is None:
            la_next.build_index()
        pipe.last_step, pipe.step_tab = last_step.data_ptr(), step_tab.data_ptr()
        pipe.next_occ_ptr = la_next.occ_ptr.data_ptr()
        if next_plan is not None and next_plan is not la_next:
            raise ValueError("pipelined look-ahead step: the records are prepared for the batch the look-ahead names")
        if listed:
            rows = plan.lookahead_rows(la_next)
            if rows.numel() > 0:
                ix.touched_ids, ix.n_touched = rows.data_ptr(), rows.numel()
    p = st.problem
    p.flags = plan.spec.link_flag | (FLAG_SCALED_MOMENTS if scaled_moments else 0) | (p.flags & FLAG_SHARE_GPU)
    p.wrec = wrec.data_ptr() if wrec is not None else None
    p.dev_step = dev_step.data_ptr() if dev_step is not None else None
    check(_lib.load().vfm_elbo_bwd_adam_pipe_f32(
        C.byref(p), C.byref(ix), C.byref(pipe), ptr(entity_params), ptr(bias_params), ptr(scalars), ptr(inv_occ),
        ptr(plan.W), ptr(st.grow), ptr(st.partials), ptr(m_views[0]), ptr(v_views[0]), ptr(m_views[1]), ptr(v_views[1]),
        ptr(m_views[2]), ptr(v_views[2]), lr, beta1, beta2, eps_adam, int(step), ptr(loss_out),
        current_stream_ptr(zrec.device)), "vfm_elbo_bwd_adam_pipe_f32")


def elbo_backward_adam_lookahead(plan: BatchPlan, st: FwdState, next_plan: BatchPlan, entity_params, bias_params,
                                 scalars, inv_occ, m_views, v_views, lr, step, loss_out, last_step, step_tab,
                                 beta1=0.9, beta2=0.999, eps_adam=1e-8, listed=True, wrec=None, dev_step=None):
    ix = _index_struct(plan)
    if listed:
        rows = plan.lookahead_rows(next_plan)
        if rows.numel() > 0:
            ix.touched_ids, ix.n_touched = rows.data_ptr(), rows.numel()
    if next_plan.occ_ptr is None:
        next_plan.build_index()
    p = st.problem
    share = p.flags & FLAG_SHARE_GPU
    p.flags = plan.spec.link_flag | FLAG_SCALED_MOMENTS | share
    p.wrec = wrec.data_ptr() if wrec is not None else None
    p.dev_step = dev_step.data_ptr() if dev_step is not None else None
    check(_lib.load().vfm_elbo_bwd_adam_lookahead_f32(
        C.byref(p), C.byref(ix), ptr(entity_params), ptr(bias_params), ptr(scalars), ptr(inv_occ), ptr(plan.W),
        ptr(st.sumz), ptr(st.grow), ptr(st.partials), ptr(m_views[0]), ptr(v_views[0]), ptr(m_views[1]), ptr(v_views[1]),
        ptr(m_views[2]), ptr(v_views[2]), lr, beta1, beta2, eps_adam, int(step), ptr(loss_out), ptr(last_step),
        ptr(next_plan.occ_ptr), ptr(step_tab), current_stream_ptr(entity_params.device)),
        "vfm_elbo_bwd_adam_lookahead_f32")
    p.flags = plan.spec.link_flag | share


def adam_catchup(entity_params, bias_params, m_views, v_views, last_step, ids, lr_of_step, upto, mark,
                 beta1=0.9, beta2=0.999, eps_adam=1e-8, wrec=None):
    T, d = entity_params.shape[0], entity_params.shape[1] // 2
    n = T if ids is None else ids.numel()
    need = (int(upto) - 1) % MOMENT_PERIOD + 1 if upto > 0 else 0
    vals = [float(v) for v in lr_of_step] + [0.0] * max(0, need - len(lr_of_step))
    lrs = (C.c_float * max(len(vals), 1))(*vals)
    check(_lib.load().vfm_adam_catchup_f32(ptr(entity_params), ptr(bias_params), ptr(m_views[0]), ptr(v_views[0]),
                                           ptr(m_views[1]), ptr(v_views[1]), ptr(last_step), ptr(ids), n, T, d, lrs,
                                           len(vals), beta1, beta2, eps_adam, int(upto), int(mark), ptr(wrec),
                                           current_stream_ptr(entity_params.device)), "vfm_adam_catchup_f32")


def wrec_build(bias_params, inv_occ, wrec):
    check(_lib.load().vfm_wrec_build_f32(ptr(bias_params), ptr(inv_occ), bias_params.shape[0], ptr(wrec),
                                         current_stream_ptr(wrec.device)), "vfm_wrec_build_f32")


class StepState:
    WINDOW = 4096

    def __init__(self, device):
        self.dev = torch.zeros(8, dtype=torch.int64, device=device)
        self.tab = torch.zeros(self.WINDOW, 16, dtype=torch.float32, device=device)
        self.first, self.length, self.key = 0, 0, None
        self.counters = None

    def cover(self, adam_step: int, lr: float, beta1: float, beta2: float, eps: float, scaled: bool):
        key = (float(lr), float(beta1), float(beta2), float(eps), bool(scaled))
        if key == self.key and self.first <= adam_step < self.first + self.length:
            return
        lib = _lib.load()
        host = (_lib.StepConsts * self.WINDOW)()
        for i in range(self.WINDOW):
            check(lib.vfm_step_consts(key[0], key[1], key[2], key[3], adam_step + i, int(scaled), C.byref(host[i])),
                  "vfm_step_consts")
        raw = torch.frombuffer(bytearray(bytes(host)), dtype=torch.float32).view(self.WINDOW, 16)
        self.tab.copy_(raw)
        hdr = _lib.DevStep()
        hdr.tab_first, hdr.tab_len, hdr.tab = adam_step, self.WINDOW, self.tab.data_ptr()
        hdr.error = int(self.dev[7].item())
        self.dev.copy_(torch.frombuffer(bytearray(bytes(hdr)), dtype=torch.int64))
        self.first, self.length, self.key, self.counters = adam_step, self.WINDOW, key, None

    def set(self, philox_step: int, adam_step: int):
        if self.counters != (philox_step, adam_step):
            check(_lib.load().vfm_dev_step_set(ptr(self.dev), int(philox_step), int(adam_step),
                                               current_stream_ptr(self.dev.device)), "vfm_dev_step_set")
            self.counters = (philox_step, adam_step)

    def advanced(self):
        self.counters = (self.counters[0] + 1, self.counters[1] + 1)

    def error(self) -> bool:
        return bool(int(self.dev[7].item()))


def exchange_record_len(d: int) -> int:
    return 4 + (d + 3) // 4 * 4


def elbo_backward_acc(plan: BatchPlan, st: FwdState, acc, sums, e_lo=0, e_hi=0):
    if plan.occ_ptr is None:
        plan.build_index()
    spec = plan.spec
    _lib.ops().elbo_bwd_acc(plan.index_tensors(), st.sumz, st.grow, st.partials, acc, sums,
                            spec.T, spec.F, spec.d, e_lo, e_hi)


def elbo_apply_adam(plan: BatchPlan, st: FwdState, acc, sums, entity_params, bias_params, scalars,
                    inv_occ, m_views, v_views, lr, step, beta1=0.9, beta2=0.999, eps_adam=1e-8, e_lo=0, e_hi=0,
                    scaled_moments=False):
    e = st.eps if st.eps is not None else (None, None, None)
    p, spec = st.problem, plan.spec
    _lib.ops().elbo_apply_adam(acc, sums, entity_params, bias_params, scalars, inv_occ, plan.W,
                               e[0], e[1], e[2], m_views[0], v_views[0], m_views[1], v_views[1], m_views[2],
                               v_views[2], spec.F, list(spec.group_hi), list(spec.group_n), p.nb_train,
                               p.B_global, p.likelihood,
                               (p.flags & ~FLAG_NO_PRIOR_TERMS) | (FLAG_SCALED_MOMENTS if scaled_moments else 0),
                               p.seed & _I63, p.step,
                               lr, beta1, beta2, eps_adam, int(step), e_lo, e_hi)


def elbo_backward_acc_rows(plan: BatchPlan, st: FwdState, row_ids, acc, sums):
    ix = _index_struct(plan)
    spec = plan.spec
    p = _problem(spec, plan.B, plan.B, 64)
    check(_lib.load().vfm_elbo_bwd_acc_rows_f32(C.byref(p), C.byref(ix), ptr(row_ids), row_ids.numel(), ptr(st.sumz),
                                                ptr(st.grow), ptr(st.partials), ptr(acc), ptr(sums),
                                                current_stream_ptr(acc.device)), "vfm_elbo_bwd_acc_rows_f32")


def elbo_apply_adam_rows(plan: BatchPlan, st: FwdState, acc, sums, row_ids, entity_params, bias_params, scalars, inv_occ,
                         m_views, v_views, lr, step, move_scalars: bool, compact: bool = False, beta1=0.9, beta2=0.999,
                         eps_adam=1e-8, wrec=None):
    p0, spec = st.problem, plan.spec
    p = _problem(spec, 0, p0.B_global, 64, p0.seed, p0.step, (p0.flags & ~FLAG_NO_PRIOR_TERMS) | FLAG_SCALED_MOMENTS, wrec=wrec)
    p.e_lo, p.e_hi = 0, (0 if move_scalars else 1)
    check(_lib.load().vfm_elbo_apply_adam_rows_f32(
        C.byref(p), ptr(acc), ptr(sums), ptr(row_ids), row_ids.numel(), int(bool(compact)), ptr(entity_params), ptr(bias_params),
        ptr(scalars),
        ptr(inv_occ), ptr(plan.W), ptr(m_views[0]), ptr(v_views[0]), ptr(m_views[1]), ptr(v_views[1]), ptr(m_views[2]),
        ptr(v_views[2]), lr, beta1, beta2, eps_adam, int(step), current_stream_ptr(entity_params.device)),
        "vfm_elbo_apply_adam_rows_f32")


def moments_rescale(m, v, step, to_scaled, beta1=0.9, beta2=0.999):
    _lib.ops().moments_rescale(m, v, beta1, beta2, int(step), bool(to_scaled))


def adam_step(p, g, m, v, lr, step, beta1=0.9, beta2=0.999, eps=1e-8):
    for t in (p, g, m, v):
        _need_cuda(t, "adam tensor")
    _lib.ops().adam(p, g, m, v, lr, beta1, beta2, eps, int(step))


def philox_eps(spec: Spec, seed: int, step: int, device):
    S = int(spec.n_samples)
    lead = () if S == 1 else (S,)
    ee = torch.empty(*lead, spec.T, spec.d, dtype=torch.float32, device=device)
    eb = torch.empty(*lead, spec.T, dtype=torch.float32, device=device)
    eg = torch.empty(S, dtype=torch.float32, device=device)
    p = _problem(spec, 0, 0, 64, seed, step)
    lib = _lib.load()
    check(lib.vfm_philox_eps_f32(C.byref(p), ptr(ee), ptr(eb), ptr(eg), current_stream_ptr(ee.device)),
          "vfm_philox_eps_f32")
    return ee, eb, eg
# ... 25 lines not shown
```

Before: 516.6 million.

## Split sample records into aligned z table and separate header table

Record tables previously interleaved a 4-float header with the d-float latent sample, giving a row stride of 4+d. The z samples now live in their own table with rows padded to a multiple of 32 floats, and the (w, kl) header goes to a separate T x 4 table. Forward, backward, heavy-item and sampling kernels take the strides as parameters. The aim is cache-line-aligned, coalesced loads of z rows in the gather-heavy kernels, at the cost of an extra header access per entity, padding memory, and more plumbing across the ABI.

```diff
diff --git a/include/vfm_hip.h b/include/vfm_hip.h
--- a/include/vfm_hip.h
+++ b/include/vfm_hip.h
@@ -82,6 +82,9 @@
   int64_t e_lo, e_hi;
   vfm_dev_step_t* dev_step;
   float* wrec;
+  float* zrec_hdr;
+  int64_t zrec_stride;
+  int64_t zrec_hdr_stride;
 } vfm_problem_t;
 int vfm_wrec_build_f32(const float* bias_params, const float* inv_occ, int64_t T, float* wrec, void* stream);
 
@@ -182,6 +185,7 @@
   uint64_t next_step;
   int32_t* last_step;
   float* step_tab;
+  float* zrec_next_hdr;
 } vfm_pipe_t;
 int vfm_sample_records_f32(const vfm_problem_t* p, const int32_t* ids, int64_t n, const float* entity_params,
                            const float* bias_params, const float* inv_occ, const double* W, float* zrec, void* stream);
diff --git a/vae_amd/_abi_gen.py b/vae_amd/_abi_gen.py
--- a/vae_amd/_abi_gen.py
+++ b/vae_amd/_abi_gen.py
@@ -90,6 +90,9 @@
         ("e_hi", C.c_int64),
         ("dev_step", C.c_void_p),
         ("wrec", C.c_void_p),
+        ("zrec_hdr", C.c_void_p),
+        ("zrec_stride", C.c_int64),
+        ("zrec_hdr_stride", C.c_int64),
     ]
 
     def __init__(self, *a, **k):
@@ -133,6 +136,7 @@
         ("next_step", C.c_uint64),
         ("last_step", C.c_void_p),
         ("step_tab", C.c_void_p),
+        ("zrec_next_hdr", C.c_void_p),
     ]
 
     def __init__(self, *a, **k):
diff --git a/vae_amd/csrc/vfm_abi.hip b/vae_amd/csrc/vfm_abi.hip
--- a/vae_amd/csrc/vfm_abi.hip
+++ b/vae_amd/csrc/vfm_abi.hip
@@ -127,6 +127,19 @@
   return a;
 }
 
+int rec_layout(const vfm_problem_t* p, const float* table, const float* hdr, const float** z, const float** h, int64_t* zs,
+               int64_t* hs, const char* who) {
+  if (!p->zrec_hdr) {
+    *z = table ? table + 4 : nullptr; *h = table; *zs = *hs = 4 + (int64_t)p->d;
+    return 0;
+  }
+  const bool ok = p->zrec_stride >= p->d && (p->zrec_stride & 3) == 0 && p->zrec_hdr_stride >= 4 &&
+                  (p->zrec_hdr_stride & 3) == 0 && ((uintptr_t)table & 15) == 0 && ((uintptr_t)hdr & 15) == 0;
+  if (!ok) return fail(VFM_E_INVALID, who);
+  *z = table; *h = hdr; *zs = p->zrec_stride; *hs = p->zrec_hdr_stride;
+  return 0;
+}
+
 bool use_fwd2(const vfm_problem_t* p, int eps, bool multi = false) {
   if (p->F != 2 || (p->d & 3) != 0 || p->d > 512) return false;
   if (multi ? (p->n_samples < 2 || p->n_samples > 4 || eps == EPS_ZERO) : p->n_samples != 1) return false;
@@ -169,14 +182,14 @@
 
 template <int LPE, int CPL, int VEC>
 int launch_heavy_t(const vfm_problem_t* p, const vfm_index_t* idx, const float* sumz, const float* grow, float* hacc, int d,
-                   hipStream_t st, const float* zrec = nullptr) {
+                   hipStream_t st, const float* zrec = nullptr, int64_t zs = 0) {
   constexpr int GPB = BLOCK / LPE;
   const size_t xs = 4 + (((size_t)d + 3) & ~(size_t)3);
   float* item_acc = hacc + xs * (size_t)idx->n_heavy;
   int64_t nb = ((int64_t)idx->n_items + GPB - 1) / GPB;
   if (nb > 4096) nb = 4096;
   hipLaunchKernelGGL((k_heavy<LPE, CPL, VEC>), dim3((unsigned)nb), dim3(BLOCK), 0, st, idx->heavy_items,
-                     (int)idx->n_items, idx->occ_rows, sumz, grow, item_acc, d, zrec ? idx->occ_other : nullptr, zrec, hacc,
+                     (int)idx->n_items, idx->occ_rows, sumz, grow, item_acc, d, zrec ? idx->occ_other : nullptr, zrec, zs, hacc,
                      (int)idx->n_heavy, (int)(p->B * (int64_t)p->F), (int)p->B, p->T, idx->status);
   if (idx->max_items > 0 && idx->max_items <= VFM_HEAVY_DIRECT) return 0;
   nb = idx->n_heavy;
@@ -187,7 +200,7 @@
 }
 
 int run_heavy(const vfm_problem_t* p, const vfm_index_t* idx, const float* sumz, const float* grow,
-              hipStream_t st, BwdArgs* b, const float* zrec = nullptr) {
+              hipStream_t st, BwdArgs* b, const float* zrec = nullptr, int64_t zs = 0) {
   b->heavy_ids = nullptr; b->heavy_acc = nullptr; b->n_heavy = 0; b->heavy_stride = 0;
   if (idx->n_heavy <= 0 || idx->n_items <= 0) return 0;
   if (!idx->heavy_ids || !idx->heavy_items || !idx->heavy_acc)
@@ -202,7 +215,7 @@
     const float* sz = sumz ? sumz + (size_t)sm * (size_t)p->B * (size_t)p->d : nullptr;
     float* hacc = idx->heavy_acc + (size_t)sm * per_sample;
 #define X(L_, C_, V_) \
-    if (s.lpe == L_ && s.cpl == C_ && s.vec == V_) launch_heavy_t<L_, C_, V_>(p, idx, sz, grow, hacc, p->d, st, zrec);
+    if (s.lpe == L_ && s.cpl == C_ && s.vec == V_) launch_heavy_t<L_, C_, V_>(p, idx, sz, grow, hacc, p->d, st, zrec, zs);
     VFM_FOR_SHAPES(X)
 #undef X
   }
@@ -399,7 +412,12 @@
     if (!use_fwd2(p, EPS_ZREC)) return fail(VFM_E_UNSUPPORTED, "VFM_FLAG_ZREC: two fields, one sample, d % 4 == 0, d <= 512, |.| link");
     if (!x || !y || !entity_params || !scalars || !pred || !grow || eps_entity || eps_bias || eps_global)
       return fail(VFM_E_INVALID, "vfm_elbo_fwd_f32 (VFM_FLAG_ZREC): x, y, the record table, scalars, pred, grow; no eps tables");
+    const float* z;
     KArgs a = make_args(p, x, y, entity_params, nullptr, nullptr, scalars, nullptr, nullptr, nullptr, nullptr, 0);
+    if (int rc = rec_layout(p, entity_params, p->zrec_hdr, &z, &a.zhdr, &a.zs, &a.hs,
+                            "vfm_elbo_fwd_f32 (VFM_FLAG_ZREC): record strides multiples of 4 (zrec_stride >= d), tables 16-byte aligned"))
+      return rc;
+    a.entity = z;
     FwdOut o{pred, partials, nullptr, grow};
     if (int rc = launch_fwd2_abs(EPS_ZREC, MODE_TRAIN, a, o, (hipStream_t)stream)) return rc;
     return after_launch("vfm_elbo_fwd_f32");
@@ -667,9 +685,14 @@
     return fail(VFM_E_INVALID, "vfm_sample_records_f32: bad argument");
   if (n == 0) return 0;
   KArgs a = make_args(p, nullptr, nullptr, entity_params, bias_params, inv_occ, nullptr, W, nullptr, nullptr, nullptr);
+  const float *z, *h;
+  if (int rc = rec_layout(p, zrec, p->zrec_hdr, &z, &h, &a.zs, &a.hs,
+                          "vfm_sample_records_f32: record strides multiples of 4 (zrec_stride >= d), tables 16-byte aligned"))
+    return rc;
   Shape s;
   pick_shape(p->d, &s);
-  if (int rc = launch_sample_rec_abs(s, a, ids, (int)n, zrec, (hipStream_t)stream)) return rc;
+  if (int rc = launch_sample_rec_abs(s, a, ids, (int)n, const_cast<float*>(z), const_cast<float*>(h), (hipStream_t)stream))
+    return rc;
   return after_launch("vfm_sample_records_f32");
 }
 
@@ -705,9 +728,19 @@
   KArgs a = make_args(p, nullptr, nullptr, entity_params, bias_params, inv_occ, scalars, W, nullptr, nullptr, nullptr);
   BwdArgs b = bwd_args(p, idx);
   b.grow = grow; b.partials = partials; b.loss = loss;
-  if (int rc = run_heavy(p, idx, nullptr, grow, (hipStream_t)stream, &b, pipe->zrec)) return rc;
-  b.zrec = pipe->zrec; b.occ_other = idx->occ_other;
-  b.zrec_next = pipe->zrec_next; b.next_occ_ptr = pipe->next_occ_ptr; b.next_W = pipe->next_W;
+  const float *z, *h, *zn = nullptr, *hn = nullptr;
+  int64_t zs, hs;
+  const char* bad_layout = "vfm_elbo_bwd_adam_pipe_f32: record strides multiples of 4 (zrec_stride >= d), tables 16-byte "
+                           "aligned, a header table for each record table (vfm_problem_t.zrec_hdr, vfm_pipe_t.zrec_next_hdr)";
+  if (int rc = rec_layout(p, pipe->zrec, p->zrec_hdr, &z, &h, &zs, &hs, bad_layout)) return rc;
+  if (pipe->zrec_next) {
+    if (p->zrec_hdr ? !pipe->zrec_next_hdr : pipe->zrec_next_hdr != nullptr) return fail(VFM_E_INVALID, bad_layout);
+    if (int rc = rec_layout(p, pipe->zrec_next, pipe->zrec_next_hdr, &zn, &hn, &zs, &hs, bad_layout)) return rc;
+  }
+  if (int rc = run_heavy(p, idx, nullptr, grow, (hipStream_t)stream, &b, z, zs)) return rc;
+  b.zrec = z; b.occ_other = idx->occ_other; b.zrec_zs = zs; b.zrec_hs = hs;
+  b.zrec_next = const_cast<float*>(zn); b.zrec_next_hdr = const_cast<float*>(hn);
+  b.next_occ_ptr = pipe->next_occ_ptr; b.next_W = pipe->next_W;
   b.next_key = a.key;
   b.next_key.step_lo = (uint32_t)pipe->next_step; b.next_key.step_hi = (uint32_t)(pipe->next_step >> 32);
   if (pipe->last_step) {
diff --git a/vae_amd/csrc/vfm_args.hpp b/vae_amd/csrc/vfm_args.hpp
--- a/vae_amd/csrc/vfm_args.hpp
+++ b/vae_amd/csrc/vfm_args.hpp
@@ -42,6 +42,8 @@
   float* wrec;
   int64_t group_hi[VFM_MAX_FIELDS];
   double group_n[VFM_MAX_FIELDS];
+  const float* zhdr;
+  int64_t zs, hs;
 };
 
 struct FwdOut {
@@ -73,6 +75,8 @@
   const float* zrec;
   const int32_t* occ_other;
   float* zrec_next;
+  float* zrec_next_hdr;
+  int64_t zrec_zs, zrec_hs;
   const int32_t* next_occ_ptr;
   const double* next_W;
   RngKey next_key;
@@ -153,7 +157,8 @@
 VFM_INTERNAL int launch_fwd2_abs(int eps, int mode, KArgs& a, const FwdOut& o, hipStream_t st);
 VFM_INTERNAL int launch_fwd2m_abs(int eps, int mode, KArgs& a, const FwdOut& o, hipStream_t st);
 VFM_INTERNAL int launch_fwdg_abs(int eps, int mode, KArgs& a, const FwdOut& o, hipStream_t st);
-VFM_INTERNAL int launch_sample_rec_abs(const Shape& s, KArgs& a, const int32_t* ids, int n, float* zrec, hipStream_t st);
+VFM_INTERNAL int launch_sample_rec_abs(const Shape& s, KArgs& a, const int32_t* ids, int n, float* z, float* hdr,
+                                      hipStream_t st);
 
 #define VFM_FOR_SHAPES(X)                                                                      \
   X(4, 1, 4) X(8, 1, 4) X(16, 1, 4) X(32, 1, 4) X(64, 1, 4) X(64, 2, 4) \
diff --git a/vae_amd/csrc/vfm_bwd.hip b/vae_amd/csrc/vfm_bwd.hip
--- a/vae_amd/csrc/vfm_bwd.hip
+++ b/vae_amd/csrc/vfm_bwd.hip
@@ -90,13 +90,13 @@
 }
 
 #if VFM_BWD_PART == 1 && VFM_LINK == 0
-int dispatch_sample_rec(const Shape& s, KArgs& a, const int32_t* ids, int n, float* zrec, hipStream_t st) {
+int dispatch_sample_rec(const Shape& s, KArgs& a, const int32_t* ids, int n, float* zrec, float* zhdr, hipStream_t st) {
 #define X(L_, C_, V_)                                                                                   \
   if (s.lpe == L_ && s.cpl == C_ && s.vec == V_) {                                                      \
     constexpr int GPB = BLOCK / L_;                                                                     \
     int64_t nb = ((int64_t)n + GPB - 1) / GPB;                                                          \
     if (nb > 65535) nb = 65535;                                                                         \
-    hipLaunchKernelGGL((k_sample_rec<L_, C_, V_, LINK>), dim3((unsigned)nb), dim3(BLOCK), 0, st, a, ids, n, zrec); \
+    hipLaunchKernelGGL((k_sample_rec<L_, C_, V_, LINK>), dim3((unsigned)nb), dim3(BLOCK), 0, st, a, ids, n, zrec, zhdr); \
     return 0;                                                                                           \
   }
   VFM_FOR_SHAPES(X)
@@ -109,8 +109,8 @@
 }
 
 #if VFM_BWD_PART == 1 && VFM_LINK == 0
-int launch_sample_rec_abs(const Shape& s, KArgs& a, const int32_t* ids, int n, float* zrec, hipStream_t st) {
-  return dispatch_sample_rec(s, a, ids, n, zrec, st);
+int launch_sample_rec_abs(const Shape& s, KArgs& a, const int32_t* ids, int n, float* z, float* hdr, hipStream_t st) {
+  return dispatch_sample_rec(s, a, ids, n, z, hdr, st);
 }
 #endif
 
diff --git a/vae_amd/csrc/vfm_bwd.hpp b/vae_amd/csrc/vfm_bwd.hpp
--- a/vae_amd/csrc/vfm_bwd.hpp
+++ b/vae_amd/csrc/vfm_bwd.hpp
@@ -240,7 +240,7 @@
         o = end;
       }
       auto src = [&](int oo, int r) -> const float* {
-        if constexpr (PIPE) return b.zrec + (size_t)ent_ok(b.occ_other[oo]) * xs + 4;
+        if constexpr (PIPE) return b.zrec + (size_t)ent_ok(b.occ_other[oo]) * (size_t)b.zrec_zs;
         return sz + (size_t)r * d;
       };
       for (; o + 1 < end; o += 2) {
@@ -442,7 +442,7 @@
                 zn.v[t] = fmaf(sg2, ep2.v[t], pm.v[t]);
                 kl_next += kl_std_normal(pm.v[t], sg2);
               }
-              st_chunk<VEC>(b.zrec_next + (size_t)e * xs + 4 + (size_t)j * VEC, zn);
+              st_chunk<VEC>(b.zrec_next + (size_t)e * (size_t)b.zrec_zs + (size_t)j * VEC, zn);
             }
           }
 
@@ -497,7 +497,7 @@
       if (in_next) {
         kl_next = group_sum<LPE>(kl_next);
         if (lig == 0)
-          *reinterpret_cast<float4*>(b.zrec_next + (size_t)e * xs) =
+          *reinterpret_cast<float4*>(b.zrec_next_hdr + (size_t)e * (size_t)b.zrec_hs) =
               make_float4(w_next, kl_next * (sh_cs_next[group_index(sh_hi, a.G, e)] * io), 0.f, 0.f);
       }
     }
diff --git a/vae_amd/csrc/vfm_fwd2.hpp b/vae_amd/csrc/vfm_fwd2.hpp
--- a/vae_amd/csrc/vfm_fwd2.hpp
+++ b/vae_amd/csrc/vfm_fwd2.hpp
@@ -51,10 +51,10 @@
   const size_t d = (size_t)a.d;
   R.e = e;
   if constexpr (EPS == EPS_ZREC) {
-    const float* rec = a.entity + (size_t)e * (4 + d);
-    R.mu[0] = ld_chunk<4>(rec + 4 + off0);
-    R.mu[1] = ld_chunk<4>(rec + 4 + off1);
-    const float4 h = *reinterpret_cast<const float4*>(rec);
+    const float* zr = a.entity + (size_t)e * (size_t)a.zs;
+    R.mu[0] = ld_chunk<4>(zr + off0);
+    R.mu[1] = ld_chunk<4>(zr + off1);
+    const float4 h = *reinterpret_cast<const float4*>(a.zhdr + (size_t)e * (size_t)a.hs);
     R.th = make_float2(h.x, 0.f);
     R.io = h.y;
     return;
diff --git a/vae_amd/csrc/vfm_heavy.hpp b/vae_amd/csrc/vfm_heavy.hpp
--- a/vae_amd/csrc/vfm_heavy.hpp
+++ b/vae_amd/csrc/vfm_heavy.hpp
@@ -5,7 +5,7 @@
                                                  const int32_t* __restrict__ occ_rows,
                                                  const float* __restrict__ sumz, const float* __restrict__ grow,
                                                  float* __restrict__ item_acc, int d,
-                                                 const int32_t* __restrict__ occ_other, const float* __restrict__ zrec,
+                                                 const int32_t* __restrict__ occ_other, const float* __restrict__ zrec, int64_t zs,
                                                  float* __restrict__ heavy_acc, int n_heavy, int n_occ, int B, int64_t T,
                                                  int32_t* __restrict__ status) {
   constexpr int GPB = BLOCK / LPE;
@@ -45,7 +45,7 @@
         gs += g[u];
         int64_t oe = on[u];
         if (oe < 0 || oe >= T) { oe = 0; ++nclamp; }
-        src[u] = zrec ? zrec + (size_t)oe * xs + 4 : sumz + (size_t)r[u] * d;
+        src[u] = zrec ? zrec + (size_t)oe * zs : sumz + (size_t)r[u] * d;
       }
       Chunk<VEC> sv0[W];
       const bool has0 = lig < C;
diff --git a/vae_amd/csrc/vfm_sample.hpp b/vae_amd/csrc/vfm_sample.hpp
--- a/vae_amd/csrc/vfm_sample.hpp
+++ b/vae_amd/csrc/vfm_sample.hpp
@@ -2,7 +2,7 @@
 
 template <int LPE, int CPL, int VEC, int LINK>
 __global__ __launch_bounds__(BLOCK) void k_sample_rec(const KArgs a, const int32_t* __restrict__ ids, int n,
-                                                      float* __restrict__ zrec) {
+                                                      float* __restrict__ zrec, float* __restrict__ zhdr) {
   constexpr int GPB = BLOCK / LPE;
   __shared__ float sh_cs[VFM_MAX_FIELDS];
   __shared__ int64_t sh_hi[VFM_MAX_FIELDS];
@@ -14,11 +14,10 @@
   const int lig = threadIdx.x % LPE;
   const int d = a.d;
   const int C = (d + VEC - 1) / VEC;
-  const int64_t xs = 4 + (((int64_t)d + 3) & ~(int64_t)3);
   for (int i = blockIdx.x * GPB + threadIdx.x / LPE; i < n; i += gridDim.x * GPB) {
     const uint32_t e = (uint32_t)ids[i];
     const float* row = a.entity + (size_t)e * (2 * (size_t)d);
-    float* rec = zrec + (size_t)e * xs;
+    float* rec = zrec + (size_t)e * (size_t)a.zs;
     float epw = 0.f, klv = 0.f;
 #pragma unroll
     for (int c = 0; c < CPL; ++c) {
@@ -36,7 +35,7 @@
           z.v[t] = fmaf(sg, ep.v[t], mu.v[t]);
           klv += kl_std_normal(mu.v[t], sg);
         }
-        st_chunk<VEC>(rec + 4 + (size_t)j * VEC, z);
+        st_chunk<VEC>(rec + (size_t)j * VEC, z);
       }
     }
     const float2 th = *reinterpret_cast<const float2*>(a.bias + 2 * (size_t)e);
@@ -45,7 +44,7 @@
     klv = group_sum<LPE>(klv);
     if (lig == 0) {
       const float cs = sh_cs[group_index(sh_hi, a.G, (int64_t)e)];
-      *reinterpret_cast<float4*>(rec) = make_float4(fmaf(sgw, epw, th.x), klv * (cs * a.inv_occ[e]), 0.f, 0.f);
+      *reinterpret_cast<float4*>(zhdr + (size_t)e * (size_t)a.hs) = make_float4(fmaf(sgw, epw, th.x), klv * (cs * a.inv_occ[e]), 0.f, 0.f);
     }
   }
 }
diff --git a/vae_amd/dist.py b/vae_amd/dist.py
--- a/vae_amd/dist.py
+++ b/vae_amd/dist.py
@@ -211,8 +211,7 @@
         model.sync_lazy(t - 1)
         mark("catchup")
     if model._zrec is None:
-        rl = ops.record_len(model.d)
-        model._zrec = [torch.zeros(model.T, rl, dtype=torch.float32, device=model.device) for _ in range(2)]
+        model._zrec = [ops.new_records(model.T, model.d, model.device) for _ in range(2)]
     cur, nxt = model._zrec
     fresh = not model._records_ready(gp, step)
     mv, vv = model._views(model._adam_m), model._views(model._adam_v)
diff --git a/vae_amd/model.py b/vae_amd/model.py
--- a/vae_amd/model.py
+++ b/vae_amd/model.py
@@ -600,8 +600,7 @@
         ent, bia, scal = self._views(self._flat)
         loss3 = self._gflat[self._n_flat: self._n_flat + 3]
         if self._zrec is None:
-            rl = ops.record_len(self.d)
-            self._zrec = [torch.zeros(self.T, rl, dtype=torch.float32, device=self.device) for _ in range(2)]
+            self._zrec = [ops.new_records(self.T, self.d, self.device) for _ in range(2)]
         cur, nxt = self._zrec
         fresh = not self._records_ready(plan, step)
         la = la_next is not None
diff --git a/vae_amd/ops.py b/vae_amd/ops.py
--- a/vae_amd/ops.py
+++ b/vae_amd/ops.py
@@ -3,7 +3,7 @@
 import contextlib
 import ctypes as C
 from dataclasses import dataclass
-from typing import Optional
+from typing import NamedTuple, Optional
 
 import torch
 
@@ -544,6 +544,28 @@
     return 4 + d
 
 
+def record_stride(d: int) -> int:
+    return (d + 31) // 32 * 32
+
+
+class Records(NamedTuple):
+    z: torch.Tensor
+    hdr: torch.Tensor
+
+
+def new_records(T: int, d: int, device) -> Records:
+    return Records(torch.zeros(T, record_stride(d), dtype=torch.float32, device=device),
+                   torch.zeros(T, 4, dtype=torch.float32, device=device))
+
+
+def _rec_layout(p: Problem, zrec):
+    if isinstance(zrec, Records):
+        p.zrec_hdr, p.zrec_stride, p.zrec_hdr_stride = zrec.hdr.data_ptr(), zrec.z.stride(0), zrec.hdr.stride(0)
+        return zrec.z
+    p.zrec_hdr, p.zrec_stride, p.zrec_hdr_stride = None, 0, 0
+    return zrec
+
+
 def pipeline_supported(spec: Spec) -> bool:
     return spec.F == 2 and int(spec.n_samples) == 1 and spec.d % 4 == 0 and spec.d <= 512 and spec.link == "abs"
 
@@ -551,17 +573,19 @@
 def sample_records(plan: BatchPlan, entity_params, bias_params, inv_occ, zrec, seed, step):
     p = _problem(plan.spec, plan.B, plan.B_global, plan.id_bits, seed, step, 0)
     ids = plan.touched_ids()
+    z = _rec_layout(p, zrec)
     check(_lib.load().vfm_sample_records_f32(C.byref(p), ptr(ids), ids.numel(), ptr(entity_params), ptr(bias_params),
-                                             ptr(inv_occ), ptr(plan.W), ptr(zrec), current_stream_ptr(zrec.device)),
+                                             ptr(inv_occ), ptr(plan.W), ptr(z), current_stream_ptr(z.device)),
           "vfm_sample_records_f32")
 
 
 def elbo_forward_records(plan: BatchPlan, zrec, scalars, seed, step, out_pred, out_grow, out_partials, dev_step=None, flags=0) -> FwdState:
     spec = plan.spec
     p = _problem(spec, plan.B, plan.B_global, plan.id_bits, seed, step, FLAG_ZREC | flags, dev_step=dev_step)
-    check(_lib.load().vfm_elbo_fwd_f32(C.byref(p), ptr(plan.x), ptr(plan.y), ptr(zrec), None, None, ptr(scalars), None,
+    z = _rec_layout(p, zrec)
+    check(_lib.load().vfm_elbo_fwd_f32(C.byref(p), ptr(plan.x), ptr(plan.y), ptr(z), None, None, ptr(scalars), None,
                                        None, None, None, ptr(out_pred), ptr(out_partials), None, ptr(out_grow),
-                                       current_stream_ptr(zrec.device)), "vfm_elbo_fwd_f32 (records)")
+                                       current_stream_ptr(z.device)), "vfm_elbo_fwd_f32 (records)")
     p.flags = spec.link_flag | (flags & FLAG_SHARE_GPU)
     return FwdState(out_pred, out_partials, None, out_grow, p, None)
 
@@ -573,10 +597,19 @@
     ix = _index_struct(plan)
     ix.occ_other = plan.occ_other.data_ptr()
     pipe = _lib.Pipe()
-    pipe.zrec = zrec.data_ptr()
+    p = st.problem
+    z = _rec_layout(p, zrec)
+    pipe.zrec = z.data_ptr()
     if next_plan is not None:
         if next_plan.occ_ptr is None:
             next_plan.build_index()
+        if isinstance(zrec_next, Records) != isinstance(zrec, Records):
+            raise ValueError("elbo_backward_adam_pipe: both record tables in one layout")
+        if isinstance(zrec_next, Records):
+            if zrec_next.z.stride(0) != z.stride(0) or zrec_next.hdr.stride(0) != zrec.hdr.stride(0):
+                raise ValueError("elbo_backward_adam_pipe: both record tables with the same strides")
+            pipe.zrec_next_hdr = zrec_next.hdr.data_ptr()
+            zrec_next = zrec_next.z
         pipe.zrec_next, pipe.next_occ_ptr, pipe.next_W = zrec_next.data_ptr(), next_plan.occ_ptr.data_ptr(), next_plan.W.data_ptr()
         pipe.next_step = int(next_step)
     if last_step is not None:
@@ -590,7 +623,6 @@
             rows = plan.lookahead_rows(la_next)
             if rows.numel() > 0:
                 ix.touched_ids, ix.n_touched = rows.data_ptr(), rows.numel()
-    p = st.problem
     p.flags = plan.spec.link_flag | (FLAG_SCALED_MOMENTS if scaled_moments else 0) | (p.flags & FLAG_SHARE_GPU)
     p.wrec = wrec.data_ptr() if wrec is not None else None
     p.dev_step = dev_step.data_ptr() if dev_step is not None else None
@@ -598,7 +630,7 @@
         C.byref(p), C.byref(ix), C.byref(pipe), ptr(entity_params), ptr(bias_params), ptr(scalars), ptr(inv_occ),
         ptr(plan.W), ptr(st.grow), ptr(st.partials), ptr(m_views[0]), ptr(v_views[0]), ptr(m_views[1]), ptr(v_views[1]),
         ptr(m_views[2]), ptr(v_views[2]), lr, beta1, beta2, eps_adam, int(step), ptr(loss_out),
-        current_stream_ptr(zrec.device)), "vfm_elbo_bwd_adam_pipe_f32")
+        current_stream_ptr(z.device)), "vfm_elbo_bwd_adam_pipe_f32")
 
 
 def elbo_backward_adam_lookahead(plan: BatchPlan, st: FwdState, next_plan: BatchPlan, entity_params, bias_params,
```

After: 516.1 million, median of 2. Within noise of the previous version (-0.1%).
